# MaxChen228/pingpong-selfplay-ai

Measured on AMD Instinct MI355X. Metric: env-steps/sec (whole node) at 65536 arenas, 1/2/4/8 GPUs; CPU-ref baseline, higher is better.
Workload: dtype f64 env state / f32 QNet; 1 GPU; configs[2]: 65536 arenas/GPU, full DQN train_iterative loop (act both players + env tick + PER push/sample + double-DQN update + Adam + target sync); arenas_per_gpu=65536, global_arenas=65536, pool=8, batch=256, updates_per_vector_step=1, memory_size=1000000, parallelism=dp1 (arena shards, 1 all-reduce/update)

## Files before the change

### include/pongmi.h

```cpp
#ifndef PONGMI_H
#define PONGMI_H

#include <stddef.h>
#include <stdint.h>

#ifdef __cplusplus
extern "C" {
#endif

#define PM_ABI_VERSION 25

#define PM_OK 0
#define PM_E_ARG (-1)
#define PM_E_SIZE (-2)
#define PM_E_LAUNCH (-3)
#define PM_E_COMM (-4)


typedef struct pm_env_params {
    double paddle_width, paddle_speed, magnus_factor, restitution, friction, ball_mass, radius;
    double speed_lo, speed_hi, spin_lo, spin_hi;
    double ang0_lo, ang0_hi, ang1_lo, ang1_hi;
    double half_width, speed_scale, inertia, jt_coef, inv_mass, inv_inertia;
    int32_t max_score, speed_scale_every, enable_spin, _pad;
} pm_env_params;

typedef struct pm_env_state {
    double *x, *y, *vx, *vy, *spin, *top, *bot;
    int32_t *scoreA, *scoreB, *bounces, *serves;
} pm_env_state;

int pm_env_reset(const pm_env_params* p, const pm_env_state* s, const uint8_t* mask, const double* inject,
                 int32_t inject_cap, uint64_t seed, float* obsA, float* obsB, int32_t* status, int32_t n,
                 void* stream);

int pm_env_step(const pm_env_params* p, const pm_env_state* s, const int8_t* aA, const int8_t* aB, float* obsA,
                float* obsB, float* rA, float* rB, uint8_t* done, float* term_obsA, float* term_obsB,
                int32_t autoreset, const double* inject, int32_t inject_cap, uint64_t seed, uint64_t counter,
                int32_t* status, int32_t n, void* stream);

int pm_collide(const double* in, const double* inertia, double* out, int32_t n, void* stream);

int pm_env_step1(const pm_env_params* p, const pm_env_state* s, int32_t aA, int32_t aB, float* out, uint32_t seq,
                 void* stream);
int pm_env_reset1(const pm_env_state* s, double vx, double vy, double spin, float* out, uint32_t seq, void* stream);
int pm_collide1(const double* row, double inertia, double* out, uint32_t seq, void* stream);
void* pm_host_mapped_alloc(int64_t bytes, void** dev);
int pm_host_mapped_free(void* host);


#define PM_QNET_NP 5452
#define PM_QNET_NHEAD 520
#define PM_QNET_HEAD_OFF 4672
#define PM_QNET_EPS_OFF 5192
#define PM_QNET_NW 9944
#define PM_GRAD_EPISODES 520
#define PM_GRAD_UPDATED 521
#define PM_GRAD_LEN 528

#define PM_FOLD_EVAL 0
#define PM_FOLD_TRAIN 1
#define PM_FOLD_TRAIN_FRESH 2

int pm_qnet_fold(const float* params, float* params_out, int32_t mode, uint64_t seed, uint64_t counter,
                 const uint64_t* counter_dev, float* w_eff, int32_t count, void* stream);

int pm_qnet_q(const float* w_eff, const float* x, float* q, int32_t n, void* stream);

int pm_qnet_act(const float* w_opp, const int32_t* opp_id, int32_t n_opp, const float* w_B, const float* obsA,
                const float* obsB, float epsilon, const double* eps_dev, uint64_t seed, uint64_t counter,
                const uint64_t* counter_dev, int8_t* aA, int8_t* aB, float* qA, float* qB, int32_t n,
                int32_t chunk0, int32_t chunk1, void* stream);

int pm_play(const pm_env_params* p, const float* w_nets, int32_t n_nets, const int32_t* blk_nets,
            const int32_t* blk_range, int32_t n_blocks, const int32_t* order, const double* serves, int32_t n,
            int32_t max_steps, int32_t* scoreA, int32_t* scoreB, int32_t* length, int8_t* last, int32_t* status,
            void* stream);

int pm_play_rnn(const pm_env_params* p, const float* w_qnet, int32_t n_qnet, const float* w_rnn, int32_t n_rnn,
                const int32_t* blk_nets, const int32_t* blk_range, int32_t n_blocks, const int32_t* order,
                const double* serves, int32_t n, int32_t max_steps, float* hc_scratch,
                int32_t* scoreA, int32_t* scoreB, int32_t* length, int8_t* last, int32_t* status, void* stream);
size_t pm_play_rnn_scratch_bytes(int32_t n_blocks);

int pm_play_rec(const pm_env_params* p, const float* w_nets, int32_t n_nets, const int32_t* blk_nets,
                const int32_t* blk_range, int32_t n_blocks, const int32_t* order, const double* serves, int32_t n,
                int32_t max_steps, int32_t* scoreA, int32_t* scoreB, int32_t* length, int8_t* last, int32_t* status,
                const int32_t* rec_row, int32_t n_rec, int32_t rec_cap, double* rec_f64, float* rec_q,
                int32_t* rec_i32, void* stream);
int pm_play_rnn_rec(const pm_env_params* p, const float* w_qnet, int32_t n_qnet, const float* w_rnn, int32_t n_rnn,
                    const int32_t* blk_nets, const int32_t* blk_range, int32_t n_blocks, const int32_t* order,
                    const double* serves, int32_t n, int32_t max_steps, float* hc_scratch,
                    int32_t* scoreA, int32_t* scoreB, int32_t* length, int8_t* last, int32_t* status,
                    const int32_t* rec_row, int32_t n_rec, int32_t rec_cap, double* rec_f64, float* rec_q,
                    int32_t* rec_i32, void* stream);

#define PM_ROLL_HEADS 264
int pm_rollout(const pm_env_params* p, const pm_env_state* s, const float* wA, const float* wB, const float* paramsB,
               float epsilon, uint64_t seed_env, uint64_t seed_net, uint64_t counter0, int32_t steps, float* heads_ws,
               float* obsA, float* obsB, int64_t* stats, int32_t n, void* stream);

typedef struct pm_roll_replay {
    float *trans;
    float *prios;
    void *per_work;
    float *ep_reward;
    int64_t pos, cap;
    float prio, alpha;
} pm_roll_replay;
int pm_rollout_push(const pm_env_params* p, const pm_env_state* s, const float* wA, const float* wB,
                    const float* paramsB, float epsilon, uint64_t seed_env, uint64_t seed_net, uint64_t counter0,
                    int32_t steps, float* heads_ws, float* obsA, float* obsB, const pm_roll_replay* rp, int64_t* stats,
                    int32_t n, void* stream);


#define PM_RNN_NP 192012
#define PM_RNN_NPARAM 174984
#define PM_RNN_NW 157456

int pm_rnn_fold(const float* params, float* params_out, int32_t mode, uint64_t seed, uint64_t counter,
                const uint64_t* counter_dev, float* w_eff, int32_t count, void* stream);

int pm_rnn_q(const float* w_eff, const float* x, float* h, float* c, const uint8_t* reset, float* q, int32_t n,
             void* stream);

int pm_rnn_act(const float* w_opp, const int32_t* opp_id, int32_t n_opp, const float* w_B, const float* obsA,
               const float* obsB, float* hA, float* cA, float* hB, float* cB, const uint8_t* reset, float epsilon,
               const double* eps_dev, uint64_t seed, uint64_t counter, const uint64_t* counter_dev, int8_t* aA,
               int8_t* aB, float* qA, float* qB, int32_t n, int32_t chunk0, int32_t chunk1, const int32_t* opp_list,
               const int32_t* opp_cnt, void* stream);


typedef struct pm_drqn_stats {
    int64_t steps;
    int64_t adam_t;
    float loss;
    float norm;
    float q_mean;
    int32_t status;
} pm_drqn_stats;

typedef struct pm_drqn {
    float *params;
    float *target;
    float *adam_m, *adam_v;
    float *grad;
    void *work;
    pm_drqn_stats *stats;
    const float *obs, *next;
    const int32_t *act;
    const float *rew;
    const uint8_t *done;
    const int32_t *enable;
    int32_t batch;
    int32_t T;
    int64_t target_update_interval;
    double gamma, lr, beta1, beta2, adam_eps, max_norm;
    int32_t poll_limit;
    int32_t reserved;
} pm_drqn;

int64_t pm_drqn_work_bytes(int32_t batch, int32_t T);
int pm_drqn_init(const pm_drqn *d, void *stream);
int pm_drqn_grads(const pm_drqn *d, void *stream);
int pm_drqn_apply(const pm_drqn *d, void *stream);
int pm_drqn_update(const pm_drqn *d, void *stream);


typedef struct pm_rnn_ctrl {
    uint64_t step;
    int64_t episodes;
    int64_t seq_count;
    int64_t seq_size;
    double epsilon;
    int64_t win_A, ep_A, win_P, ep_P;
    double reward_B;
    int32_t status;
    int32_t train;
} pm_rnn_ctrl;

typedef struct pm_rnn_selfplay {
    pm_env_params env;
    pm_env_state st;
    int32_t *opp;
    float *ep_reward;
    int32_t *ep_len;
    int32_t *ep_steps;
    uint8_t *reset;
    const float *w_opp;
    float *paramsB;
    float *w_B;
    float *hA, *cA, *hB, *cB;
    float *obsA, *obsB;
    int8_t *aA, *aB;
    float *trans;
    int64_t *seq_eps;
    int64_t *seq_mark;
    int64_t *fin;
    int64_t *partials;
    int32_t *opp_list;
    int32_t *opp_cnt;
    int32_t *enable;
    pm_rnn_ctrl *ctrl;
    int32_t n, n_pool, depth, T, chunk_A, chunk_P;
    int32_t max_steps;
    int32_t _pad;
    int64_t seq_cap, min_episodes;
    double min_epsilon, epsilon_decay, pool_ratio;
    uint64_t seed_env, seed_net;
    const float *hA_in, *cA_in;
    float *qA, *qB;
} pm_rnn_selfplay;

int pm_rnn_selfplay_init(const pm_rnn_selfplay *sp, void *stream);
int pm_rnn_selfplay_act(const pm_rnn_selfplay *sp, void *stream);
int pm_rnn_selfplay_env(const pm_rnn_selfplay *sp, const pm_drqn *d, void *stream);
int pm_rnn_selfplay_rollout(const pm_rnn_selfplay *sp, const pm_drqn *d, void *stream);
int pm_rnn_selfplay_step(const pm_rnn_selfplay *sp, const pm_drqn *d, void *stream);
int pm_rnn_selfplay_sample(const pm_rnn_selfplay *sp, const pm_drqn *d, int32_t u, void *stream);
int pm_rnn_selfplay_step_multi(const pm_rnn_selfplay *sp, const pm_drqn *d, int32_t updates, void *stream);
int pm_rnn_selfplay_act_part(const pm_rnn_selfplay *sp, int32_t part, void *stream);
int pm_rnn_selfplay_step_overlap(const pm_rnn_selfplay *sp, const pm_drqn *d, int32_t updates, void *side_stream,
                                 void *stream);
int pm_rnn_selfplay_finish_overlap(const pm_rnn_selfplay *sp, const pm_drqn *d, int32_t updates, void *side_stream,
                                   void *stream);


#define PM_TRANS_F 16

int64_t pm_per_work_bytes(int64_t cap);
int pm_per_sample(const float* prios, int64_t size, float alpha, float beta, const double* u, uint64_t seed,
                  uint64_t counter, int64_t* idx, float* w, int32_t bs, void* work, void* stream);

int pm_per_update(float* prios, const int64_t* idx, const float* err, int32_t bs, void* stream);
int pm_per_build(const float* prios, int64_t cap, float alpha, void* work, void* stream);


typedef struct pm_ctrl {
    uint64_t step;
    int64_t pos, size;
    int64_t train_steps;
    int64_t frame_idx;
    int64_t episodes;
    double epsilon;
    float max_prio;
    float last_loss;
    int64_t ep_step;
    int64_t win_A, ep_A, win_P, ep_P;
    double reward_B;
    int32_t status;
    int32_t max_bits;
} pm_ctrl;

typedef struct pm_selfplay {
    pm_env_params env;
    pm_env_state st;
    int32_t *opp;
    float *ep_reward;
    float *w_opp;
    float *paramsB;
    float *paramsT;
    float *w_B;
    float *adam_m, *adam_v;
    float *trans;
    float *prios;
    void *per_work;
    int64_t *idx;
    float *isw;
    float *grad;
    int64_t *partials;
    float *obsA, *obsB;
    int8_t *aA, *aB;
    float *hfeat;
    float *learn_heads;
    pm_ctrl *ctrl;
    int32_t *opp_list;
    int32_t *opp_cnt;
    int32_t n, n_pool, batch, world;
    int32_t chunk_A, chunk_P;
    int32_t fuse_apply;
    int32_t _pad0;
    int64_t cap;
    double gamma, alpha, lr, beta1, beta2, adam_eps;
    double min_epsilon, epsilon_decay, pool_ratio, beta_start;
    int64_t beta_frames, target_update_interval;
    uint64_t seed_env;
    uint64_t seed_net;
    float *featB;
    float *frow;
    int32_t frow_ready;
    int32_t _pad1;
} pm_selfplay;

#define PM_MAX_BATCH 256

int pm_selfplay_init(const pm_selfplay* sp, void* stream);
int pm_selfplay_prepare(const pm_selfplay* sp, void* stream);
int pm_selfplay_repair_tree(const pm_selfplay* sp, void* stream);
int pm_selfplay_rollout(const pm_selfplay* sp, void* stream);
int pm_selfplay_act(const pm_selfplay* sp, void* stream);
int pm_selfplay_env(const pm_selfplay* sp, void* stream);
int pm_selfplay_learn(const pm_selfplay* sp, void* stream);
int pm_selfplay_apply(const pm_selfplay* sp, void* stream);
int pm_selfplay_step(const pm_selfplay* sp, void* stream);

#define PM_ACT_ALL 0
#define PM_ACT_B 1
#define PM_ACT_A 2
int pm_selfplay_act_part(const pm_selfplay* sp, int32_t part, void* stream);
int pm_selfplay_learn_act(const pm_selfplay* sp, void* stream);
int pm_selfplay_actenv(const pm_selfplay* sp, void* stream);
int pm_selfplay_step_overlap(const pm_selfplay* sp, void* stream);

#define PM_UPD_FIRST 1
#define PM_UPD_LAST 2
int pm_selfplay_learn_ex(const pm_selfplay* sp, int32_t mode, int32_t with_act, void* stream);
int pm_selfplay_apply_ex(const pm_selfplay* sp, int32_t mode, void* stream);
int pm_selfplay_resample(const pm_selfplay* sp, void* stream);
int pm_selfplay_commit(const pm_selfplay* sp, void* stream);
int pm_selfplay_step_multi(const pm_selfplay* sp, int32_t updates, void* stream);


#define PM_COMM_ID_BYTES 128
typedef struct pm_comm pm_comm;
int pm_comm_unique_id(const char* rccl_path, uint8_t* id);
int pm_comm_init(const char* rccl_path, const uint8_t* id, int32_t nranks, int32_t rank, pm_comm** out);
int pm_comm_allreduce_f32(pm_comm* comm, float* buf, int64_t n, void* stream);
int pm_comm_destroy(pm_comm* comm);
int pm_comm_info(const pm_comm* comm, int32_t* nranks, int32_t* rank, int32_t* device);
int pm_selfplay_step_sharded(const pm_selfplay* sp, pm_comm* comm, int32_t updates, void* stream);
int pm_rnn_selfplay_step_sharded(const pm_rnn_selfplay* sp, const pm_drqn* d, pm_comm* comm, int32_t updates,
                                 void* stream);
int pm_rnn_selfplay_step_sharded_overlap(const pm_rnn_selfplay* sp, const pm_drqn* d, pm_comm* comm, int32_t updates,
                                         void* side_stream, void* stream);

#define PM_TIMER_ACTENV 0
#define PM_TIMER_LEARN 1
#define PM_TIMER_RNN_ACT 2
#define PM_TIMER_ENV_STEP 3
#define PM_TIMER_ROLLOUT 4
#define PM_TIMER_DRQN 5
#define PM_TIMER_LEARN_MULTI 6
#define PM_TIMER_N 7
int pm_timer_arm(int32_t kernel);
int pm_timer_read(int32_t kernel, float* ms);

const char* pm_last_error(void);
int pm_abi_version(void);
int32_t pm_sizeof(int32_t which);

#ifdef __cplusplus
}
#endif
#endif
```

### pingpong-selfplay-ai_amd/csrc/pm_mfma.h

```cpp
#pragma once
#include "pm_dev.h"

namespace pm {

typedef float f32x16 __attribute__((ext_vector_type(16)));
typedef __attribute__((address_space(3))) void lds_void;

constexpr int PLAIN = 4936;
enum : int {
    F_W1 = 0,
    F_W2 = 512,
    F_B1 = 4608,
    F_B2 = 4672,
    F_H = 4736,
    F_BH = 4992,
    F_SIZE = 5008,
};
static_assert(PLAIN + F_SIZE == PM_QNET_NW, "effective weight block size");

__device__ __forceinline__ int rho(int r) { return (r & 3) + 8 * (r >> 2); }

__device__ __forceinline__ float relu(float x) { return __int_as_float(max(__float_as_int(x), 0)); }

__device__ __forceinline__ void write_feature_frags(const float* __restrict__ p, float* __restrict__ w) {
    const int t = threadIdx.x, nt = blockDim.x;
    for (int k = t; k < PM_QNET_HEAD_OFF; k += nt) w[k] = p[k];
    float* f = w + PLAIN;
    for (int k = t; k < 512; k += nt) {
        const int jt = k >> 8, lane = (k >> 2) & 63, s = k & 3;
        const int row = 32 * jt + (lane & 31), kk = 2 * s + (lane >> 5);
        f[F_W1 + k] = kk == 0 ? p[B1 + row] : p[W1 + row * 7 + kk - 1];
    }
    for (int k = t; k < 4096; k += nt) {
        const int e = k & 3, lane = (k >> 2) & 63, rq = (k >> 8) & 3, tt = (k >> 10) & 1, jt = k >> 11;
        const int row = 32 * jt + (lane & 31), col = 32 * tt + rho(4 * rq + e) + 4 * (lane >> 5);
        f[F_W2 + k] = p[W2 + row * 64 + col];
    }
    for (int k = t; k < 64; k += nt) {
        const int r = k & 15, h = (k >> 4) & 1, jt = k >> 5;
        f[F_B1 + k] = p[B1 + 32 * jt + rho(r) + 4 * h];
        f[F_B2 + k] = p[B2 + 32 * jt + rho(r) + 4 * h];
    }
}

__device__ __forceinline__ void write_head_frags(const float* heads, float* __restrict__ w) {
    const int t = threadIdx.x, nt = blockDim.x;
    for (int k = t; k < 260; k += nt) w[WH + k] = heads[k];
    float* f = w + PLAIN;
    for (int k = t; k < 256; k += nt) {
        const int c = k & 3, r = (k >> 2) & 15, tt = (k >> 6) & 1, h = k >> 7;
        f[F_H + k] = heads[c * 64 + 32 * tt + rho(r) + 4 * h];
    }
    if (t < 16) f[F_BH + t] = t < 4 ? heads[256 + t] : 0.f;
}

constexpr int kLwChunks = (F_SIZE / 4 + 63) / 64;
constexpr int kLwFloats = kLwChunks * 256;

template <int N>
__device__ __forceinline__ void copy_lds_f32(const float* __restrict__ src, float* dst) {
    const int wv = threadIdx.x >> 6, lane = threadIdx.x & 63, nw = blockDim.x >> 6;
    for (int c = wv; c * 64 < N; c += nw) {
        const int k = min(c * 64 + lane, N - 1);
        __builtin_amdgcn_global_load_lds((const void*)(src + k), (lds_void*)(dst + c * 64), 4, 0, 0);
    }
}
constexpr int pad64(int n) { return (n + 63) / 64 * 64; }
template <int N>
__device__ __forceinline__ void copy_lds_f32x4(const float* __restrict__ src, float* dst) {
    static_assert(N % 4 == 0, "whole float4s");
    const int wv = threadIdx.x >> 6, lane = threadIdx.x & 63, nw = blockDim.x >> 6;
    const float4* s4 = reinterpret_cast<const float4*>(src);
    for (int c = wv; c * 256 < N; c += nw) {
        const int k = min(c * 64 + lane, N / 4 - 1);
        __builtin_amdgcn_global_load_lds((const void*)(s4 + k), (lds_void*)(dst + c * 256), 16, 0, 0);
    }
}
constexpr int pad256(int n) { return (n + 255) / 256 * 256; }

__device__ __forceinline__ void stage_frags_lds(const float* __restrict__ w, float* lw, int rot) {
    const int wv = threadIdx.x >> 6, lane = threadIdx.x & 63, nw = blockDim.x >> 6;
    const float4* src = reinterpret_cast<const float4*>(w + PLAIN);
    float4* lw4 = reinterpret_cast<float4*>(lw);
    rot %= kLwChunks;
    for (int c0 = wv; c0 < kLwChunks; c0 += nw) {
        const int c = c0 + rot < kLwChunks ? c0 + rot : c0 + rot - kLwChunks;
        const int k = min(c * 64 + lane, F_SIZE / 4 - 1);
        __builtin_amdgcn_global_load_lds((const void*)(src + k), (lds_void*)(lw4 + c * 64), 16, 0, 0);
    }
}

constexpr int kListNets = 64;
constexpr int kListBlock = 256;
struct OppListSmem {
    int woff[kListBlock / 64][kListNets];
    int noff[kListNets], ncnt[kListNets];
};
__device__ __forceinline__ void write_opp_lists(int nn, int32_t* opp_list, int32_t* opp_cnt, OppListSmem& sm, int blk,
                                                int i, bool valid, int net) {
    if (nn > kListNets) return;
    const int lane = threadIdx.x & 63, wv = threadIdx.x >> 6;
    int rank = 0;
    for (int k = 0; k < nn; ++k) {
        const bool m = valid && net == k;
        const unsigned long long b = __ballot(m);
        if (m) rank = __popcll(b & ((1ull << lane) - 1ull));
        if (lane == 0) sm.woff[wv][k] = __popcll(b);
    }
    __syncthreads();
    if (wv == 0) {
        int acc = 0;
        if (lane < nn) {
            for (int w = 0; w < kListBlock / 64; ++w) {
                const int c = sm.woff[w][lane];
                sm.woff[w][lane] = acc;
                acc += c;
            }
        }
        const int inc = wave_incl_scan_i32(acc);
        if (lane < nn) { sm.ncnt[lane] = acc; sm.noff[lane] = inc - acc; }
    }
    __syncthreads();
    if (valid) opp_list[(size_t)blk * kListBlock + sm.noff[net] + sm.woff[wv][net] + rank] = i;
    if ((int)threadIdx.x < nn) opp_cnt[(size_t)blk * nn + threadIdx.x] = (sm.noff[threadIdx.x] << 16) | sm.ncnt[threadIdx.x];
}

__device__ __forceinline__ void compact_load(const int32_t* __restrict__ id, int lo, int hi, int (&v)[16]) {
    const int base = lo + 16 * (int)threadIdx.x;
    if (base + 16 <= hi && (reinterpret_cast<uintptr_t>(id + base) & 15) == 0) {
        const int4* p4 = reinterpret_cast<const int4*>(id + base);
#pragma unroll
        for (int q = 0; q < 4; ++q) {
            const int4 x = p4[q];
            v[4 * q] = x.x; v[4 * q + 1] = x.y; v[4 * q + 2] = x.z; v[4 * q + 3] = x.w;
        }
    } else {
#pragma unroll
        for (int r = 0; r < 16; ++r) v[r] = base + r < hi ? id[base + r] : -1;
    }
}
__device__ __forceinline__ void compact_scan(const int (&v)[16], int net, int lo, int* list, int* count, int* wtot) {
    const int t = threadIdx.x, lane = t & 63, wv = t >> 6, nw = blockDim.x >> 6;
    const int base = lo + 16 * t;
    unsigned mask = 0;
#pragma unroll
    for (int r = 0; r < 16; ++r) mask |= (v[r] == net ? 1u : 0u) << r;
    const int c = __popc(mask);
    const int incl = wave_incl_scan_i32(c);
    if (lane == 63) wtot[wv] = incl;
    __syncthreads();
    int off = 0, total = 0;
    for (int w = 0; w < nw; ++w) {
        off += w < wv ? wtot[w] : 0;
        total += wtot[w];
    }
    int p = off + incl - c;
    while (mask) {
        const int r = __ffs(mask) - 1;
        mask &= mask - 1;
        list[p++] = base + r;
    }
    if (t == 0) *count = total;
}

struct TileOut {
    int8_t* act;
    float* q;
    double eps;
    uint64_t seed, ctr;
};

__device__ __forceinline__ void heads_to_frags(const float* heads, float* hf) {
    for (int k = threadIdx.x; k < 260; k += blockDim.x) {
        if (k < 256) {
            const int c = k & 3, r = (k >> 2) & 15, tt = (k >> 6) & 1, h = k >> 7;
            hf[k] = heads[c * 64 + 32 * tt + rho(r) + 4 * h];
        } else {
            hf[k] = heads[k];
        }
    }
}

__device__ __forceinline__ void tile_hidden(const float* lw, const float (&xs)[4], int lane, f32x16 (&c2)[2]) {
    const int h = lane >> 5;
    f32x16 c1[2];
    const f32x16 zero = {};
#pragma unroll
    for (int jt = 0; jt < 2; ++jt) {
        const float4 w = reinterpret_cast<const float4*>(lw + F_W1)[jt * 64 + lane];
        c1[jt] = __builtin_amdgcn_mfma_f32_32x32x2f32(w.x, xs[0], zero, 0, 0, 0);
        c1[jt] = __builtin_amdgcn_mfma_f32_32x32x2f32(w.y, xs[1], c1[jt], 0, 0, 0);
        c1[jt] = __builtin_amdgcn_mfma_f32_32x32x2f32(w.z, xs[2], c1[jt], 0, 0, 0);
        c1[jt] = __builtin_amdgcn_mfma_f32_32x32x2f32(w.w, xs[3], c1[jt], 0, 0, 0);
    }
#pragma unroll
    for (int jt = 0; jt < 2; ++jt)
#pragma unroll
        for (int r = 0; r < 16; ++r) c1[jt][r] = relu(c1[jt][r]);
    const float4* w2 = reinterpret_cast<const float4*>(lw + F_W2) + lane;
#pragma unroll
    for (int jt = 0; jt < 2; ++jt) {
        const float4* b = reinterpret_cast<const float4*>(lw + F_B2 + (jt * 2 + h) * 16);
#pragma unroll
        for (int q4 = 0; q4 < 4; ++q4) {
            const float4 v = b[q4];
            c2[jt][4 * q4 + 0] = v.x; c2[jt][4 * q4 + 1] = v.y; c2[jt][4 * q4 + 2] = v.z; c2[jt][4 * q4 + 3] = v.w;
        }
    }
    float4 wcur = w2[0];
#pragma unroll
    for (int g8 = 0; g8 < 16; ++g8) {
        const int jt = g8 >> 3, t = (g8 >> 2) & 1, rq = g8 & 3;
        const float4 wnext = w2[((g8 + 1) & 15) * 64];
        c2[jt] = __builtin_amdgcn_mfma_f32_32x32x2f32(wcur.x, c1[t][4 * rq + 0], c2[jt], 0, 0, 0);
        c2[jt] = __builtin_amdgcn_mfma_f32_32x32x2f32(wcur.y, c1[t][4 * rq + 1], c2[jt], 0, 0, 0);
        c2[jt] = __builtin_amdgcn_mfma_f32_32x32x2f32(wcur.z, c1[t][4 * rq + 2], c2[jt], 0, 0, 0);
        c2[jt] = __builtin_amdgcn_mfma_f32_32x32x2f32(wcur.w, c1[t][4 * rq + 3], c2[jt], 0, 0, 0);
        wcur = wnext;
        __builtin_amdgcn_sched_barrier(0);
    }
}

__device__ __forceinline__ void tile_heads(const float* hf, const f32x16 (&c2)[2], int lane, float (&q)[3]) {
    const int h = lane >> 5;
    float v = 0.f, a0 = 0.f, a1 = 0.f, a2 = 0.f;
    const float4* hw = reinterpret_cast<const float4*>(hf + h * 128);
#pragma unroll
    for (int t = 0; t < 2; ++t) {
#pragma unroll
        for (int r = 0; r < 16; ++r) {
            const float x = relu(c2[t][r]);
            const float4 w = hw[t * 16 + r];
            v = fmaf(w.x, x, v);
            a0 = fmaf(w.y, x, a0);
            a1 = fmaf(w.z, x, a1);
            a2 = fmaf(w.w, x, a2);
        }
        __builtin_amdgcn_sched_barrier(0);
    }
    v += __shfl_xor(v, 32);
    a0 += __shfl_xor(a0, 32);
    a1 += __shfl_xor(a1, 32);
    a2 += __shfl_xor(a2, 32);
    v += hf[256];
    a0 += hf[257];
    a1 += hf[258];
    a2 += hf[259];
    const float mean = ((a0 + a1) + a2) / 3.0f;
    q[0] = v + (a0 - mean);
    q[1] = v + (a1 - mean);
    q[2] = v + (a2 - mean);
}

__device__ __forceinline__ void hidden_half(const float* lw, const float (&xs)[4], int lane, int jt, f32x16& c2) {
    const int h = lane >> 5;
    f32x16 c1[2];
    const f32x16 zero = {};
#pragma unroll
    for (int t = 0; t < 2; ++t) {
        const float4 w = reinterpret_cast<const float4*>(lw + F_W1)[t * 64 + lane];
        c1[t] = __builtin_amdgcn_mfma_f32_32x32x2f32(w.x, xs[0], zero, 0, 0, 0);
        c1[t] = __builtin_amdgcn_mfma_f32_32x32x2f32(w.y, xs[1], c1[t], 0, 0, 0);
        c1[t] = __builtin_amdgcn_mfma_f32_32x32x2f32(w.z, xs[2], c1[t], 0, 0, 0);
        c1[t] = __builtin_amdgcn_mfma_f32_32x32x2f32(w.w, xs[3], c1[t], 0, 0, 0);
    }
#pragma unroll
    for (int t = 0; t < 2; ++t)
#pragma unroll
        for (int r = 0; r < 16; ++r) c1[t][r] = relu(c1[t][r]);
    {
        const float4* b = reinterpret_cast<const float4*>(lw + F_B2 + (jt * 2 + h) * 16);
#pragma unroll
        for (int q4 = 0; q4 < 4; ++q4) {
            const float4 v = b[q4];
            c2[4 * q4 + 0] = v.x; c2[4 * q4 + 1] = v.y; c2[4 * q4 + 2] = v.z; c2[4 * q4 + 3] = v.w;
        }
    }
    const float4* w2 = reinterpret_cast<const float4*>(lw + F_W2) + lane + jt * 8 * 64;
    float4 wcur = w2[0];
#pragma unroll
    for (int g = 0; g < 8; ++g) {
        const int t = g >> 2, rq = g & 3;
        const float4 wnext = w2[((g + 1) & 7) * 64];
        c2 = __builtin_amdgcn_mfma_f32_32x32x2f32(wcur.x, c1[t][4 * rq + 0], c2, 0, 0, 0);
        c2 = __builtin_amdgcn_mfma_f32_32x32x2f32(wcur.y, c1[t][4 * rq + 1], c2, 0, 0, 0);
        c2 = __builtin_amdgcn_mfma_f32_32x32x2f32(wcur.z, c1[t][4 * rq + 2], c2, 0, 0, 0);
        c2 = __builtin_amdgcn_mfma_f32_32x32x2f32(wcur.w, c1[t][4 * rq + 3], c2, 0, 0, 0);
        wcur = wnext;
        __builtin_amdgcn_sched_barrier(0);
    }
}

__device__ __forceinline__ void heads_half(const float* hf, const f32x16& c2, int lane, int t, float (&acc)[4]) {
    const float4* hw = reinterpret_cast<const float4*>(hf + (lane >> 5) * 128) + t * 16;
#pragma unroll
    for (int r = 0; r < 16; ++r) {
        const float x = relu(c2[r]);
        const float4 w = hw[r];
        acc[0] = fmaf(w.x, x, acc[0]);
        acc[1] = fmaf(w.y, x, acc[1]);
        acc[2] = fmaf(w.z, x, acc[2]);
        acc[3] = fmaf(w.w, x, acc[3]);
    }
}

__device__ __forceinline__ void heads_finish(const float (&acc)[4], const float* hf, float (&q)[3]) {
    float v = acc[0], a0 = acc[1], a1 = acc[2], a2 = acc[3];
    v += __shfl_xor(v, 32);
    a0 += __shfl_xor(a0, 32);
    a1 += __shfl_xor(a1, 32);
    a2 += __shfl_xor(a2, 32);
    v += hf[256];
    a0 += hf[257];
    a1 += hf[258];
    a2 += hf[259];
    const float mean = ((a0 + a1) + a2) / 3.0f;
    q[0] = v + (a0 - mean);
    q[1] = v + (a1 - mean);
    q[2] = v + (a2 - mean);
}

__device__ __forceinline__ void tile_inputs(const float* __restrict__ o, int h, float (&xs)[4]) {
    xs[0] = h ? o[0] : 1.0f;
    xs[1] = o[1 + h];
    xs[2] = o[3 + h];
    xs[3] = o[5 + h];
}

struct TilePre {
    bool have;
    float xs[4];
};

__device__ __forceinline__ void run_tiles(const float* lw, const float* __restrict__ obs, const int* list, int count,
                                          const TileOut& out, const TilePre pre) {
    const int lane = threadIdx.x & 63, wave = threadIdx.x >> 6, nw = blockDim.x >> 6;
    const int h = lane >> 5, col = lane & 31;
    const int ntiles = (count + 31) >> 5;
    int tl = wave;
    if (tl >= ntiles) return;
    int arena = list[min(tl * 32 + col, count - 1)];
    float xs[4];
    if (pre.have) {
#pragma unroll
        for (int k = 0; k < 4; ++k) xs[k] = pre.xs[k];
    } else {
        tile_inputs(obs + (size_t)arena * 7, h, xs);
    }
    for (; tl < ntiles; tl += nw) {
        const int row = tl * 32 + col;
        const bool valid = row < count;
        const int tn = tl + nw;
        int arena_n = arena;
        float xn[4] = {xs[0], xs[1], xs[2], xs[3]};
        if (tn < ntiles) {
            arena_n = list[min(tn * 32 + col, count - 1)];
            tile_inputs(obs + (size_t)arena_n * 7, h, xn);
        }
        f32x16 c2[2];
#ifdef PM_DIAG
        if (tl == wave) {
            __builtin_amdgcn_s_waitcnt(0);
            PM_BLK(5);
        }
#endif
        tile_hidden(lw, xs, lane, c2);
#ifdef PM_DIAG
        if (tl == wave) PM_BLK(6);
#endif
        float q[3];
        tile_heads(lw + F_H, c2, lane, q);
#ifdef PM_DIAG
        if (tl == wave) PM_BLK(7);
#endif
        int a = argmax3(q);
        if (out.eps >= 0.0) {
            const U4 rr = philox64((uint32_t)arena, TAG_ACT, out.ctr, out.seed);
            if (u53(rr.x, rr.y) < out.eps) a = below(rr.z, 3u);
        }
        if (h == 0 && valid) {
            if (out.act) out.act[arena] = (int8_t)a;
            if (out.q) {
                out.q[(size_t)arena * 3 + 0] = q[0];
                out.q[(size_t)arena * 3 + 1] = q[1];
                out.q[(size_t)arena * 3 + 2] = q[2];
            }
        }
        arena = arena_n;
#pragma unroll
        for (int k = 0; k < 4; ++k) xs[k] = xn[k];
    }
}

constexpr int kChunkB = 256;

struct ActGrid {
    int n, n_opp, chunk0, chunk1, side_b;
    __host__ __device__ int nb() const { return side_b ? (n + kChunkB - 1) / kChunkB : 0; }
    __host__ __device__ int na0() const { return (n + chunk0 - 1) / chunk0; }
    __host__ __device__ int na1() const { return (n + chunk1 - 1) / chunk1; }
    __host__ __device__ int blocks() const { return nb() + na0() + (n_opp - 1) * na1(); }
};

constexpr int kActBlock = 256;
constexpr int kListMax = 4096;
constexpr int kListMaxLearn = 16384;

template <int LIST>
struct ActSharedT {
    static constexpr int kList = LIST;
    float lw[kLwFloats];
    int list[LIST];
    int count;
    int wtot[16];
    int lpre[LIST / 256], loff[LIST / 256], lcnt[LIST / 256];
};
using ActShared = ActSharedT<kListMax>;
using ActSharedLearn = ActSharedT<kListMaxLearn>;
static_assert(kListMaxLearn / 256 <= 64, "one lane per list segment in act_block's scan");

template <class Sh>
__device__ __forceinline__ void act_block(Sh& sh, const ActGrid& g, const float* __restrict__ w_opp,
                                          const int32_t* __restrict__ opp, const float* __restrict__ w_B,
                                          const float* __restrict__ obsA, const float* __restrict__ obsB,
                                          TileOut outA, TileOut outB, int b,
                                          const int32_t* __restrict__ opp_list = nullptr,
                                          const int32_t* __restrict__ opp_cnt = nullptr) {
    const float* w;
    const float* obs;
    TileOut out;
    int net, lo, hi;
    bool compact;
    if (b < g.nb()) {
        w = w_B; obs = obsB; out = outB; net = -1; lo = b * kChunkB; hi = min(lo + kChunkB, g.n); compact = false;
    } else {
        b -= g.nb();
        if (b < g.na0()) { net = 0; lo = b * g.chunk0; hi = min(lo + g.chunk0, g.n); }
        else { b -= g.na0(); net = 1 + b / g.na1(); lo = (b % g.na1()) * g.chunk1; hi = min(lo + g.chunk1, g.n); }
        w = w_opp + (size_t)net * PM_QNET_NW; obs = obsA; out = outA;
        compact = opp != nullptr;
        if (!compact && net != 0) return;
    }
    __builtin_amdgcn_s_setprio(2);
    stage_frags_lds(w, sh.lw, b);
    const bool lists = compact && opp_list != nullptr && (lo & 255) == 0 && (((hi - lo) & 255) == 0 || hi == g.n);
    int ids[16];
    if (compact && !lists) compact_load(opp, lo, hi, ids);
    PM_BLK(4);
    if (lists) {
        const int g0 = lo >> 8, G = (hi - lo + 255) >> 8;
        if (threadIdx.x < 64) {
            const int lane = threadIdx.x;
            const int v = lane < G ? opp_cnt[(size_t)(g0 + lane) * g.n_opp + net] : 0;
            const int c = v & 0xFFFF;
            const int incl = wave_incl_scan_i32(c);
            if (lane < G) { sh.lpre[lane] = incl - c; sh.loff[lane] = v >> 16; sh.lcnt[lane] = c; }
            if (lane == 63) sh.count = incl;
        }
        __syncthreads();
        const int j0 = threadIdx.x & 15;
        for (int seg = threadIdx.x >> 4; seg < G; seg += blockDim.x >> 4) {
            const int c = sh.lcnt[seg], dst = sh.lpre[seg];
            const int32_t* src = opp_list + (size_t)(g0 + seg) * 256 + sh.loff[seg];
            int v[16];
#pragma unroll
            for (int r = 0; r < 16; ++r) v[r] = j0 + 16 * r < c ? src[j0 + 16 * r] : 0;
#pragma unroll
            for (int r = 0; r < 16; ++r)
                if (j0 + 16 * r < c) sh.list[dst + j0 + 16 * r] = v[r];
        }
    } else if (compact) {
        compact_scan(ids, net, lo, sh.list, &sh.count, sh.wtot);
    } else {
        if (threadIdx.x == 0) sh.count = hi - lo;
        for (int k = threadIdx.x; k < hi - lo; k += blockDim.x) sh.list[k] = lo + k;
    }
    TilePre pre{false, {0.f, 0.f, 0.f, 0.f}};
    if (!compact && !lists) {
        const int wave = threadIdx.x >> 6, lane = threadIdx.x & 63, cnt = hi - lo;
        if (wave * 32 < cnt) {
            pre.have = true;
            tile_inputs(obs + (size_t)(lo + min(wave * 32 + (lane & 31), cnt - 1)) * 7, lane >> 5, pre.xs);
        }
    }
    __syncthreads();
    PM_BLK(1);
    __builtin_amdgcn_s_setprio(0);
    run_tiles(sh.lw, obs, sh.list, sh.count, out, pre);
}

constexpr int kFeatTileFloats = 8 * 64 * 4;
__device__ __forceinline__ void store_f4_sc1(__amdgpu_buffer_rsrc_t r, int byte_off, float4 v) {
    typedef __attribute__((ext_vector_type(4))) unsigned u32x4;
    __builtin_amdgcn_raw_buffer_store_b128(*reinterpret_cast<const u32x4*>(&v), r, byte_off, 0, 16 );
}
__device__ __forceinline__ void feat_tiles(float* lw, const float* __restrict__ w, const float* __restrict__ obs, int n,
                                           int t0, int t1, float* __restrict__ feat) {
    const int wave = threadIdx.x >> 6, lane = threadIdx.x & 63, nw = blockDim.x >> 6;
    stage_frags_lds(w, lw, t0);
    int tl = t0 + wave;
    float xs[4] = {0.f, 0.f, 0.f, 0.f};
    if (tl < t1) tile_inputs(obs + (size_t)min(tl * 32 + (lane & 31), n - 1) * 7, lane >> 5, xs);
    __syncthreads();
    for (; tl < t1; tl += nw) {
        const int tn = tl + nw;
        float xn[4] = {xs[0], xs[1], xs[2], xs[3]};
        if (tn < t1) tile_inputs(obs + (size_t)min(tn * 32 + (lane & 31), n - 1) * 7, lane >> 5, xn);
        f32x16 c2[2];
        tile_hidden(lw, xs, lane, c2);
        const __amdgpu_buffer_rsrc_t rs = __builtin_amdgcn_make_buffer_rsrc(feat, (short)0, 0x7fffffff, 0x00020000);
        const int off = (tl * 8 * 64 + lane) * 16;
#pragma unroll
        for (int k = 0; k < 4; ++k) {
            store_f4_sc1(rs, off + k * 64 * 16, make_float4(c2[0][4 * k], c2[0][4 * k + 1], c2[0][4 * k + 2], c2[0][4 * k + 3]));
            store_f4_sc1(rs, off + (4 + k) * 64 * 16,
                         make_float4(c2[1][4 * k], c2[1][4 * k + 1], c2[1][4 * k + 2], c2[1][4 * k + 3]));
        }
#pragma unroll
        for (int k = 0; k < 4; ++k) xs[k] = xn[k];
    }
}
__device__ __forceinline__ void feat_load(const float* __restrict__ feat, int tile, int lane, f32x16 (&c2)[2]) {
    const float4* src = reinterpret_cast<const float4*>(feat) + (size_t)tile * 8 * 64 + lane;
#pragma unroll
    for (int k = 0; k < 4; ++k) {
        const float4 a = src[k * 64], b = src[(4 + k) * 64];
        c2[0][4 * k] = a.x; c2[0][4 * k + 1] = a.y; c2[0][4 * k + 2] = a.z; c2[0][4 * k + 3] = a.w;
        c2[1][4 * k] = b.x; c2[1][4 * k + 1] = b.y; c2[1][4 * k + 2] = b.z; c2[1][4 * k + 3] = b.w;
    }
}

}
```

### pingpong-selfplay-ai_amd/csrc/pm_selfplay.hip

```cpp
#include <algorithm>
#include <cmath>

#include "pm_host.h"
#include "pm_mfma.h"
#include "pm_per.h"

using namespace pm;

#ifdef PM_DIAG
static __device__ unsigned long long pm_diag_env[8][1024];
static __device__ unsigned long long pm_diag_side[4][1024];
#define PM_SIDE(k, sb, v)                                                        \
    do {                                                                         \
        if (threadIdx.x == 0 && (sb) < 1024) pm_diag_side[(k)][(sb)] = (v);      \
    } while (0)
#define PM_ENV_STAMP(k, blk)                                                                   \
    do {                                                                                       \
        asm volatile("" ::: "memory");                                                         \
        if (threadIdx.x == 0 && (blk) < 1024) pm_diag_env[(k)][(blk)] = __builtin_amdgcn_s_memrealtime(); \
    } while (0)
#define PM_ENV_STAMP_DRAIN(k, blk)                                                             \
    do {                                                                                       \
        asm volatile("s_waitcnt vmcnt(0) lgkmcnt(0)" ::: "memory");                            \
        if (threadIdx.x == 0 && (blk) < 1024) pm_diag_env[(k)][(blk)] = __builtin_amdgcn_s_memrealtime(); \
    } while (0)
#else
#define PM_SIDE(k, sb, v) \
    do {                  \
    } while (0)
#define PM_ENV_STAMP(k, blk) \
    do {                     \
    } while (0)
#define PM_ENV_STAMP_DRAIN(k, blk) \
    do {                           \
    } while (0)
#endif

namespace {

constexpr int kBlock = 256;
static_assert(kBlock == kRowBlock, "row staging assumes kRowBlock-thread blocks");
constexpr int kLearn = 1024;
constexpr int kGradN = PM_GRAD_EPISODES;
static_assert(PM_GRAD_EPISODES == PM_QNET_NHEAD && PM_GRAD_UPDATED == kGradN + 1 && PM_GRAD_LEN >= kGradN + 2, "grad layout");
constexpr uint32_t kHashEmpty = 0xFFFFFFFFu;

__device__ __forceinline__ bool learner_active(const pm_selfplay& sp) {
    const int64_t s = sp.ctrl->size + sp.n;
    return (s < sp.cap ? s : sp.cap) >= sp.batch;
}

__device__ __forceinline__ double beta_of(const pm_selfplay& sp, int64_t frame) {
    const double b = sp.beta_start + (double)frame * (1.0 - sp.beta_start) / (double)sp.beta_frames;
    return b < 1.0 ? b : 1.0;
}

__device__ __forceinline__ float push_prio(int64_t size, float max_prio) { return size == 0 ? 1.0f : max_prio; }
__device__ __forceinline__ PushRange push_of(const pm_selfplay& sp, int64_t pos, int64_t size, float max_prio) {
    return PushRange{pos, sp.n, sp.cap, prio_pow(push_prio(size, max_prio), (float)sp.alpha)};
}
}

template <int NS = PER_BS, class Hook = NoHook>
__device__ __forceinline__ void sample_block(const pm_selfplay& sp, int b, bool pending, PerSampleSmem& sm,
                                             int64_t* sidx = nullptr, Hook l2done = Hook()) {
    static_assert(NS == PER_BS || NS == PER_BS / 2, "64 or 32 samples per block");
    const pm_ctrl* c = sp.ctrl;
    const int64_t s = c->size + sp.n;
    const int64_t size = s < sp.cap ? s : sp.cap;
    const int64_t frame = c->frame_idx + 1;
    const PushRange pr = pending ? push_of(sp, c->pos, c->size, c->max_prio) : PushRange{0, 0, sp.cap, 0.f};
    const uint64_t key = sp.seed_env;
    per_sample_block(
        size >= sp.batch, size, per_tree(sp.per_work, sp.cap), pr, beta_of(sp, frame), b * NS,
        min(sp.batch, b * NS + NS), sm,
        [&](int j) {
            const U4 r = philox64((uint32_t)j, TAG_PER, (uint64_t)frame, key);
            return u53(r.x, r.y);
        },
        [&](int j, int64_t idx, float w) {
            sp.idx[j] = idx;
            sp.isw[j] = w;
            if (sidx) sidx[j - b * NS] = idx;
        },
        l2done);
}

union ActSpShared {
    ActShared act;
    PerSampleSmem per;
};
constexpr int kFeatTilesAct = 8, kFeatTilesLearn = 16;
#ifndef PM_ENV_WT
#define PM_ENV_WT 6
#endif
constexpr bool kEnvWTRows = (PM_ENV_WT & 1) != 0, kEnvWTState = (PM_ENV_WT & 2) != 0, kEnvWTObs = (PM_ENV_WT & 4) != 0;
__host__ __device__ inline int feat_ntiles(int n) { return (n + 31) / 32; }

__global__ __launch_bounds__(kActBlock, 4) void k_act_sp(const pm_selfplay sp, int part) {
    __shared__ __attribute__((aligned(16))) ActSpShared sh;
    PM_BLK(0);
    const int nsb = part == PM_ACT_A ? 0 : (sp.batch + PER_BS - 1) / PER_BS;
    {
        const ActGrid g{sp.n, sp.n_pool + 1, sp.chunk_A, sp.chunk_P, part == PM_ACT_A ? 0 : 1};
        const int fb = (int)blockIdx.x - nsb - g.blocks();
        if (fb >= 0) {
            const int t0 = fb * kFeatTilesAct;
            feat_tiles(sh.act.lw, sp.w_B, sp.obsB, sp.n, t0, min(t0 + kFeatTilesAct, feat_ntiles(sp.n)), sp.featB);
            return;
        }
    }
    if ((int)blockIdx.x < nsb) {
        PM_STAMP(64);
        sample_block(sp, (int)blockIdx.x, true, sh.per);
        PM_STAMP(65);
        PM_BLK_END();
        return;
    }
    if ((int)blockIdx.x == nsb) PM_STAMP_ANY(70);
    const ActGrid g{sp.n, sp.n_pool + 1, sp.chunk_A, sp.chunk_P, part == PM_ACT_A ? 0 : 1};
    const TileOut outA{sp.aA, nullptr, -1.0, 0, 0};
    const TileOut outB{sp.aB, nullptr, -1.0, 0, 0};
    act_block(sh.act, g, sp.w_opp, sp.n_pool > 0 ? sp.opp : nullptr, sp.w_B, sp.obsA, sp.obsB, outA, outB,
              (int)blockIdx.x - nsb, sp.n_pool + 1 <= kListNets ? sp.opp_list : nullptr, sp.opp_cnt);
    PM_BLK_END();
}

__device__ __forceinline__ void batch_row_fwd(const pm_selfplay& sp, const float* lw, const float* hf0, const float* hf1,
                                              int64_t id, bool nxt, int lane, f32x16 (&c2)[2], float (&qb)[3],
                                              float (&qt)[3], float (&rb)[2]) {
    float xs[4];
    const float* tr = sp.trans + id * PM_TRANS_F;
    tile_inputs(tr + (nxt ? 8 : 0), lane >> 5, xs);
    rb[0] = tr[7];
    rb[1] = tr[15];
    tile_hidden(lw, xs, lane, c2);
    tile_heads(hf0, c2, lane, qb);
    tile_heads(hf1, c2, lane, qt);
}

template <bool WT = false>
__device__ __forceinline__ void store_hfeat(float* hfeat, int j, bool nxt, int lane, const f32x16 (&c2)[2],
                                            const float (&qb)[3], const float (&qt)[3], const float (&rb)[2]) {
    float* row = hfeat + (size_t)j * 80;
    const int h = lane >> 5;
    if (!nxt) {
#pragma unroll
        for (int t = 0; t < 2; ++t)
#pragma unroll
            for (int q = 0; q < 16; ++q) st_out<WT>(&row[32 * t + rho(q) + 4 * h], relu(c2[t][q]));
    }
    if (h == 0) {
        if (!nxt) {
            st_out<WT>(&row[64], qb[0]); st_out<WT>(&row[65], qb[1]); st_out<WT>(&row[66], qb[2]);
            st_out<WT>(&row[67], rb[0]);
            st_out<WT>(&row[71], rb[1]);
        } else {
            st_out<WT>(&row[68], qb[0]); st_out<WT>(&row[69], qb[1]); st_out<WT>(&row[70], qb[2]);
            st_out<WT>(&row[72], qt[0]); st_out<WT>(&row[73], qt[1]); st_out<WT>(&row[74], qt[2]);
        }
    }
}

__device__ __forceinline__ void env_fwd_block(const pm_selfplay& sp, int f, bool pending = true) {
    __shared__ __attribute__((aligned(16))) float lw[kLwFloats];
    __shared__ __attribute__((aligned(16))) float hf[2][264];
    if (!learner_active(sp)) return;
    stage_frags_lds(sp.w_B, lw, f * 5);
    for (int k = threadIdx.x; k < 2 * 264; k += blockDim.x) hf[k / 264][k % 264] = sp.learn_heads[k];
    __syncthreads();
    const int lane = threadIdx.x & 63, B = sp.batch;
    const int r0 = f * 128 + (int)(threadIdx.x >> 6) * 32;
    if (r0 >= 2 * B) return;
    const int r = min(r0 + (lane & 31), 2 * B - 1);
    const bool nxt = r >= B;
    const int j = nxt ? r - B : r;
    const int64_t id = sp.idx[j];
    const pm_ctrl* c = sp.ctrl;
    const bool mine = r0 + (lane & 31) < 2 * B && !(pending && push_of(sp, c->pos, c->size, c->max_prio).covers(id));
    f32x16 c2[2];
    float qb[3], qt[3];
    float rb[2];
    batch_row_fwd(sp, lw, hf[0], hf[1], id, nxt, lane, c2, qb, qt, rb);
    if (mine) store_hfeat(sp.hfeat, j, nxt, lane, c2, qb, qt, rb);
}

struct SampleFwd32Smem {
    PerSampleSmem per;
    float lw[kLwFloats];
    float hf[pad256(2 * 264)];
    int64_t sidx[PER_BS / 2];
    float part[2][64][8];
};
__device__ __forceinline__ void sample_fwd_block32(const pm_selfplay& sp, int b, SampleFwd32Smem& sm) {
    constexpr int NS = PER_BS / 2;
    sample_block<NS>(sp, b, true, sm.per, sm.sidx, [&] {
        stage_frags_lds(sp.w_B, sm.lw, b * 5);
        copy_lds_f32x4<2 * 264>(sp.learn_heads, sm.hf);
    });
    if (!learner_active(sp)) return;
    __syncthreads();
    PM_BLK(1);
    const int lane = threadIdx.x & 63, B = sp.batch;
    const int wv = __builtin_amdgcn_readfirstlane(threadIdx.x >> 6);
    const bool nxt = (wv >> 1) != 0;
    const int jt = wv & 1;
    const int j = b * NS + (lane & 31);
    const int64_t id = sm.sidx[min(j, B - 1) - b * NS];
    const pm_ctrl* c = sp.ctrl;
    const bool mine = j < B && !push_of(sp, c->pos, c->size, c->max_prio).covers(id);
    float xs[4];
    const float* tr = sp.trans + id * PM_TRANS_F;
    tile_inputs(tr + (nxt ? 8 : 0), lane >> 5, xs);
    const float rb0 = tr[7], rb1 = tr[15];
    f32x16 c2;
    hidden_half(sm.lw, xs, lane, jt, c2);
    const float* hf0 = sm.hf;
    const float* hf1 = sm.hf + 264;
    float ab[4] = {0.f, 0.f, 0.f, 0.f}, at[4] = {0.f, 0.f, 0.f, 0.f};
    float* row = sp.hfeat + (size_t)j * 80;
    const int h = lane >> 5;
    if (jt == 0) {
        heads_half(hf0, c2, lane, 0, ab);
        if (nxt) heads_half(hf1, c2, lane, 0, at);
        *reinterpret_cast<float4*>(&sm.part[nxt][lane][0]) = make_float4(ab[0], ab[1], ab[2], ab[3]);
        if (nxt) *reinterpret_cast<float4*>(&sm.part[nxt][lane][4]) = make_float4(at[0], at[1], at[2], at[3]);
    }
    if (mine && !nxt) {
#pragma unroll
        for (int q = 0; q < 16; ++q) row[32 * jt + rho(q) + 4 * h] = relu(c2[q]);
    }
    __syncthreads();
    if (jt == 0) return;
    {
        const float4 pa = *reinterpret_cast<const float4*>(&sm.part[nxt][lane][0]);
        ab[0] = pa.x; ab[1] = pa.y; ab[2] = pa.z; ab[3] = pa.w;
    }
    heads_half(hf0, c2, lane, 1, ab);
    float qb[3], qt[3];
    heads_finish(ab, hf0, qb);
    if (nxt) {
        const float4 pt = *reinterpret_cast<const float4*>(&sm.part[nxt][lane][4]);
        at[0] = pt.x; at[1] = pt.y; at[2] = pt.z; at[3] = pt.w;
        heads_half(hf1, c2, lane, 1, at);
        heads_finish(at, hf1, qt);
    }
    if (mine && h == 0) {
        if (!nxt) {
            row[64] = qb[0]; row[65] = qb[1]; row[66] = qb[2];
            row[67] = rb0;
            row[71] = rb1;
        } else {
            row[68] = qb[0]; row[69] = qb[1]; row[70] = qb[2];
            row[72] = qt[0]; row[73] = qt[1]; row[74] = qt[2];
        }
    }
}

__device__ __forceinline__ void write_opp_lists(const pm_selfplay& sp, OppListSmem& sm, int blk, int i, bool valid,
                                                int net) {
    write_opp_lists(sp.n_pool + 1, sp.opp_list, sp.opp_cnt, sm, blk, i, valid, net);
}

struct EnvSmem {
    float lds[2][kBlock][7];
    long long red[kBlock / 64][6];
    OppListSmem ol;
};
struct ActEnvSmem {
    EnvSmem e;
    float lw[kLwFloats];
};

template <bool ACT>
__device__ __forceinline__ void env_block(const pm_selfplay& sp, int blk, EnvSmem& sm, float* lw) {
    const int i0 = blk * kBlock;
    const int i = i0 + threadIdx.x;
    const int lane = threadIdx.x & 63, wv = threadIdx.x >> 6;
    const bool valid = i < sp.n;
    const int ii = valid ? i : sp.n - 1;
    const pm_ctrl* c = sp.ctrl;
    if (blk == 0) PM_STAMP_ANY(72);
    PM_ENV_STAMP(0, blk);
    float xs[2][4];
    f32x16 fc2[2][2];
    if (ACT && sp.featB) {
        if (threadIdx.x < 65)
            reinterpret_cast<float4*>(lw + F_H)[threadIdx.x] =
                reinterpret_cast<const float4*>(sp.w_B + PLAIN + F_H)[threadIdx.x];
#pragma unroll
        for (int k = 0; k < 2; ++k) feat_load(sp.featB, blk * 8 + 2 * wv + k, lane, fc2[k]);
    } else if (ACT) {
        stage_frags_lds(sp.w_B, lw, blk);
#pragma unroll
        for (int k = 0; k < 2; ++k) {
            const int row = min(i0 + 64 * wv + 32 * k + (lane & 31), sp.n - 1);
            tile_inputs(sp.obsB + (size_t)row * 7, lane >> 5, xs[k]);
        }
    }
    const uint32_t ns = (uint32_t)__builtin_nontemporal_load(&sp.st.serves[ii]);
    const int64_t pos = c->pos, size = c->size;
    const float cmaxp = c->max_prio;
    const uint64_t cstep = c->step;
    const double ceps = c->epsilon;
    const int o = sp.opp[ii];
    const float er0 = sp.ep_reward[ii];
    Arena a = load_arena(sp.st, ii);
    const int aA = sp.aA[ii];
    int aB = ACT ? 0 : sp.aB[ii];
    __builtin_amdgcn_sched_barrier(0);
    const float maxp = push_prio(size, cmaxp);
    float* leaf = per_tree(sp.per_work, sp.cap).leaf;
    const float pval = prio_pow(maxp, (float)sp.alpha);

    int onext, eps_a;
    bool eps_hit;
    double svx, svy, sspn;
    {
        const U4 rr = philox64((uint32_t)ii, TAG_ACT, cstep, sp.seed_env);
        eps_hit = u53(rr.x, rr.y) < ceps;
        eps_a = (int)below(rr.z, 3u);
        const U4 q = philox((uint32_t)ii, TAG_OPP, ns, 0u, sp.seed_env);
        onext = (sp.n_pool > 0 && u53(q.x, q.y) < sp.pool_ratio) ? 1 + below(q.z, (uint32_t)sp.n_pool) : 0;
        philox_serve(sp.env, (uint32_t)ii, ns, sp.seed_env, svx, svy, sspn);
        asm volatile("" ::"v"(onext), "v"(svx), "v"(svy), "v"(sspn), "v"(eps_hit), "v"(eps_a));
        __builtin_amdgcn_sched_barrier(0);
    }
    if (ACT) {
        __syncthreads();
        PM_ENV_STAMP(7, blk);
        int act[2];
#pragma unroll
        for (int k = 0; k < 2; ++k) {
            float q[3];
            if (sp.featB) {
                tile_heads(lw + F_H, fc2[k], lane, q);
            } else {
                f32x16 c2[2];
                tile_hidden(lw, xs[k], lane, c2);
                tile_heads(lw + F_H, c2, lane, q);
            }
            act[k] = argmax3(q);
            if (sp.featB && sp.frow) {
                const int ar = i0 + 64 * wv + 32 * k + (lane & 31);
                if (ar < sp.n) {
                    int64_t slot = pos + ar;
                    if (slot >= sp.cap) slot -= sp.cap;
                    float4* fr = reinterpret_cast<float4*>(sp.frow + slot * 64) + (lane >> 5);
#pragma unroll
                    for (int jt = 0; jt < 2; ++jt)
#pragma unroll
                        for (int q4 = 0; q4 < 4; ++q4)
                            st_f4<kEnvWTRows>(fr + 8 * jt + 2 * q4,
                                              make_float4(relu(fc2[k][jt][4 * q4]), relu(fc2[k][jt][4 * q4 + 1]),
                                                          relu(fc2[k][jt][4 * q4 + 2]), relu(fc2[k][jt][4 * q4 + 3])));
                }
            }
        }
        aB = lane < 32 ? act[0] : act[1];
    }
    PM_ENV_STAMP(1, blk);
    if (eps_hit) aB = eps_a;
    float oA[7], oB[7];
    observe(a, oA, oB);
    float rA, rB;
    const int d = tick(sp.env, a, aA, aB, rA, rB);
    float nA[7], nB[7];
    observe(a, nA, nB);
#ifdef PM_DIAG
    asm volatile("" ::"v"(nA[0]), "v"(nB[1]), "v"(d));
#endif
    PM_ENV_STAMP(2, blk);
    const float er = er0 + rB;
    const bool fin = valid && d;
    {
        const bool win = er > 0.f;
        const unsigned long long mf = __ballot(fin), mA = __ballot(fin && o == 0), mwA = __ballot(fin && o == 0 && win);
        const unsigned long long mP = __ballot(fin && o != 0), mwP = __ballot(fin && o != 0 && win);
        const int rs = wave_sum(fin ? (int)er : 0);
        if (lane == 0) {
            sm.red[wv][0] = __popcll(mf); sm.red[wv][1] = __popcll(mA); sm.red[wv][2] = __popcll(mwA);
            sm.red[wv][3] = __popcll(mP); sm.red[wv][4] = __popcll(mwP); sm.red[wv][5] = rs;
        }
    }
    int onew = o;
    if (valid) {
        int64_t slot = pos + i;
        if (slot >= sp.cap) slot -= sp.cap;
        float4* row = reinterpret_cast<float4*>(sp.trans + slot * PM_TRANS_F);
        st_f4<kEnvWTRows>(row + 0, make_float4(oB[0], oB[1], oB[2], oB[3]));
        st_f4<kEnvWTRows>(row + 1, make_float4(oB[4], oB[5], oB[6], rB));
        st_f4<kEnvWTRows>(row + 2, make_float4(nB[0], nB[1], nB[2], nB[3]));
        st_f4<kEnvWTRows>(row + 3, make_float4(nB[4], nB[5], nB[6], __int_as_float(aB | (d << 8))));
        sp.prios[slot] = maxp;
        leaf[slot] = pval;
        float ernew = er;
        if (d) {
            onew = onext;
            serve(a, svx, svy, sspn);
            sp.st.serves[i] = (int32_t)ns + 1;
            ernew = 0.f;
            observe(a, nA, nB);
        }
        store_arena<kEnvWTState>(sp.st, i, a);
        sp.opp[i] = onew;
        sp.aB[i] = (int8_t)aB;
        sp.ep_reward[i] = ernew;
    }
    PM_ENV_STAMP(3, blk);
#pragma unroll
    for (int k = 0; k < 7; ++k) { sm.lds[0][threadIdx.x][k] = nA[k]; sm.lds[1][threadIdx.x][k] = nB[k]; }
    __syncthreads();
    PM_ENV_STAMP(4, blk);
    if (threadIdx.x < 6) {
        long long t = 0;
        for (int w = 0; w < kBlock / 64; ++w) t += sm.red[w][threadIdx.x];
        sp.partials[(size_t)blk * 8 + threadIdx.x] = t;
    }
    write_opp_lists(sp, sm.ol, blk, i, valid, onew);
    PM_ENV_STAMP(5, blk);
    copy_rows7<kEnvWTObs>(sp.obsA, sm.lds[0], i0, sp.n);
    copy_rows7<kEnvWTObs>(sp.obsB, sm.lds[1], i0, sp.n);
    PM_ENV_STAMP_DRAIN(6, blk);
}

__global__ __launch_bounds__(kBlock) void k_env(const pm_selfplay sp) {
    const int blk = (int)blockIdx.x;
    const int nenv = (sp.n + kBlock - 1) / kBlock;
    if (blk >= nenv) {
        env_fwd_block(sp, blk - nenv);
        return;
    }
    __shared__ __attribute__((aligned(16))) EnvSmem sm;
    env_block<false>(sp, blk, sm, nullptr);
}

union ActEnvShared {
    ActEnvSmem ae;
    SampleFwd32Smem sf32;
};
__global__ __launch_bounds__(kBlock) void k_actenv(const pm_selfplay sp) {
    __shared__ __attribute__((aligned(16))) ActEnvShared sh;
    const int nsb = (sp.batch + 31) / 32;
    if ((int)blockIdx.x < nsb) {
        PM_BLK(0);
        sample_fwd_block32(sp, (int)blockIdx.x, sh.sf32);
        PM_BLK_END();
        return;
    }
    env_block<true>(sp, (int)blockIdx.x - nsb, sh.ae.e, sh.ae.lw);
}

__global__ __launch_bounds__(kBlock) void k_sp_init(const pm_selfplay sp) {
    __shared__ __attribute__((aligned(16))) float lds[kBlock][7];
    const int i0 = blockIdx.x * kBlock;
    const int i = i0 + threadIdx.x;
    float oA[7] = {0}, oB[7] = {0};
    int net = 0;
    if (i < sp.n) {
        const uint32_t ns = (uint32_t)sp.st.serves[i];
        const U4 q = philox((uint32_t)i, TAG_OPP, ns, 0u, sp.seed_env);
        net = (sp.n_pool > 0 && u53(q.x, q.y) < sp.pool_ratio) ? 1 + below(q.z, (uint32_t)sp.n_pool) : 0;
        sp.opp[i] = net;
        Arena a;
        double vx, vy, spn;
        philox_serve(sp.env, (uint32_t)i, ns, sp.seed_env, vx, vy, spn);
        serve(a, vx, vy, spn);
        store_arena(sp.st, i, a);
        sp.st.serves[i] = (int32_t)ns + 1;
        sp.ep_reward[i] = 0.f;
        observe(a, oA, oB);
    }
    {
        __shared__ OppListSmem ol;
        write_opp_lists(sp, ol, blockIdx.x, i, i < sp.n, net);
    }
    store_rows7(sp.obsA, lds, oA, i0, sp.n);
    store_rows7(sp.obsB, lds, oB, i0, sp.n);
}

struct __attribute__((aligned(16))) ApplySmem {
    float hp[pad256(PM_QNET_NHEAD)];
    float tmu[pad256(PM_QNET_NHEAD)];
    float m[pad256(PM_QNET_NHEAD)], v[pad256(PM_QNET_NHEAD)];
    float g[PM_QNET_NHEAD + 2];
    float ak[2];
    float nact[132], ntrain[132];
    float heads[3][260];
    double eps_next;
};

__device__ __forceinline__ void adam_consts(const pm_selfplay& sp, int64_t ts, ApplySmem& sm) {
    const double bc1 = 1.0 - pow(sp.beta1, (double)ts);
    const double bc2 = 1.0 - pow(sp.beta2, (double)ts);
    sm.ak[0] = (float)(sp.lr / bc1);
    sm.ak[1] = (float)sqrt(bc2);
}
__device__ __forceinline__ void adam_const_lane(const pm_selfplay& sp, int64_t ts, ApplySmem& sm, int which) {
    const double bc = 1.0 - pow(which ? sp.beta2 : sp.beta1, (double)ts);
    sm.ak[which] = which ? (float)sqrt(bc) : (float)(sp.lr / bc);
}

__device__ __forceinline__ void load_apply_inputs(const pm_selfplay& sp, ApplySmem& sm, bool with_grad) {
    copy_lds_f32x4<PM_QNET_NHEAD>(sp.paramsB + PM_QNET_HEAD_OFF, sm.hp);
    copy_lds_f32x4<PM_QNET_NHEAD>(sp.paramsT + PM_QNET_HEAD_OFF, sm.tmu);
    copy_lds_f32x4<PM_QNET_NHEAD>(sp.adam_m, sm.m);
    copy_lds_f32x4<PM_QNET_NHEAD>(sp.adam_v, sm.v);
    if (with_grad)
        for (int k = threadIdx.x; k < PM_QNET_NHEAD + 2; k += blockDim.x) sm.g[k] = sp.grad[k];
}

__device__ __forceinline__ void derive_weights(const pm_selfplay& sp, ApplySmem& sm) {
    const int t = threadIdx.x;
    float* lh = sp.learn_heads;
    const int g = (t - 256) >> 8, u = (t - 256) & 255;
    if (t >= 256 && g == 0) {
        fold_heads_from(sm.hp, nullptr, sm.nact, PM_FOLD_TRAIN_FRESH, sm.heads[0], sp.paramsB + PM_QNET_EPS_OFF, u, 256);
    } else if (t >= 256 && g == 1) {
        fold_heads_from(sm.hp, nullptr, sm.ntrain, PM_FOLD_TRAIN_FRESH, sm.heads[1], lh + 528, u, 256);
    } else if (t >= 256 && g == 2) {
        fold_heads_from(sm.tmu, nullptr, nullptr, PM_FOLD_EVAL, sm.heads[2], nullptr, u, 256);
    }
    __syncthreads();
    write_head_frags(sm.heads[0], sp.w_B);
    heads_to_frags(sm.heads[1], lh);
    heads_to_frags(sm.heads[2], lh + 264);
}

__device__ __forceinline__ void derive_weights_lds(ApplySmem& sm) {
    const int t = threadIdx.x;
    const int g = (t - 256) >> 8, u = (t - 256) & 255;
    if (t >= 256 && g == 1) {
        fold_heads_from(sm.hp, nullptr, sm.ntrain, PM_FOLD_TRAIN_FRESH, sm.heads[1], nullptr, u, 256);
    } else if (t >= 256 && g == 2) {
        fold_heads_from(sm.tmu, nullptr, nullptr, PM_FOLD_EVAL, sm.heads[2], nullptr, u, 256);
    }
    __syncthreads();
}

__device__ __forceinline__ void gen_both_noises(const pm_selfplay& sp, ApplySmem& sm, uint64_t act_ctr,
                                                uint64_t train_ctr) {
    const int t = threadIdx.x, half = blockDim.x / 2;
    if (t < half) gen_noise(sp.seed_net, TAG_NOISE_ACT, act_ctr, sm.nact, t, half);
    else gen_noise(sp.seed_net, TAG_NOISE_TRAIN, train_ctr, sm.ntrain, t - half, half);
}
__device__ __forceinline__ void gen_both_noises_on(const pm_selfplay& sp, ApplySmem& sm, uint64_t act_ctr,
                                                   uint64_t train_ctr, int t0) {
    const int u = (int)threadIdx.x - t0;
    if (u < 0 || u >= 512) return;
    if (u < 256) gen_noise(sp.seed_net, TAG_NOISE_ACT, act_ctr, sm.nact, u, 256);
    else gen_noise(sp.seed_net, TAG_NOISE_TRAIN, train_ctr, sm.ntrain, u - 256, 256);
}

__device__ __forceinline__ void adam_one(const pm_selfplay& sp, ApplySmem& sm, int k, float gsum, bool store = true) {
    const float step_size = sm.ak[0], bc2s = sm.ak[1];
    const float g = gsum / (float)sp.world;
    float m = sm.m[k], v = sm.v[k], p = sm.hp[k];
    m = m + (float)(1.0 - sp.beta1) * (g - m);
    v = v * (float)sp.beta2 + (float)(1.0 - sp.beta2) * g * g;
    const float denom = sqrtf(v) / bc2s + (float)sp.adam_eps;
    p = p - step_size * (m / denom);
    if (store) {
        sp.paramsB[PM_QNET_HEAD_OFF + k] = p;
        sp.adam_m[k] = m;
        sp.adam_v[k] = v;
    }
    sm.hp[k] = p;
    sm.m[k] = m;
    sm.v[k] = v;
}
__device__ __forceinline__ void apply_adam(const pm_selfplay& sp, ApplySmem& sm) {
    const int t = threadIdx.x, nt = blockDim.x;
    if (sm.g[kGradN + 1] > 0.5f)
        for (int k = t; k < PM_QNET_NHEAD; k += nt) adam_one(sp, sm, k, sm.g[k]);
}
__device__ __forceinline__ void apply_finish(const pm_selfplay& sp, ApplySmem& sm, const pm_ctrl& cs, int mode) {
    const int t = threadIdx.x, nt = blockDim.x;
    const bool train = sm.g[kGradN + 1] > 0.5f;
    const int64_t ts = cs.train_steps + (train ? 1 : 0);
    const uint64_t step = cs.step;
    PM_STAMP(20);
    if (train && ts % sp.target_update_interval == 0) {
        for (int k = t; k < PM_QNET_NHEAD; k += nt) sm.tmu[k] = sm.hp[k];
        for (int k = t; k < PM_QNET_NP; k += nt) {
            const int h = k - PM_QNET_HEAD_OFF;
            sp.paramsT[k] = (h >= 0 && h < PM_QNET_NHEAD) ? sm.hp[h] : sp.paramsB[k];
        }
        __syncthreads();
    }
    derive_weights(sp, sm);
    PM_STAMP(21);
    if (t == 0) {
        pm_ctrl* c = sp.ctrl;
        if (mode & PM_UPD_FIRST) {
            const double e = sm.eps_next;
            c->epsilon = e > sp.min_epsilon ? e : sp.min_epsilon;
        }
        if (train) { c->train_steps = ts; c->frame_idx = cs.frame_idx + 1; }
        if (mode & PM_UPD_LAST) {
            c->pos = (cs.pos + sp.n) % sp.cap;
            const int64_t s = cs.size + sp.n;
            c->size = s < sp.cap ? s : sp.cap;
            c->step = step + 1;
        }
    }
}

template <typename Emit>
__device__ __forceinline__ void push_rows_fwd(const pm_selfplay& sp, const float* lw, const float* hf,
                                              const int64_t* sidx, const int* plist, const int* pcnt, int wv, int lane,
                                              Emit emit) {
    int pre[5] = {0, 0, 0, 0, 0};
#pragma unroll
    for (int w = 0; w < 4; ++w) pre[w + 1] = pre[w] + pcnt[w];
    const int np = pre[4];
    if (wv * 32 >= 2 * np) return;
    const int rr = min(wv * 32 + (lane & 31), 2 * np - 1);
    const bool nxt = rr >= np;
    const int k = nxt ? rr - np : rr;
    const int w = k >= pre[3] ? 3 : k >= pre[2] ? 2 : k >= pre[1] ? 1 : 0;
    const int pw = k >= pre[3] ? pre[3] : k >= pre[2] ? pre[2] : k >= pre[1] ? pre[1] : 0;
    const int j = plist[w * 64 + k - pw];
    f32x16 c2[2];
    float qb[3], qt[3], rb[2];
    batch_row_fwd(sp, lw, hf, hf + 264, sidx[j], nxt, lane, c2, qb, qt, rb);
    if (wv * 32 + (lane & 31) < 2 * np) emit(j, nxt, lane, c2, qb, qt, rb);
}

constexpr int kPushPollMax = 20000;
constexpr int PM_CTRL_PUSH_TIMEOUT = 1;
constexpr int PM_CTRL_NAN_PRIO = 2;
__device__ __forceinline__ bool push_handoff(int mode, bool train) { return (mode & PM_UPD_FIRST) && train; }
__device__ __forceinline__ int* push_flag(const pm_selfplay& sp) {
    return reinterpret_cast<int*>(sp.hfeat + (size_t)2 * sp.batch * 80);
}
__device__ __forceinline__ int push_token(const pm_ctrl& cs) { return (int)((uint32_t)cs.step + 1u); }
__device__ __forceinline__ uint32_t* tr_epoch(const pm_selfplay& sp) {
    return reinterpret_cast<uint32_t*>(sp.hfeat + (size_t)2 * sp.batch * 80) + 1;
}
constexpr int kPushGF = 76;
constexpr int kPushGN = 75;
__device__ __forceinline__ uint64_t* push_granules(const pm_selfplay& sp) {
    return reinterpret_cast<uint64_t*>(sp.hfeat + (size_t)(2 * sp.batch + 8) * 80);
}
__device__ __forceinline__ void push_publish(uint64_t* g, uint32_t tag, float v) {
    __hip_atomic_store(g, ((uint64_t)tag << 32) | __float_as_uint(v), __ATOMIC_RELAXED, __HIP_MEMORY_SCOPE_AGENT);
}

__device__ __forceinline__ bool push_wait(const pm_selfplay& sp, const pm_ctrl& cs) {
    const int* flag = push_flag(sp);
    const int tok = push_token(cs);
    for (int it = 0; __hip_atomic_load(flag, __ATOMIC_RELAXED, __HIP_MEMORY_SCOPE_AGENT) != tok; ++it) {
        if (it == kPushPollMax) {
            sp.ctrl->status = cs.status | PM_CTRL_PUSH_TIMEOUT;
            return false;
        }
        __builtin_amdgcn_s_sleep(2);
    }
    return true;
}

struct PushFwdSmem {
    float lw[kLwFloats];
    float hf[pad256(2 * 264)];
    int64_t sidx[PM_MAX_BATCH];
    int plist[PM_MAX_BATCH];
    int pcnt[16];
    float part[8][64][8];
};

__device__ __forceinline__ void push_rows_fwd2(const pm_selfplay& sp, PushFwdSmem& sm, int wv, int lane, float* pay,
                                               uint32_t gtag) {
    uint64_t* pg = push_granules(sp);
    auto put = [&](int j, int f, float v) {
        if (gtag) push_publish(pg + (size_t)j * kPushGF + f, gtag, v);
        else st_out<true>(pay + (size_t)j * 80 + f, v);
    };
    int pre[5] = {0, 0, 0, 0, 0};
#pragma unroll
    for (int w = 0; w < 4; ++w) pre[w + 1] = pre[w] + sm.pcnt[w];
    const int np = pre[4];
    const int ntile = (2 * np + 31) >> 5;
    const int jt = wv & 1, h = lane >> 5;
    const float* hf0 = sm.hf;
    const float* hf1 = sm.hf + 264;
    for (int it = 0; it * 8 < ntile; ++it) {
        const int tile = it * 8 + (wv >> 1);
        const bool act = tile < ntile;
        f32x16 c2 = {};
        float ab[4] = {0.f, 0.f, 0.f, 0.f}, at[4] = {0.f, 0.f, 0.f, 0.f};
        float rb0 = 0.f, rb1 = 0.f;
        bool nxt = false, mine = false;
        int j = 0;
        if (act) {
            const int r0 = tile * 32 + (lane & 31);
            const int rr = min(r0, 2 * np - 1);
            nxt = rr >= np;
            const int k = nxt ? rr - np : rr;
            const int w = k >= pre[3] ? 3 : k >= pre[2] ? 2 : k >= pre[1] ? 1 : 0;
            const int pw = k >= pre[3] ? pre[3] : k >= pre[2] ? pre[2] : k >= pre[1] ? pre[1] : 0;
            j = sm.plist[w * 64 + k - pw];
            mine = r0 < 2 * np;
            const float* tr = sp.trans + sm.sidx[j] * PM_TRANS_F;
            float xs[4];
            tile_inputs(tr + (nxt ? 8 : 0), h, xs);
            rb0 = tr[7];
            rb1 = tr[15];
            hidden_half(sm.lw, xs, lane, jt, c2);
            if (mine && !nxt) {
#pragma unroll
                for (int q = 0; q < 16; ++q) put(j, 32 * jt + rho(q) + 4 * h, relu(c2[q]));
            }
            if (jt == 0) {
                heads_half(hf0, c2, lane, 0, ab);
                heads_half(hf1, c2, lane, 0, at);
                *reinterpret_cast<float4*>(&sm.part[wv >> 1][lane][0]) = make_float4(ab[0], ab[1], ab[2], ab[3]);
                *reinterpret_cast<float4*>(&sm.part[wv >> 1][lane][4]) = make_float4(at[0], at[1], at[2], at[3]);
            }
        }
        __syncthreads();
        if (act && jt == 1) {
            const float4 pb = *reinterpret_cast<const float4*>(&sm.part[wv >> 1][lane][0]);
            const float4 pt = *reinterpret_cast<const float4*>(&sm.part[wv >> 1][lane][4]);
            ab[0] = pb.x; ab[1] = pb.y; ab[2] = pb.z; ab[3] = pb.w;
            at[0] = pt.x; at[1] = pt.y; at[2] = pt.z; at[3] = pt.w;
            heads_half(hf0, c2, lane, 1, ab);
            heads_half(hf1, c2, lane, 1, at);
            float qb[3], qt[3];
            heads_finish(ab, hf0, qb);
            heads_finish(at, hf1, qt);
            if (mine && h == 0) {
                if (!nxt) {
                    put(j, 64, qb[0]); put(j, 65, qb[1]); put(j, 66, qb[2]);
                    put(j, 67, rb0);
                    put(j, 71, rb1);
                } else {
                    put(j, 68, qb[0]); put(j, 69, qb[1]); put(j, 70, qb[2]);
                    put(j, 72, qt[0]); put(j, 73, qt[1]); put(j, 74, qt[2]);
                }
            }
        }
        if ((it + 1) * 8 < ntile) __syncthreads();
    }
}
__device__ __forceinline__ pm_ctrl push_fwd_block(const pm_selfplay& sp, int mode, PushFwdSmem& sm, bool push2, bool pushg) {
    const int t = threadIdx.x, lane = t & 63, wv = t >> 6, B = sp.batch;
    PM_STAMP_ANY(50);
    stage_frags_lds(sp.w_B, sm.lw, 0);
    copy_lds_f32x4<2 * 264>(sp.learn_heads, sm.hf);
    const int64_t id = t < B ? sp.idx[t] : 0;
    const uint32_t gtag = pushg ? __hip_atomic_load(tr_epoch(sp), __ATOMIC_RELAXED, __HIP_MEMORY_SCOPE_AGENT) + 1u : 0u;
    __builtin_amdgcn_sched_barrier(0);
    const pm_ctrl cs = *sp.ctrl;
    const int64_t s_after = cs.size + sp.n < sp.cap ? cs.size + sp.n : sp.cap;
    if (!push_handoff(mode, s_after >= B)) {
        if ((mode & PM_UPD_FIRST) && t == 0) st_out<true>(push_flag(sp), push_token(cs));
        return cs;
    }
    if (pushg && t == 0) st_out<true>(push_flag(sp), push_token(cs));
    const bool ip = t < B && push_of(sp, cs.pos, cs.size, cs.max_prio).covers(id);
    const unsigned long long m = __ballot(ip);
    if (ip) sm.plist[wv * 64 + __popcll(m & ((1ull << lane) - 1ull))] = t;
    if (lane == 0) sm.pcnt[wv] = __popcll(m);
    if (t < B) sm.sidx[t] = id;
    __syncthreads();
    PM_STAMP_ANY(51);
    float* pay = sp.hfeat + (size_t)B * 80;
    if (push2)
        push_rows_fwd2(sp, sm, wv, lane, pay, gtag);
    else
        push_rows_fwd(sp, sm.lw, sm.hf, sm.sidx, sm.plist, sm.pcnt, wv, lane,
                      [&](int j, bool nxt, int ln, const f32x16 (&c2)[2], const float (&qb)[3], const float (&qt)[3],
                          const float (&rb)[2]) { store_hfeat<true>(pay, j, nxt, ln, c2, qb, qt, rb); });
    PM_STAMP_ANY(52);
    if (pushg) return cs;
    asm volatile("s_waitcnt vmcnt(0)" ::: "memory");
    __syncthreads();
    PM_STAMP_ANY(53);
    if (t == 0) st_out<true>(push_flag(sp), push_token(cs));
    return cs;
}

constexpr int kTrSlots = PM_MAX_BATCH + 8;
constexpr int kTrHash = 1024;
constexpr uint32_t kTrEmpty = 0xFFFFFFFFu;
constexpr int kTrPollMax = 20000;
constexpr int PM_CTRL_TREE_TIMEOUT = 4;
constexpr int PM_CTRL_TREE_REPAIRED = 8;
struct TreeRefreshSmem {
    __attribute__((aligned(16))) float lf[kTrSlots][PER_SUB];
    __attribute__((aligned(16))) double ls[kTrSlots][PER_FAN];
    double subv[kTrSlots];
    uint32_t subid[kTrSlots], chid[kTrSlots];
    int16_t cmap[kTrSlots][PER_FAN];
    uint32_t skey[kTrHash];
    int sslot[kTrHash];
    uint32_t ckey[kTrHash];
    int cslot[kTrHash];
    uint32_t ikey[512];
    int iwin[512];
    uint32_t eidx[kTrSlots];
    int esub[kTrSlots];
    float leaf_new[PM_MAX_BATCH];
    float maxp_next;
    int scattered, ok, nsub, nch;
};
__device__ __forceinline__ uint64_t* tr_granules(const pm_selfplay& sp) {
    return reinterpret_cast<uint64_t*>(sp.hfeat + (size_t)(2 * sp.batch + 1) * 80);
}
__device__ __forceinline__ void tr_publish(const pm_selfplay& sp, int k, uint32_t v, uint32_t tag) {
    __hip_atomic_store(tr_granules(sp) + k, ((uint64_t)tag << 32) | v, __ATOMIC_RELAXED, __HIP_MEMORY_SCOPE_AGENT);
}
__device__ __forceinline__ int tr_hash(uint32_t k, int bits) { return (int)((k * 2654435761u) >> (32 - bits)); }
__device__ __forceinline__ int tr_insert(uint32_t* key, uint32_t k, int bits) {
    const int mask = (1 << bits) - 1;
    int h = tr_hash(k, bits);
    for (;;) {
        const uint32_t old = atomicCAS(&key[h], kTrEmpty, k);
        if (old == kTrEmpty || old == k) return h;
        h = (h + 1) & mask;
    }
}
__device__ __forceinline__ int tr_lookup(const uint32_t* key, uint32_t k, int bits) {
    const int mask = (1 << bits) - 1;
    for (int h = tr_hash(k, bits);; h = (h + 1) & mask) {
        const uint32_t v = key[h];
        if (v == k) return h;
        if (v == kTrEmpty) return -1;
    }
}

__device__ __forceinline__ void tree_block(const pm_selfplay& sp, int mode, TreeRefreshSmem& sm, const pm_ctrl& cs,
                                           int poll_max) {
    const int t = threadIdx.x, lane = t & 63, wv = t >> 6, B = sp.batch;
    PM_STAMP_ANY(55);
    const PerTree tree = per_tree(sp.per_work, sp.cap);
    const uint32_t tag = __hip_atomic_load(tr_epoch(sp), __ATOMIC_RELAXED, __HIP_MEMORY_SCOPE_AGENT) + 1u;
    const bool last = mode & PM_UPD_LAST;
    const int64_t s_after = cs.size + sp.n < sp.cap ? cs.size + sp.n : sp.cap;
    const int ns = s_after >= B ? B : 0;
    const int64_t npos = (cs.pos + sp.n) % sp.cap;
    const int64_t end1 = npos + sp.n < sp.cap ? npos + sp.n : sp.cap;
    const int64_t end2 = npos + sp.n - sp.cap;
    const int nedge = last ? (end2 > 0 ? 4 : 2) : 0;
    const int ne = ns + nedge;
    for (int k = t; k < kTrHash; k += kLearn) { sm.skey[k] = kTrEmpty; sm.ckey[k] = kTrEmpty; }
    for (int k = t; k < 512; k += kLearn) { sm.ikey[k] = kTrEmpty; sm.iwin[k] = -1; }
    for (int k = t; k < kTrSlots * PER_FAN; k += kLearn) (&sm.cmap[0][0])[k] = -1;
    if (t == 0) { sm.nsub = 0; sm.nch = 0; sm.ok = 1; }
    if (t < ne) {
        const int64_t e = t < ns ? sp.idx[t] : (t - ns == 0 ? npos : t - ns == 1 ? end1 - 1 : t - ns == 2 ? 0 : end2 - 1);
        sm.eidx[t] = (uint32_t)e;
    }
    __syncthreads();
    if (t < ne) {
        tr_insert(sm.skey, sm.eidx[t] / PER_SUB, 10);
        if (t < ns) atomicMax(&sm.iwin[tr_insert(sm.ikey, sm.eidx[t], 9)], t);
    }
    __syncthreads();
    if (t < kTrHash && sm.skey[t] != kTrEmpty) {
        const int s = atomicAdd(&sm.nsub, 1);
        sm.sslot[t] = s;
        sm.subid[s] = sm.skey[t];
    }
    __syncthreads();
    const int nsub = sm.nsub;
    if (t < ne) sm.esub[t] = sm.sslot[tr_lookup(sm.skey, sm.eidx[t] / PER_SUB, 10)];
    if (t < nsub) tr_insert(sm.ckey, sm.subid[t] / PER_FAN, 10);
    __syncthreads();
    if (t < kTrHash && sm.ckey[t] != kTrEmpty) {
        const int c = atomicAdd(&sm.nch, 1);
        sm.cslot[t] = c;
        sm.chid[c] = sm.ckey[t];
    }
    __syncthreads();
    const int nch = sm.nch;
    if (t < nsub) sm.cmap[sm.cslot[tr_lookup(sm.ckey, sm.subid[t] / PER_FAN, 10)]][sm.subid[t] % PER_FAN] = (int16_t)t;
    for (int i = wv; 4 * i < nsub; i += kLearn / 64) {
        const int s = min(4 * i + (lane >> 4), nsub - 1);
        __builtin_amdgcn_global_load_lds((const void*)(tree.leaf + (size_t)sm.subid[s] * PER_SUB + 4 * (lane & 15)),
                                         (lds_void*)&sm.lf[4 * i][0], 16, 0, 0);
    }
    for (int i = wv; 8 * i < nch; i += kLearn / 64) {
        const int c = min(8 * i + (lane >> 3), nch - 1);
        __builtin_amdgcn_global_load_lds((const void*)(tree.sub + (size_t)sm.chid[c] * PER_FAN + 2 * (lane & 7)),
                                         (lds_void*)&sm.ls[8 * i][0], 16, 0, 0);
    }
    PM_STAMP_ANY(56);
    if (t < B + 2) {
        uint64_t g = 0;
        bool got = false;
        for (int it = 0; it < poll_max; ++it) {
            g = __hip_atomic_load(tr_granules(sp) + t, __ATOMIC_RELAXED, __HIP_MEMORY_SCOPE_AGENT);
            if ((uint32_t)(g >> 32) == tag) { got = true; break; }
            __builtin_amdgcn_s_sleep(2);
        }
        if (!got) sm.ok = 0;
        const uint32_t v = (uint32_t)g;
        if (t < B) sm.leaf_new[t] = __uint_as_float(v);
        else if (t == B) sm.maxp_next = __uint_as_float(v);
        else sm.scattered = (int)(v & 1u);
    }
    asm volatile("s_waitcnt vmcnt(0)" ::: "memory");
    __syncthreads();
    PM_STAMP_ANY(57);
    if (!sm.ok) {
        if (t == 0) {
            atomicOr(&sp.ctrl->status, PM_CTRL_TREE_TIMEOUT);
            __hip_atomic_store(tr_epoch(sp), tag, __ATOMIC_RELAXED, __HIP_MEMORY_SCOPE_AGENT);
        }
        return;
    }
    if (sm.scattered && t < ns && sm.iwin[tr_lookup(sm.ikey, sm.eidx[t], 9)] == t)
        sm.lf[sm.esub[t]][sm.eidx[t] % PER_SUB] = sm.leaf_new[t];
    const float pval = last ? prio_pow(push_prio(s_after, sm.maxp_next), (float)sp.alpha) : 0.f;
    const PushRange next = last ? PushRange{npos, sp.n, sp.cap, pval} : PushRange{0, 0, sp.cap, 0.f};
    const int cap32 = (int)sp.cap;
    const int q1lo = last ? (int)npos : 0, q1hi = last ? (int)end1 : 0, q2hi = last && end2 > 0 ? (int)end2 : 0;
    const int p1lo = (q1lo + PER_SUB - 1) / PER_SUB, p1hi = q1hi / PER_SUB, p2hi = q2hi / PER_SUB;
    PM_STAMP_ANY(60);
    __syncthreads();
    for (int base = 0; base < 4 * nsub; base += kLearn) {
        const int k = base + t, s = min(k >> 2, nsub - 1), q = k & 3;
        const int lo = (int)sm.subid[s] * PER_SUB + 16 * q;
        float v[16];
        const float4* l4 = reinterpret_cast<const float4*>(&sm.lf[s][16 * q]);
#pragma unroll
        for (int j = 0; j < 4; ++j) {
            const float4 x = l4[j];
            v[4 * j] = x.x; v[4 * j + 1] = x.y; v[4 * j + 2] = x.z; v[4 * j + 3] = x.w;
        }
#pragma unroll
        for (int j = 0; j < 16; ++j) asm volatile("" : "+v"(v[j]));
        double acc = 0.0;
#pragma unroll
        for (int i = 0; i < 16; ++i) {
            const int e = lo + i;
            const bool pushed = (e >= q1lo && e < q1hi) || e < q2hi;
            const double x = (double)(pushed ? pval : v[i]);
            acc += e < cap32 ? x : 0.0;
        }
        const double node = per_combine(quad_f64<0>(acc), quad_f64<1>(acc), quad_f64<2>(acc), quad_f64<3>(acc));
        if (q == 0 && k < 4 * nsub) {
            sm.subv[s] = node;
            tree.sub[sm.subid[s]] = node;
        }
    }
    PM_STAMP_ANY(61);
    const double csub = per_sub_pushed_sum(next);
    {
        const int n1 = p1hi > p1lo ? p1hi - p1lo : 0;
        for (int k = t; k < n1 + p2hi; k += kLearn) tree.sub[k < n1 ? p1lo + k : k - n1] = csub;
    }
    PM_STAMP_ANY(62);
    __syncthreads();
    PM_STAMP_ANY(58);
    const int nsub_tree = (int)tree.nsub;
    static_assert(PER_FAN == 16, "one DPP row per level-2 node");
    for (int base = wv * 4; base < nch; base += kLearn / 16) {
        const int slot = min(base + (lane >> 4), nch - 1), k = lane & 15;
        const int m = sm.cmap[slot][k];
        const double old = sm.ls[slot][k];
        const double fresh = sm.subv[m >= 0 ? m : 0];
        const int sb = (int)sm.chid[slot] * PER_FAN + k;
        const bool pushed = (sb >= p1lo && sb < p1hi) || sb < p2hi;
        const double v = m >= 0 ? fresh : (pushed ? csub : old);
        const double x = sb < nsub_tree ? v : 0.0;
        double acc = 0.0;
        acc += x;
        acc += dpp_f64<0x101>(x); acc += dpp_f64<0x102>(x); acc += dpp_f64<0x103>(x);
        acc += dpp_f64<0x104>(x); acc += dpp_f64<0x105>(x); acc += dpp_f64<0x106>(x);
        acc += dpp_f64<0x107>(x); acc += dpp_f64<0x108>(x); acc += dpp_f64<0x109>(x);
        acc += dpp_f64<0x10A>(x); acc += dpp_f64<0x10B>(x); acc += dpp_f64<0x10C>(x);
        acc += dpp_f64<0x10D>(x); acc += dpp_f64<0x10E>(x); acc += dpp_f64<0x10F>(x);
        if (k == 0 && base + (lane >> 4) < nch) tree.chunk[sm.chid[slot]] = acc;
    }
    PM_STAMP_ANY(63);
    if (last) {
        double cc = 0.0;
#pragma unroll
        for (int k = 0; k < PER_FAN; ++k) cc += csub;
        const int c1lo = q1lo / PER_CHUNK, c1hi = (q1hi - 1) / PER_CHUNK + 1;
        const int c2hi = q2hi > 0 ? (q2hi - 1) / PER_CHUNK + 1 : 0;
        const int n1 = c1hi > c1lo ? c1hi - c1lo : 0;
        for (int k = t; k < n1 + c2hi; k += kLearn) {
            const int ch = k < n1 ? c1lo + k : k - n1;
            if (tr_lookup(sm.ckey, (uint32_t)ch, 10) < 0) tree.chunk[ch] = cc;
        }
    }
    PM_STAMP_ANY(59);
    if (t == 0) __hip_atomic_store(tr_epoch(sp), tag, __ATOMIC_RELAXED, __HIP_MEMORY_SCOPE_AGENT);
}

struct LearnSmem {
    union {
        float gpart[16][256];
    } u;
    __attribute__((aligned(16))) float Hs[PM_MAX_BATCH][64];
    __attribute__((aligned(16))) float qv4[3][PM_MAX_BATCH][4];
    float coef[PM_MAX_BATCH][4];
    float eps_tr[pad256(260)];
    int64_t sidx[PM_MAX_BATCH];
    uint32_t hkey[512];
    int hwin[512];
    float red[16][8];
    long long cnt[16][6];
    long long ctot[6];
    int plist[PM_MAX_BATCH];
    int pcnt[16];
    int void_upd;
    float loss_out;
    ApplySmem ap;
};

union LearnShared {
    LearnSmem learn;
    ActSharedLearn act;
    PushFwdSmem pf;
    TreeRefreshSmem tr;
};
static_assert(sizeof(LearnShared) <= 160 * 1024, "k_learn LDS");

__device__ __forceinline__ void side_nap(int n) {
    for (int i = 0; i < n; ++i) __builtin_amdgcn_s_sleep(16);
}

template <bool PG>
__global__ __launch_bounds__(kLearn) void k_learn(const pm_selfplay sp, int chunkA, int chunkP, int mode, int tr, int ftiles, int sleepf) {
    __shared__ __attribute__((aligned(16))) LearnShared shm;
    const bool push2 = (tr & 2) != 0, late_noise = (tr & 4) != 0;
    const int tr_poll = (tr & 16) ? 0 : kTrPollMax;
    constexpr bool pushg = PG;
    tr &= 1;
    if (blockIdx.x > 0) {
        if (blockIdx.x == 1) {
            const pm_ctrl cs = push_fwd_block(sp, mode, shm.pf, push2, pushg);
            if (tr) {
                __syncthreads();
                tree_block(sp, mode, shm.tr, cs, tr_poll);
            }
            return;
        }
        const int sb = (int)blockIdx.x - 2;
        PM_SIDE(0, sb, __builtin_amdgcn_s_memrealtime());
        const ActGrid g{sp.n, sp.n_pool + 1, chunkA, chunkP, 0};
        const int fb = sb - g.blocks();
        if (fb >= 0) {
            if (sleepf & 2) side_nap(sleepf >> 8);
            const int t0 = fb * ftiles;
            feat_tiles(shm.act.lw, sp.w_B, sp.obsB, sp.n, t0, min(t0 + ftiles, feat_ntiles(sp.n)), sp.featB);
            PM_STAMP_MAX(67);
            PM_SIDE(2, sb, __builtin_amdgcn_s_memrealtime());
            PM_SIDE(3, sb, 1ull | ((unsigned long long)(min(t0 + ftiles, feat_ntiles(sp.n)) - t0) << 16));
            return;
        }
        if (sleepf & 1) side_nap(sleepf >> 8);
        PM_SIDE(1, sb, __builtin_amdgcn_s_memrealtime());
        const TileOut outA{sp.aA, nullptr, -1.0, 0, 0};
        act_block(shm.act, g, sp.w_opp, sp.n_pool > 0 ? sp.opp : nullptr, nullptr, sp.obsA, nullptr, outA, outA,
                  sb, sp.n_pool + 1 <= kListNets ? sp.opp_list : nullptr, sp.opp_cnt);
        PM_STAMP_MAX(66);
        PM_SIDE(2, sb, __builtin_amdgcn_s_memrealtime());
        PM_SIDE(3, sb, 0ull | ((unsigned long long)shm.act.count << 16));
        return;
    }
    LearnSmem& sm = shm.learn;
    const int t = threadIdx.x, lane = t & 63, wv = t >> 6;
    const int B = sp.batch;
    pm_ctrl* c = sp.ctrl;
    PM_STAMP(0);
    const pm_ctrl cs = *c;
    const PerTree tree = per_tree(sp.per_work, sp.cap);
    const bool first = mode & PM_UPD_FIRST, last = mode & PM_UPD_LAST;

    const int nbr = (sp.n + kBlock - 1) / kBlock;
    copy_lds_f32x4<260>(sp.learn_heads + 528, sm.eps_tr);
    if (sp.fuse_apply) load_apply_inputs(sp, sm.ap, false);
    long long part[6] = {0, 0, 0, 0, 0, 0};
    if (first && t < nbr) {
#pragma unroll
        for (int k = 0; k < 6; ++k) part[k] = sp.partials[(size_t)t * 8 + k];
    }
    const float wraw_l = t < B ? sp.isw[t] : 0.f;
    const int64_t id_l = t < B ? sp.idx[t] : 0;
    const float eps_v = t < 260 ? sp.learn_heads[528 + t] : 0.f;
    const uint32_t tr_tag = tr ? __hip_atomic_load(tr_epoch(sp), __ATOMIC_RELAXED, __HIP_MEMORY_SCOPE_AGENT) + 1u : 0u;
    if (t < PM_MAX_BATCH) {
        const float4* src = reinterpret_cast<const float4*>(sp.hfeat + (size_t)min(t, B - 1) * 80 + 64);
#pragma unroll
        for (int k = 0; k < 3; ++k)
            __builtin_amdgcn_global_load_lds((const void*)(src + k), (lds_void*)&sm.qv4[k][wv * 64][0], 16, 0, 0);
    }
    for (int b = t + kLearn; first && b < nbr; b += kLearn)
#pragma unroll
        for (int k = 0; k < 6; ++k) part[k] += sp.partials[(size_t)b * 8 + k];
    const int64_t s_after = cs.size + sp.n < sp.cap ? cs.size + sp.n : sp.cap;
    bool train = s_after >= B;
    const bool train0 = train;
    bool act = train && t < B;
    if (t == 0) sm.void_upd = 0;
    PM_STAMP(35);
    if (sp.fuse_apply && !late_noise) {
        if (t >= kLearn - 2) adam_const_lane(sp, cs.train_steps + 1, sm.ap, t - (kLearn - 2));
        gen_both_noises_on(sp, sm.ap, cs.step + 1, (uint64_t)(cs.train_steps + (train ? 1 : 0)) + 1, kLearn / 2);
    }
    PM_STAMP(34);
    if (train && t < 260) sp.paramsB[PM_QNET_EPS_OFF + t] = eps_v;
    const float wraw = act ? wraw_l : 0.f;
    const int64_t id = act ? id_l : 0;
    for (int k = t; k < 512; k += kLearn) { sm.hkey[k] = kHashEmpty; sm.hwin[k] = -1; }
    if (act) sm.sidx[t] = id;
    {
        const bool ip = first && act && push_of(sp, cs.pos, cs.size, cs.max_prio).covers(id);
        const unsigned long long m = __ballot(ip);
        if (ip) sm.plist[wv * 64 + __popcll(m & ((1ull << lane) - 1ull))] = t;
        if (lane == 0) sm.pcnt[wv] = __popcll(m);
    }
    PM_STAMP(16);
#if defined(PM_DIAG) && !defined(PM_DIAG_NOWAIT)
    PM_STAMP(30);
    asm volatile("" ::"v"(wraw_l), "v"((int)id_l));
    PM_STAMP(31);
    PM_STAMP(32);
    PM_STAMP(33);
#endif
#pragma unroll
    for (int k = 0; k < 6; ++k) {
        const long long s = wave_sum(part[k]);
        if (lane == 0) sm.cnt[wv][k] = s;
    }
    PM_STAMP(17);
    {
        const float m = wave_max(wraw);
        if (lane == 0) sm.red[wv][0] = m;
    }
    PM_STAMP(18);
    PM_STAMP_T(19, 960);
    if (train)
        for (int ci = wv; 4 * ci < B; ci += kLearn / 64) {
            const int row = min(4 * ci + (lane >> 4), B - 1);
            __builtin_amdgcn_global_load_lds((const void*)(sp.hfeat + (size_t)row * 80 + 4 * (lane & 15)),
                                             (lds_void*)&sm.Hs[4 * ci][0], 16, 0, 0);
        }
#if defined(PM_DIAG) && !defined(PM_DIAG_NOWAIT)
    asm volatile("s_waitcnt vmcnt(0) lgkmcnt(0)" ::: "memory");
    PM_STAMP_T(40, 0); PM_STAMP_T(41, 256); PM_STAMP_T(42, 512); PM_STAMP_T(43, 960);
#endif
    __syncthreads();
    PM_STAMP(1);

    long long ep_fin = 0;
    bool waited = false;
    if (t < 6) {
        long long s = 0;
        for (int w = 0; w < 16; ++w) s += sm.cnt[w][t];
        sm.ctot[t] = s;
    }
    if (sp.fuse_apply && first && !late_noise && t == kLearn - 1) {
        long long s = 0;
        for (int w = 0; w < 16; ++w) s += sm.cnt[w][0];
        sm.ap.eps_next = cs.epsilon * pow(sp.epsilon_decay, (double)(float)s);
        PM_STAMP_T(37, kLearn - 1);
    }
    if (train) {
        int pre[5] = {0, 0, 0, 0, 0};
#pragma unroll
        for (int w = 0; w < 4; ++w) pre[w + 1] = pre[w] + sm.pcnt[w];
        const int np = pre[4];
        if (np > 0 && push_handoff(mode, train)) {
            waited = true;
            if constexpr (PG) {
                const uint64_t* pg = push_granules(sp);
                const int tot = np * kPushGN;
                uint64_t g[4];
                int jf[4];
                auto issue = [&](int k0) {
#pragma unroll
                    for (int u = 0; u < 4; ++u) {
                        const int k = k0 + u * kLearn;
                        g[u] = (uint64_t)tr_tag << 32;
                        jf[u] = 0;
                        if (k < tot) {
                            const int q = k / kPushGN, f = k - q * kPushGN;
                            const int w = q >= pre[3] ? 3 : q >= pre[2] ? 2 : q >= pre[1] ? 1 : 0;
                            const int pw = q >= pre[3] ? pre[3] : q >= pre[2] ? pre[2] : q >= pre[1] ? pre[1] : 0;
                            jf[u] = sm.plist[w * 64 + q - pw] * kPushGF + f;
                            g[u] = __hip_atomic_load(pg + jf[u], __ATOMIC_RELAXED, __HIP_MEMORY_SCOPE_AGENT);
                        }
                    }
                };
                asm volatile("s_waitcnt vmcnt(0)" ::: "memory");
                issue(t);
                __syncthreads();
                PM_STAMP(54);
                for (int k0 = t; k0 < tot; k0 += 4 * kLearn) {
                    if (k0 != t) issue(k0);
                    for (int it = 0;; ++it) {
                        bool done = true;
#pragma unroll
                        for (int u = 0; u < 4; ++u) done &= (uint32_t)(g[u] >> 32) == tr_tag;
                        if (done) break;
                        if (it == kPushPollMax) {
                            sm.void_upd = 1;
                            sp.ctrl->status = cs.status | PM_CTRL_PUSH_TIMEOUT;
                            break;
                        }
                        __builtin_amdgcn_s_sleep(1);
#pragma unroll
                        for (int u = 0; u < 4; ++u)
                            if ((uint32_t)(g[u] >> 32) != tr_tag)
                                g[u] = __hip_atomic_load(pg + jf[u], __ATOMIC_RELAXED, __HIP_MEMORY_SCOPE_AGENT);
                    }
#pragma unroll
                    for (int u = 0; u < 4; ++u) {
                        if (k0 + u * kLearn >= tot) break;
                        const int j = jf[u] / kPushGF, f = jf[u] - j * kPushGF;
                        const float v = __uint_as_float((uint32_t)g[u]);
                        if (f < 64) sm.Hs[j][f] = v;
                        else sm.qv4[(f - 64) >> 2][j][f & 3] = v;
                    }
                }
                PM_STAMP_T(36, 0);
            } else {
            if (t == 0 && !push_wait(sp, cs)) sm.void_upd = 1;
            PM_STAMP_T(36, 0);
            asm volatile("s_waitcnt vmcnt(0)" ::: "memory");
            __syncthreads();
            PM_STAMP(54);
            const float* pay = sp.hfeat + (size_t)B * 80;
            for (int k = t; k < np * 76; k += kLearn) {
                const int q = k / 76, f = k - q * 76;
                const int w = q >= pre[3] ? 3 : q >= pre[2] ? 2 : q >= pre[1] ? 1 : 0;
                const int j = sm.plist[w * 64 + q - pre[w]];
                const float v = __hip_atomic_load(pay + (size_t)j * 80 + f, __ATOMIC_RELAXED, __HIP_MEMORY_SCOPE_AGENT);
                if (f < 64) sm.Hs[j][f] = v;
                else sm.qv4[(f - 64) >> 2][j][f & 3] = v;
            }
            }
        }
    }
    float wmax = sm.red[0][0];
    for (int w = 1; w < 16; ++w) wmax = fmaxf(wmax, sm.red[w][0]);
    if (t < PM_MAX_BATCH) asm volatile("s_waitcnt vmcnt(0)" ::: "memory");
    __syncthreads();
    PM_STAMP(2);
    if (sm.void_upd) train = act = false;
    ep_fin = sm.ctot[0];

    float lossp = 0.f, prio = 0.f;
    float cf[4] = {0.f, 0.f, 0.f, 0.f};
    int slot = 0;
    if (act) {
        const float4 v0 = *reinterpret_cast<const float4*>(sm.qv4[0][t]);
        const float4 v1 = *reinterpret_cast<const float4*>(sm.qv4[1][t]);
        const float4 v2 = *reinterpret_cast<const float4*>(sm.qv4[2][t]);
        const float rwd = v0.w;
        const int bits = __float_as_int(v1.w);
        const int a = bits & 0xff, dn = (bits >> 8) & 1;
        const float qs[3] = {v0.x, v0.y, v0.z};
        const float qn[3] = {v1.x, v1.y, v1.z};
        const float qt[3] = {v2.x, v2.y, v2.z};
        const float q = qs[a];
        const float nq = qt[argmax3(qn)];
        const float tgt = rwd + (float)sp.gamma * nq * (dn ? 0.f : 1.f);
        const float diff = q - tgt;
        const float w = wraw / wmax;
        lossp = w * (diff * diff);
        const float g = 2.f * w * diff / (float)B;
        cf[0] = g;
#pragma unroll
        for (int k = 0; k < 3; ++k) cf[1 + k] = g * ((k == a ? 1.f : 0.f) - 1.f / 3.f);
        *reinterpret_cast<float4*>(sm.coef[t]) = make_float4(cf[0], cf[1], cf[2], cf[3]);
        prio = fabsf(diff) + 1e-6f;
        const uint32_t key = (uint32_t)id;
        slot = (int)((key * 2654435761u) >> 23);
        for (;;) {
            const uint32_t old = atomicCAS(&sm.hkey[slot], kHashEmpty, key);
            if (old == kHashEmpty || old == key) break;
            slot = (slot + 1) & 511;
        }
        atomicMax(&sm.hwin[slot], t);
    } else if (sp.fuse_apply && late_noise && t >= kLearn / 2) {
        if (t >= kLearn - 3) {
            const int which = t - (kLearn - 2);
            long long s = 0;
            for (int w = 0; w < 16; ++w) s += sm.cnt[w][0];
            const double base = which < 0 ? sp.epsilon_decay : which ? sp.beta2 : sp.beta1;
            const double ex = which < 0 ? (double)(float)s : (double)(cs.train_steps + 1);
            const double p = pow(base, ex);
            if (which < 0) {
                if (first) sm.ap.eps_next = cs.epsilon * p;
            } else {
                const double bc = 1.0 - p;
                sm.ap.ak[which] = which ? (float)sqrt(bc) : (float)(sp.lr / bc);
            }
        }
        gen_both_noises_on(sp, sm.ap, cs.step + 1, (uint64_t)(cs.train_steps + (train0 ? 1 : 0)) + 1, kLearn / 2);
    }
    {
        const float s = wave_sum(lossp), mp = wave_max(prio);
#pragma unroll
        for (int k = 0; k < 4; ++k) cf[k] = wave_sum(cf[k]);
        if (lane == 0) {
            sm.red[wv][1] = s; sm.red[wv][2] = mp;
#pragma unroll
            for (int k = 0; k < 4; ++k) sm.red[wv][3 + k] = cf[k];
        }
    }
    asm volatile("s_waitcnt vmcnt(0)" ::: "memory");
    __syncthreads();
    PM_STAMP(3);

    float mpx = 0.f;
    if (train) {
        mpx = sm.red[0][2];
        for (int w = 1; w < 16; ++w) mpx = fmaxf(mpx, sm.red[w][2]);
    }
    const float leaf_v = act ? prio_pow(prio, (float)sp.alpha) : 0.f;
    if (tr) {
        if (t < B) tr_publish(sp, t, __float_as_uint(leaf_v), tr_tag);
        if (t == B) tr_publish(sp, B, __float_as_uint(train ? fmaxf(cs.max_prio, mpx) : cs.max_prio), tr_tag);
        if (t == B + 1) tr_publish(sp, B + 1, train ? 1u : 0u, tr_tag);
    }
    if (train) {
        if (act && sm.hwin[slot] == t) {
            sp.prios[id] = prio;
            tree.leaf[id] = leaf_v;
            if (prio != prio) atomicOr(&sp.ctrl->status, PM_CTRL_NAN_PRIO);
        }
        if (t == 0) {
            float l = 0.f;
            for (int w = 0; w < 16; ++w) l += sm.red[w][1];
            sm.loss_out = l / (float)B;
        }
        const int col = t & 63;
        float g[4] = {0.f, 0.f, 0.f, 0.f};
        const int j0 = wv * 16, j1 = min(j0 + 16, B);
        for (int j = j0; j < j1; ++j) {
            const float4 k4 = *reinterpret_cast<const float4*>(sm.coef[j]);
            const float h = sm.Hs[j][col];
            g[0] = fmaf(k4.x, h, g[0]);
            g[1] = fmaf(k4.y, h, g[1]);
            g[2] = fmaf(k4.z, h, g[2]);
            g[3] = fmaf(k4.w, h, g[3]);
        }
#pragma unroll
        for (int r = 0; r < 4; ++r) sm.u.gpart[wv][r * 64 + col] = g[r];
    }
    const float max_prio_next = train ? fmaxf(cs.max_prio, mpx) : cs.max_prio;
    if (!tr) __threadfence_block();
    __syncthreads();
    PM_STAMP(4);

    const PushRange next = last ? push_of(sp, (cs.pos + sp.n) % sp.cap, s_after, max_prio_next)
                                : PushRange{0, 0, sp.cap, 0.f};
    if (train) {
        if (t < 256) {
            float g = 0.f;
#pragma unroll
            for (int w = 0; w < 16; ++w) g += sm.u.gpart[w][t];
            const int row = t >> 6, col = t & 63;
            float* gs = sm.ap.g;
            const int a = row - 1;
            const int kmu = row == 0 ? col : 130 + a * 64 + col, ksg = row == 0 ? 65 + col : 325 + a * 64 + col;
            const float gsg = g * sm.eps_tr[row == 0 ? P_VWEP - PM_QNET_EPS_OFF + col
                                                     : P_AWEP - PM_QNET_EPS_OFF + a * 64 + col];
            gs[kmu] = g;
            gs[ksg] = gsg;
            if (sp.fuse_apply) {
                adam_one(sp, sm.ap, kmu, g);
                adam_one(sp, sm.ap, ksg, gsg);
            }
        } else if (t < 260) {
            const int k = t - 256;
            float g = 0.f;
            for (int w = 0; w < 16; ++w) g += sm.red[w][3 + k];
            float* gs = sm.ap.g;
            const int kmu = k == 0 ? 64 : 322 + k - 1, ksg = k == 0 ? 129 : 517 + k - 1;
            const float gsg = g * sm.eps_tr[k == 0 ? P_VBEP - PM_QNET_EPS_OFF : P_ABEP - PM_QNET_EPS_OFF + k - 1];
            gs[kmu] = g;
            gs[ksg] = gsg;
            if (sp.fuse_apply) {
                adam_one(sp, sm.ap, kmu, g);
                adam_one(sp, sm.ap, ksg, gsg);
            }
        }
        PM_STAMP(8); PM_STAMP_T(9, 960);
        if (!tr) {
            const int j = min(t >> 2, B - 1);
            const int64_t sb = sm.sidx[j] / PER_SUB;
            const double v = per_sub_sum4(tree.leaf, sb, next);
            if ((t & 3) == 0) tree.sub[sb] = v;
        }
        PM_STAMP(10); PM_STAMP_T(11, 960);
    } else {
        for (int k = t; k < kGradN; k += kLearn) sm.ap.g[k] = 0.f;
    }
    if (t == 0) { sm.ap.g[kGradN] = (float)ep_fin; sm.ap.g[kGradN + 1] = train ? 1.f : 0.f; }
    if (!tr) {
        const RingNodes rn = ring_nodes(next, PER_SUB);
        const double csub = per_sub_pushed_sum(next);
        for (int64_t k = t; k < rn.count(); k += kLearn) {
            const int64_t sb = rn.at(k);
            if (per_sub_pushed(sb, next)) tree.sub[sb] = csub;
        }
        PM_STAMP(12); PM_STAMP_T(13, 960);
        if (wv == 0) {
            const int g = lane >> 2;
            const bool ok = g < 4 && (g < 2 ? rn.na : rn.nb) > 0;
            const int64_t sb = !ok ? 0 : g == 0 ? rn.a0 : g == 1 ? rn.a0 + rn.na - 1 : g == 2 ? 0 : rn.nb - 1;
            const double v = per_sub_sum4(tree.leaf, sb, next);
            if (ok && (lane & 3) == 0 && !per_sub_pushed(sb, next)) tree.sub[sb] = v;
        }
    }
    PM_STAMP(14); PM_STAMP_T(15, 960);
    if (!tr) __threadfence_block();
    __syncthreads();
    PM_STAMP(5);
    for (int k = t; k < kGradN + 2; k += kLearn) sp.grad[k] = sm.ap.g[k];
    if (!tr && act && sm.hwin[slot] == t) {
        const int64_t ch = id / PER_CHUNK;
        tree.chunk[ch] = per_chunk_sum(tree, ch);
    }
    if (!tr) {
        const RingNodes rn = ring_nodes(next, PER_CHUNK);
        for (int64_t k = t; k < rn.count(); k += kLearn) {
            const int64_t ch = rn.at(k);
            tree.chunk[ch] = per_chunk_sum(tree, ch);
        }
    }
    PM_STAMP(6);
    if (sp.fuse_apply && first && !waited) {
        if (t == 0) push_wait(sp, cs);
        __syncthreads();
    }
    if (sp.fuse_apply) apply_finish(sp, sm.ap, cs, mode);
    if (t == 0) {
        if (first) {
            c->ep_step = ep_fin;
            c->episodes = cs.episodes + ep_fin;
            c->ep_A = cs.ep_A + sm.ctot[1]; c->win_A = cs.win_A + sm.ctot[2];
            c->ep_P = cs.ep_P + sm.ctot[3]; c->win_P = cs.win_P + sm.ctot[4];
            c->reward_B = cs.reward_B + (double)sm.ctot[5];
        }
        if (train) {
            c->last_loss = sm.loss_out;
            c->max_prio = max_prio_next;
        }
    }
    PM_STAMP(7);
}

__global__ __launch_bounds__(kLearn) void k_adam(const pm_selfplay sp, int mode) {
    __shared__ ApplySmem sm;
    const int t = threadIdx.x;
    const pm_ctrl cs = *sp.ctrl;
    load_apply_inputs(sp, sm, true);
    const float D = sp.grad[kGradN], upd = sp.grad[kGradN + 1];
    const int64_t ts = cs.train_steps + (upd > 0.5f ? 1 : 0);
    gen_both_noises_on(sp, sm, cs.step + 1, (uint64_t)ts + 1, kLearn / 2);
    if (t >= kLearn - 2) adam_const_lane(sp, cs.train_steps + 1, sm, t - (kLearn - 2));
    if (t == kLearn / 2 - 1) sm.eps_next = cs.epsilon * pow(sp.epsilon_decay, (double)D);
    __syncthreads();
    apply_adam(sp, sm);
    __syncthreads();
    apply_finish(sp, sm, cs, mode);
}

__global__ __launch_bounds__(kLearn) void k_prepare(const pm_selfplay sp) {
    __shared__ ApplySmem sm;
    write_feature_frags(sp.paramsB, sp.w_B);
    load_apply_inputs(sp, sm, false);
    gen_both_noises(sp, sm, sp.ctrl->step, (uint64_t)sp.ctrl->train_steps + 1);
    __syncthreads();
    derive_weights(sp, sm);
}

__global__ __launch_bounds__(256) void k_resample(const pm_selfplay sp) {
    __shared__ PerSampleSmem sm;
    sample_block(sp, (int)blockIdx.x, false, sm);
}
__global__ __launch_bounds__(kBlock) void k_batch_fwd(const pm_selfplay sp) { env_fwd_block(sp, (int)blockIdx.x, false); }

constexpr int kMaxBlocks = 512;
__global__ __launch_bounds__(256) void k_prio_max(const pm_selfplay sp) {
    __shared__ float red[4];
    const pm_ctrl* c = sp.ctrl;
    const int64_t s = c->size + sp.n;
    const int64_t size = s < sp.cap ? s : sp.cap;
    const int64_t n4 = size / 4;
    const float4* p4 = reinterpret_cast<const float4*>(sp.prios);
    float m = 0.f;
    for (int64_t k = (int64_t)blockIdx.x * 256 + threadIdx.x; k < n4; k += (int64_t)gridDim.x * 256) {
        const float4 v = p4[k];
        m = fmaxf(m, fmaxf(fmaxf(v.x, v.y), fmaxf(v.z, v.w)));
    }
    if (blockIdx.x == 0 && threadIdx.x < size - 4 * n4) m = fmaxf(m, sp.prios[4 * n4 + threadIdx.x]);
    m = wave_max(m);
    if ((threadIdx.x & 63) == 0) red[threadIdx.x >> 6] = m;
    __syncthreads();
    if (threadIdx.x == 0) {
        m = fmaxf(fmaxf(red[0], red[1]), fmaxf(red[2], red[3]));
        atomicMax(&sp.ctrl->max_bits, __float_as_int(m));
    }
}

__global__ __launch_bounds__(kLearn) void k_commit(const pm_selfplay sp) {
    const int t = threadIdx.x, lane = t & 63, wv = t >> 6;
    pm_ctrl* c = sp.ctrl;
    const pm_ctrl cs = *c;
    const PerTree tree = per_tree(sp.per_work, sp.cap);
    const int64_t s = cs.size + sp.n;
    const int64_t s_after = s < sp.cap ? s : sp.cap;
    const float mp = __int_as_float(cs.max_bits);
    const PushRange next = push_of(sp, (cs.pos + sp.n) % sp.cap, s_after, mp);
    {
        const RingNodes rn = ring_nodes(next, PER_SUB);
        const double csub = per_sub_pushed_sum(next);
        for (int64_t k = t; k < rn.count(); k += kLearn) {
            const int64_t sb = rn.at(k);
            if (per_sub_pushed(sb, next)) tree.sub[sb] = csub;
        }
        if (wv == 0) {
            const int g = lane >> 2;
            const bool ok = g < 4 && (g < 2 ? rn.na : rn.nb) > 0;
            const int64_t sb = !ok ? 0 : g == 0 ? rn.a0 : g == 1 ? rn.a0 + rn.na - 1 : g == 2 ? 0 : rn.nb - 1;
            const double v = per_sub_sum4(tree.leaf, sb, next);
            if (ok && (lane & 3) == 0 && !per_sub_pushed(sb, next)) tree.sub[sb] = v;
        }
    }
    __threadfence_block();
    __syncthreads();
    {
        const RingNodes rn = ring_nodes(next, PER_CHUNK);
        for (int64_t k = t; k < rn.count(); k += kLearn) {
            const int64_t ch = rn.at(k);
            tree.chunk[ch] = per_chunk_sum(tree, ch);
        }
    }
    if (t == 0) {
        c->max_prio = mp;
        c->max_bits = 0;
        c->pos = (cs.pos + sp.n) % sp.cap;
        c->size = s_after;
        c->step = cs.step + 1;
    }
}

constexpr int kMultiChunks = PER_ROUND;

struct MultiSmem {
    float Hs[PM_MAX_BATCH][68];
    float qv[PM_MAX_BATCH][12];
    float coef[PM_MAX_BATCH][4];
    float gpart[16][256];
    float hf[2][264];
    float eps_tr[pad256(260)];
    double chunk[kMultiChunks];
    double incl[kMultiChunks];
    double wsum[16];
    int64_t sidx[PM_MAX_BATCH];
    float sw[PM_MAX_BATCH];
    uint32_t hkey[512];
    int hwin[512];
    float red[16][8];
    double total;
    double pa[PM_MAX_BATCH];
    int64_t ts, frame;
    float maxp, loss;
    ApplySmem ap;
    pm_selfplay sp;
};
static_assert(sizeof(MultiSmem) <= 160 * 1024, "k_learn_multi LDS");

template <typename T>
__device__ __forceinline__ T ld_nt(const T* p) { return __builtin_nontemporal_load(p); }
typedef float f32x4v __attribute__((ext_vector_type(4)));
__device__ __forceinline__ void ld_nt16(const float* p, int64_t lo, int64_t cap, float (&v)[16]) {
    if (lo + 16 <= cap) {
        const f32x4v* p4 = reinterpret_cast<const f32x4v*>(p + lo);
#pragma unroll
        for (int q = 0; q < 4; ++q) {
            const f32x4v x = __builtin_nontemporal_load(p4 + q);
            v[4 * q] = x.x; v[4 * q + 1] = x.y; v[4 * q + 2] = x.z; v[4 * q + 3] = x.w;
        }
    } else {
#pragma unroll
        for (int i = 0; i < 16; ++i) v[i] = lo + i < cap ? ld_nt(p + lo + i) : 0.f;
    }
}

__device__ __forceinline__ double multi_quarter(const float* leaf, int64_t sb, int k, int64_t cap) {
    const int64_t lo = sb * PER_SUB + 16 * k;
    float v[16];
    ld_nt16(leaf, lo, cap, v);
    double acc = 0.0;
#pragma unroll
    for (int i = 0; i < 16; ++i) acc += lo + i < cap ? (double)v[i] : 0.0;
    return acc;
}
__device__ __forceinline__ double multi_sub_sum4(const float* leaf, int64_t sb, int64_t cap) {
    const int lane = threadIdx.x & 63;
    const double q = multi_quarter(leaf, sb, lane & 3, cap);
    return per_combine(quad_f64<0>(q), quad_f64<1>(q), quad_f64<2>(q), quad_f64<3>(q));
}
__device__ __forceinline__ double multi_chunk_sum(const PerTree& t, int64_t c) {
    typedef double f64x2v __attribute__((ext_vector_type(2)));
    double v[PER_FAN];
    if (c * PER_FAN + PER_FAN <= t.nsub) {
        const f64x2v* p = reinterpret_cast<const f64x2v*>(t.sub + c * PER_FAN);
#pragma unroll
        for (int k = 0; k < PER_FAN / 2; ++k) {
            const f64x2v x = __builtin_nontemporal_load(p + k);
            v[2 * k] = x.x;
            v[2 * k + 1] = x.y;
        }
    } else {
#pragma unroll
        for (int k = 0; k < PER_FAN; ++k) v[k] = c * PER_FAN + k < t.nsub ? ld_nt(t.sub + c * PER_FAN + k) : 0.0;
    }
    double acc = 0.0;
#pragma unroll
    for (int k = 0; k < PER_FAN; ++k) acc += v[k];
    return acc;
}

__device__ __forceinline__ void half_chains(const float* hf, int h, const float (&x)[32], float (&s)[4]) {
    float v = 0.f, a0 = 0.f, a1 = 0.f, a2 = 0.f;
    const float4* hw = reinterpret_cast<const float4*>(hf + h * 128);
#pragma unroll
    for (int k = 0; k < 32; ++k) {
        const float4 w = hw[k];
        v = fmaf(w.x, x[k], v);
        a0 = fmaf(w.y, x[k], a0);
        a1 = fmaf(w.z, x[k], a1);
        a2 = fmaf(w.w, x[k], a2);
    }
    s[0] = v; s[1] = a0; s[2] = a1; s[3] = a2;
}
__device__ __forceinline__ void half_chains2(const float* hf, int h, const float (&xa)[32], const float (&xb)[32],
                                             float (&sa)[4], float (&sb)[4]) {
    float v = 0.f, a0 = 0.f, a1 = 0.f, a2 = 0.f, u = 0.f, b0 = 0.f, b1 = 0.f, b2 = 0.f;
    const float4* hw = reinterpret_cast<const float4*>(hf + h * 128);
#pragma unroll
    for (int k = 0; k < 32; ++k) {
        const float4 w = hw[k];
        v = fmaf(w.x, xa[k], v);
        a0 = fmaf(w.y, xa[k], a0);
        a1 = fmaf(w.z, xa[k], a1);
        a2 = fmaf(w.w, xa[k], a2);
        u = fmaf(w.x, xb[k], u);
        b0 = fmaf(w.y, xb[k], b0);
        b1 = fmaf(w.z, xb[k], b1);
        b2 = fmaf(w.w, xb[k], b2);
    }
    sa[0] = v; sa[1] = a0; sa[2] = a1; sa[3] = a2;
    sb[0] = u; sb[1] = b0; sb[2] = b1; sb[3] = b2;
}
__device__ __forceinline__ void half_heads_finish(const float* hf, const float (&s)[4], float (&q)[3]) {
    float v = s[0] + __shfl_xor(s[0], 1), a0 = s[1] + __shfl_xor(s[1], 1);
    float a1 = s[2] + __shfl_xor(s[2], 1), a2 = s[3] + __shfl_xor(s[3], 1);
    v += hf[256];
    a0 += hf[257];
    a1 += hf[258];
    a2 += hf[259];
    const float mean = ((a0 + a1) + a2) / 3.0f;
    q[0] = v + (a0 - mean);
    q[1] = v + (a1 - mean);
    q[2] = v + (a2 - mean);
}

__device__ __forceinline__ void load_frow_half(const float* frow, int64_t slot, int h, float (&x)[32]) {
    const float4* p = reinterpret_cast<const float4*>(frow + slot * 64) + h;
#pragma unroll
    for (int k = 0; k < 8; ++k) {
        const float4 v = p[2 * k];
        x[4 * k] = v.x; x[4 * k + 1] = v.y; x[4 * k + 2] = v.z; x[4 * k + 3] = v.w;
    }
}
__device__ __forceinline__ void load_featB_half(const float* featB, int a, int h, float (&x)[32]) {
    const float4* p = reinterpret_cast<const float4*>(featB) + (size_t)(a >> 5) * 8 * 64 + 32 * h + (a & 31);
#pragma unroll
    for (int k = 0; k < 8; ++k) {
        const float4 v = p[k * 64];
        x[4 * k] = relu(v.x); x[4 * k + 1] = relu(v.y); x[4 * k + 2] = relu(v.z); x[4 * k + 3] = relu(v.w);
    }
}

__device__ __forceinline__ int group_find16f(const float (&f)[16], int64_t lo, int64_t size, double x, double& before,
                                             double& val) {
    const int lane = threadIdx.x & 63, q = lane & 3, g0 = lane & ~3;
    auto lv = [&](int e) { return lo + e < size ? (double)f[e] : 0.0; };
    double acc = 0.0;
#pragma unroll
    for (int e = 0; e < 16; ++e) acc += lv(e);
    const double s0 = quad_f64<0>(acc), s1 = quad_f64<1>(acc), s2 = quad_f64<2>(acc);
    const double ex = q == 0 ? 0.0 : (q == 1 ? s0 : (q == 2 ? s0 + s1 : (s0 + s1) + s2));
    int hit = -1, nz = -1;
    double hb = 0.0, hv = 0.0, nb = 0.0, nv = 0.0, run = ex;
#pragma unroll
    for (int e = 0; e < 16; ++e) {
        const double v = lv(e);
        if (hit < 0 && run + v > x) { hit = e; hb = run; hv = v; }
        if (v > 0.0) { nz = e; nb = run; nv = v; }
        run += v;
    }
    const unsigned gh = (unsigned)(__ballot(hit >= 0) >> g0) & 15u;
    const unsigned gn = (unsigned)(__ballot(nz >= 0) >> g0) & 15u;
    int src, k;
    if (gh) {
        src = __ffs(gh) - 1;
        k = hit;
    } else {
        src = gn ? 31 - __clz(gn) : 0;
        k = nz < 0 ? 0 : nz;
        hb = nz < 0 ? ex : nb;
        hv = nz < 0 ? 0.0 : nv;
    }
    const int kk = quad_sel_i32(k, src);
    before = quad_sel_f64(hb, src);
    val = quad_sel_f64(hv, src);
    return src * 16 + kk;
}

__device__ __forceinline__ void noise_to_eps(const float* noise, float* eps) {
    const int k = threadIdx.x;
    if (k >= 260) return;
    const int row = k < 256 ? k >> 6 : k - 256, col = k & 63;
    const bool w = k < 256;
    float ep;
    int eo;
    if (row == 0) {
        ep = w ? noise[64] * noise[col] : noise[64];
        eo = w ? E_VWEP + col : E_VBEP;
    } else {
        const int a = row - 1;
        ep = w ? noise[129 + a] * noise[65 + col] : noise[129 + a];
        eo = w ? E_AWEP + a * 64 + col : E_ABEP + a;
    }
    eps[eo] = ep;
}

#ifndef PM_MULTI_INLINE
#define PM_MULTI_INLINE __noinline__
#endif
__device__ PM_MULTI_INLINE void multi_update(const pm_selfplay& sp, MultiSmem& sm, int64_t size, int64_t nb, int64_t c_pos,
                                          uint64_t c_step, bool final, bool early_pow) {
    const int t = threadIdx.x, lane = t & 63, wv = t >> 6, B = sp.batch;
    const PerTree tree = per_tree(sp.per_work, sp.cap);
    PM_STAMP(100);
    const int64_t ts = sm.ts, frame = sm.frame + 1;
    for (int k = t; k < 512; k += kLearn) { sm.hkey[k] = kHashEmpty; sm.hwin[k] = -1; }
    PM_STAMP(119);
    {
        double run[4] = {0.0, 0.0, 0.0, 0.0}, acc = 0.0, incl = 0.0;
        if (t < 256) {
#pragma unroll
            for (int e = 0; e < 4; ++e) {
                const int64_t ch = 4 * t + e;
                acc += ch < nb ? sm.chunk[ch] : 0.0;
                run[e] = acc;
            }
        }
        PM_STAMP(120);
        incl = wave_incl_scan(acc, lane);
        double excl = __shfl_up(incl, 1);
        if (lane == 0) excl = 0.0;
        if (lane == 63) sm.wsum[wv] = incl;
        PM_STAMP(121);
        __syncthreads();
        PM_STAMP(122);
        if (t < 256) {
            double wb = 0.0;
            for (int w = 0; w < wv; ++w) wb += sm.wsum[w];
            const double ex = wb + excl;
#pragma unroll
            for (int e = 0; e < 4; ++e) sm.incl[4 * t + e] = ex + run[e];
        }
        if (t == 0) sm.total = ((0.0 + sm.wsum[0]) + sm.wsum[1]) + sm.wsum[2] + sm.wsum[3];
        __syncthreads();
    }
    PM_STAMP(101);
    const double total = sm.total;
    {
        const int j = t >> 2, q = t & 3;
        const int n = (int)nb;
        double x = 0.0, before = 0.0;
        int64_t blk = 0;
        {
            const U4 r = philox64((uint32_t)j, TAG_PER, (uint64_t)frame, sp.seed_env);
            const double uu = j < B ? u53(r.x, r.y) : 0.0;
            x = uu * total;
            if (total > 0.0) {
                int lo = 0, hi = n;
                while (lo < hi) {
                    const int mid = (lo + hi) >> 1;
                    if (sm.incl[mid] > x) hi = mid;
                    else lo = mid + 1;
                }
                if (lo < n) {
                    blk = lo;
                    before = lo ? sm.incl[lo - 1] : 0.0;
                } else {
                    int l2 = 0, h2 = n - 1;
                    while (l2 < h2) {
                        const int mid = (l2 + h2) >> 1;
                        if (sm.incl[mid] >= sm.incl[n - 1]) h2 = mid;
                        else l2 = mid + 1;
                    }
                    blk = l2;
                    before = l2 ? sm.incl[l2 - 1] : 0.0;
                }
            }
        }
        PM_STAMP(111);
        double sv[4];
        const int64_t s0 = blk * PER_FAN + 4 * q;
#pragma unroll
        for (int e = 0; e < 4; ++e) sv[e] = s0 + e < tree.nsub ? ld_nt(tree.sub + s0 + e) : 0.0;
        double b1, v1;
        const int64_t sb = blk * PER_FAN + per_group_find<4>(sv, x - before, b1, v1);
        PM_STAMP(112);
        float lf[16];
        const int64_t lo = sb * PER_SUB + 16 * q;
        ld_nt16(tree.leaf, lo, sp.cap, lf);
        double b0, pa;
        const int k = group_find16f(lf, lo, size, x - before - b1, b0, pa);
        PM_STAMP(113);
        const int64_t id = sb * PER_SUB + k;
        const int h = q & 1, set = q >> 1;
        float xs[32], xn[32];
        float rb[2] = {0.f, 0.f};
        {
            int64_t a = id - c_pos;
            if (a < 0) a += sp.cap;
            if (a < sp.n) {
                load_featB_half(sp.featB, (int)a, h, xn);
            } else {
                int64_t nx = id + sp.n;
                if (nx >= sp.cap) nx -= sp.cap;
                load_frow_half(sp.frow, nx, h, xn);
            }
        }
        if (set == 0) {
            load_frow_half(sp.frow, id, h, xs);
            if (h) {
                const float* tr = sp.trans + id * PM_TRANS_F;
                rb[0] = tr[7];
                rb[1] = tr[15];
            }
        } else {
#pragma unroll
            for (int e = 0; e < 32; ++e) xs[e] = xn[e];
        }
        float wr = 0.f;
        if (early_pow && q == 0 && j < B) wr = (float)pow((double)size * (pa / total), -beta_of(sp, frame));
#ifdef PM_DIAG
        asm volatile("s_waitcnt vmcnt(0)" ::: "memory");
        PM_STAMP(117);
#endif
        const float* hfs = sm.hf[set];
        float s1[4], s2[4], q1[3], q2[3];
        half_chains2(hfs, h, xs, xn, s1, s2);
        half_heads_finish(hfs, s1, q1);
        half_heads_finish(hfs, s2, q2);
        PM_STAMP(118);
        if (j < B) {
            if (set == 0) {
#pragma unroll
                for (int e = 0; e < 32; e += 4)
                    *reinterpret_cast<float4*>(&sm.Hs[j][32 * (e >> 4) + 8 * ((e >> 2) & 3) + 4 * h]) =
                        make_float4(xs[e], xs[e + 1], xs[e + 2], xs[e + 3]);
                if (h == 0) {
                    sm.qv[j][0] = q1[0]; sm.qv[j][1] = q1[1]; sm.qv[j][2] = q1[2];
                    sm.qv[j][4] = q2[0]; sm.qv[j][5] = q2[1]; sm.qv[j][6] = q2[2];
                    sm.sidx[j] = id;
                    sm.pa[j] = pa;
                    sm.sw[j] = wr;
                    if (final) sp.idx[j] = id;
                } else {
                    sm.qv[j][3] = rb[0];
                    sm.qv[j][7] = rb[1];
                }
            } else if (h == 0) {
                sm.qv[j][8] = q1[0]; sm.qv[j][9] = q1[1]; sm.qv[j][10] = q1[2];
            }
        }
        if (early_pow) {
            const float m = wave_max(wr);
            if (lane == 0) sm.red[wv][0] = m;
        }
    }
    __syncthreads();
    PM_STAMP(102);
    const bool act = t < B;
    float wraw;
    if (early_pow) {
        wraw = act ? sm.sw[t] : 0.f;
    } else {
        wraw = act ? (float)pow((double)size * (sm.pa[t] / total), -beta_of(sp, frame)) : 0.f;
        const float m = wave_max(wraw);
        if (lane == 0) sm.red[wv][0] = m;
        __syncthreads();
    }
    if (act && final) sp.isw[t] = wraw;
    const int64_t id = act ? sm.sidx[t] : 0;
    PM_STAMP(103);
    float wmax = sm.red[0][0];
    for (int w = 1; w < 16; ++w) wmax = fmaxf(wmax, sm.red[w][0]);
    PM_STAMP(104);
    float lossp = 0.f, prio = 0.f;
    float cf[4] = {0.f, 0.f, 0.f, 0.f};
    int slot = 0;
    if (act) {
        const float rwd = sm.qv[t][3];
        const int bits = __float_as_int(sm.qv[t][7]);
        const int a = bits & 0xff, dn = (bits >> 8) & 1;
        const float qs[3] = {sm.qv[t][0], sm.qv[t][1], sm.qv[t][2]};
        const float qn[3] = {sm.qv[t][4], sm.qv[t][5], sm.qv[t][6]};
        const float qt[3] = {sm.qv[t][8], sm.qv[t][9], sm.qv[t][10]};
        const float q = qs[a];
        const float nq = qt[argmax3(qn)];
        const float tgt = rwd + (float)sp.gamma * nq * (dn ? 0.f : 1.f);
        const float diff = q - tgt;
        const float w = wraw / wmax;
        lossp = w * (diff * diff);
        const float g = 2.f * w * diff / (float)B;
        cf[0] = g;
#pragma unroll
        for (int k = 0; k < 3; ++k) cf[1 + k] = g * ((k == a ? 1.f : 0.f) - 1.f / 3.f);
        *reinterpret_cast<float4*>(sm.coef[t]) = make_float4(cf[0], cf[1], cf[2], cf[3]);
        prio = fabsf(diff) + 1e-6f;
        const uint32_t key = (uint32_t)id;
        slot = (int)((key * 2654435761u) >> 23);
        for (;;) {
            const uint32_t old = atomicCAS(&sm.hkey[slot], kHashEmpty, key);
            if (old == kHashEmpty || old == key) break;
            slot = (slot + 1) & 511;
        }
        atomicMax(&sm.hwin[slot], t);
    } else if (t >= kLearn / 2) {
        if (t >= kLearn - 2) adam_const_lane(sp, ts + 1, sm.ap, t - (kLearn - 2));
        gen_both_noises_on(sp, sm.ap, c_step + 1, (uint64_t)(ts + 1) + 1, kLearn / 2);
    }
    {
        const float s = wave_sum(lossp), mp = wave_max(prio);
#pragma unroll
        for (int k = 0; k < 4; ++k) cf[k] = wave_sum(cf[k]);
        if (lane == 0) {
            sm.red[wv][1] = s; sm.red[wv][2] = mp;
#pragma unroll
            for (int k = 0; k < 4; ++k) sm.red[wv][3 + k] = cf[k];
        }
    }
    __syncthreads();
    PM_STAMP(105);
    if (act && sm.hwin[slot] == t) {
        sp.prios[id] = prio;
        tree.leaf[id] = prio_pow(prio, (float)sp.alpha);
        if (prio != prio) atomicOr(&sp.ctrl->status, PM_CTRL_NAN_PRIO);
    }
    {
        float mpx = sm.red[0][2];
        for (int w = 1; w < 16; ++w) mpx = fmaxf(mpx, sm.red[w][2]);
        float l = 0.f;
        for (int w = 0; w < 16; ++w) l += sm.red[w][1];
        if (t == 0) {
            sm.loss = l / (float)B;
            sm.maxp = fmaxf(sm.maxp, mpx);
        }
        const int col = t & 63;
        float g[4] = {0.f, 0.f, 0.f, 0.f};
        const int j0 = wv * 16, j1 = min(j0 + 16, B);
        for (int j = j0; j < j1; ++j) {
            const float4 k4 = *reinterpret_cast<const float4*>(sm.coef[j]);
            const float h = sm.Hs[j][col];
            g[0] = fmaf(k4.x, h, g[0]);
            g[1] = fmaf(k4.y, h, g[1]);
            g[2] = fmaf(k4.z, h, g[2]);
            g[3] = fmaf(k4.w, h, g[3]);
        }
#pragma unroll
        for (int r = 0; r < 4; ++r) sm.gpart[wv][r * 64 + col] = g[r];
    }
    asm volatile("s_waitcnt vmcnt(0)" ::: "memory");
    __syncthreads();
    PM_STAMP(106);
    if (t < 256) {
        float g = 0.f;
#pragma unroll
        for (int w = 0; w < 16; ++w) g += sm.gpart[w][t];
        const int row = t >> 6, col = t & 63;
        float* gs = sm.ap.g;
        const int a = row - 1;
        const int kmu = row == 0 ? col : 130 + a * 64 + col, ksg = row == 0 ? 65 + col : 325 + a * 64 + col;
        const float gsg = g * sm.eps_tr[row == 0 ? P_VWEP - PM_QNET_EPS_OFF + col
                                                 : P_AWEP - PM_QNET_EPS_OFF + a * 64 + col];
        gs[kmu] = g;
        gs[ksg] = gsg;
        adam_one(sp, sm.ap, kmu, g, final);
        adam_one(sp, sm.ap, ksg, gsg, final);
    } else if (t < 260) {
        const int k = t - 256;
        float g = 0.f;
        for (int w = 0; w < 16; ++w) g += sm.red[w][3 + k];
        float* gs = sm.ap.g;
        const int kmu = k == 0 ? 64 : 322 + k - 1, ksg = k == 0 ? 129 : 517 + k - 1;
        const float gsg = g * sm.eps_tr[k == 0 ? P_VBEP - PM_QNET_EPS_OFF : P_ABEP - PM_QNET_EPS_OFF + k - 1];
        gs[kmu] = g;
        gs[ksg] = gsg;
        adam_one(sp, sm.ap, kmu, g, final);
        adam_one(sp, sm.ap, ksg, gsg, final);
    }
    PM_STAMP(115);
    {
        const int j = min(t >> 2, B - 1);
        const int64_t sb = sm.sidx[j] / PER_SUB;
        const double v = multi_sub_sum4(tree.leaf, sb, sp.cap);
        PM_STAMP(116);
        if ((t & 3) == 0) tree.sub[sb] = v;
    }
    if (t == 0) { sm.ap.g[kGradN] = 0.f; sm.ap.g[kGradN + 1] = 1.f; }
    asm volatile("s_waitcnt vmcnt(0)" ::: "memory");
    __syncthreads();
    PM_STAMP(107);
    if (final)
        for (int k = t; k < kGradN + 2; k += kLearn) sp.grad[k] = sm.ap.g[k];
    if (act && sm.hwin[slot] == t) {
        const int64_t ch = id / PER_CHUNK;
        const double v = multi_chunk_sum(tree, ch);
        tree.chunk[ch] = v;
        sm.chunk[ch] = v;
    }
    if (t == 0) { sm.ts = ts + 1; sm.frame = frame; }
    if ((ts + 1) % sp.target_update_interval == 0) {
        for (int k = t; k < PM_QNET_NHEAD; k += kLearn) sm.ap.tmu[k] = sm.ap.hp[k];
        for (int k = t; k < PM_QNET_NP; k += kLearn) {
            const int h = k - PM_QNET_HEAD_OFF, e = k - PM_QNET_EPS_OFF;
            sp.paramsT[k] = (h >= 0 && h < PM_QNET_NHEAD) ? sm.ap.hp[h]
                            : (e >= 0 ? sm.eps_tr[e] : sp.paramsB[k]);
        }
        __syncthreads();
    }
    PM_STAMP(108);
    if (final) {
        derive_weights(sp, sm.ap);
        __syncthreads();
    } else {
        derive_weights_lds(sm.ap);
    }
    PM_STAMP(109);
    heads_to_frags(sm.ap.heads[1], sm.hf[0]);
    heads_to_frags(sm.ap.heads[2], sm.hf[1]);
    noise_to_eps(sm.ap.ntrain, sm.eps_tr);
    __syncthreads();
    PM_STAMP(124);
}

__global__ __launch_bounds__(kLearn, 1) void k_learn_multi(const pm_selfplay sp, int updates, int mflags) {
    __shared__ __attribute__((aligned(16))) MultiSmem sm;
    const int t = threadIdx.x, B = sp.batch;
    const PerTree tree = per_tree(sp.per_work, sp.cap);
    pm_ctrl* c = sp.ctrl;
    const int64_t c_pos = c->pos, c_size = c->size;
    const uint64_t c_step = c->step;
    const int64_t s_all = c_size + sp.n;
    const int64_t size = s_all < sp.cap ? s_all : sp.cap;
    if (size < B) return;
    const int64_t nb = (size + PER_CHUNK - 1) / PER_CHUNK;
    for (int k = t; k < kMultiChunks; k += kLearn) sm.chunk[k] = k < tree.nchunk ? ld_nt(tree.chunk + k) : 0.0;
    for (int k = t; k < 2 * 264; k += kLearn) sm.hf[k / 264][k % 264] = sp.learn_heads[k];
    for (int k = t; k < 260; k += kLearn) sm.eps_tr[k] = sp.learn_heads[528 + k];
    load_apply_inputs(sp, sm.ap, false);
    if (t == 0) {
        sm.ts = c->train_steps;
        sm.frame = c->frame_idx;
        sm.maxp = c->max_prio;
        sm.loss = c->last_loss;
    }
    for (int k = t; k < (int)(sizeof(pm_selfplay) / 4); k += kLearn)
        reinterpret_cast<uint32_t*>(&sm.sp)[k] = reinterpret_cast<const uint32_t*>(&sp)[k];
    __syncthreads();

    for (int u = 1; u < updates; ++u) multi_update(sm.sp, sm, size, nb, c_pos, c_step, u == updates - 1, mflags & 1);
    if (t == 0) {
        c->train_steps = sm.ts;
        c->frame_idx = sm.frame;
        c->last_loss = sm.loss;
        c->max_prio = sm.maxp;
    }
}

namespace {
int check(const pm_selfplay* sp) {
    PM_REQUIRE(sp && sp->ctrl && sp->trans && sp->prios && sp->per_work && sp->idx && sp->isw && sp->grad &&
                   sp->partials && sp->hfeat && sp->w_opp && sp->paramsB && sp->paramsT && sp->w_B && sp->adam_m &&
                   sp->adam_v && sp->opp && sp->ep_reward,
               PM_E_ARG, "pm_selfplay: null buffer");
    PM_REQUIRE(sp->n > 0 && sp->batch >= 1 && sp->batch <= PM_MAX_BATCH && sp->n > sp->batch && sp->cap >= sp->n &&
                   sp->cap < 0xFFFFFFFFll,
               PM_E_SIZE, "pm_selfplay: n=%d batch=%d cap=%lld", sp->n, sp->batch, (long long)sp->cap);
    PM_REQUIRE(sp->n_pool >= 0 && sp->n_pool <= 4096 && sp->world >= 1, PM_E_SIZE, "pm_selfplay: n_pool/world");
    PM_REQUIRE(sp->obsA && sp->obsB && sp->aA && sp->aB && sp->learn_heads && sp->opp_list && sp->opp_cnt, PM_E_ARG,
               "pm_selfplay: null buffer");
    PM_REQUIRE(!sp->fuse_apply || sp->world == 1, PM_E_ARG, "pm_selfplay: fuse_apply needs world == 1");
    PM_REQUIRE(sp->chunk_A > 0 && sp->chunk_A <= kListMax && sp->chunk_P > 0 && sp->chunk_P <= kListMax, PM_E_SIZE,
               "pm_selfplay: chunk_A/chunk_P must be in [1, %d]", kListMax);
    PM_REQUIRE(((((uintptr_t)sp->w_opp) | ((uintptr_t)sp->w_B) | ((uintptr_t)sp->prios) | ((uintptr_t)sp->per_work) |
                 ((uintptr_t)sp->paramsB) | ((uintptr_t)sp->paramsT) | ((uintptr_t)sp->adam_m) | ((uintptr_t)sp->adam_v) |
                 ((uintptr_t)sp->learn_heads)) &
                15) == 0,
               PM_E_ARG, "pm_selfplay: w_opp / w_B / prios / per_work / paramsB / paramsT / adam_m / adam_v / "
                         "learn_heads must be 16-byte aligned");
    PM_REQUIRE(sp->env.speed_scale_every > 0 && sp->target_update_interval > 0 && sp->beta_frames > 0, PM_E_ARG,
               "pm_selfplay: zero interval");
    return PM_OK;
}
}

extern "C" int pm_selfplay_prepare(const pm_selfplay* sp, void* stream) {
    int rc = check(sp);
    if (rc) return rc;
    hipStream_t st = pm_stream(stream);
    hipLaunchKernelGGL(k_prepare, dim3(1), dim3(kLearn), 0, st, *sp);
    PM_LAUNCHED("k_prepare");
    return per_launch_build(sp->prios, sp->cap, (float)sp->alpha, sp->ctrl, sp->n, sp->per_work, st);
}

namespace {
__global__ void k_tree_repaired(pm_ctrl* c) {
    if (threadIdx.x == 0 && (c->status & PM_CTRL_TREE_TIMEOUT))
        c->status = (c->status & ~PM_CTRL_TREE_TIMEOUT) | PM_CTRL_TREE_REPAIRED;
}
}

extern "C" int pm_selfplay_repair_tree(const pm_selfplay* sp, void* stream) {
    int rc = check(sp);
    if (rc) return rc;
    hipStream_t st = pm_stream(stream);
    if ((rc = per_launch_build(sp->prios, sp->cap, (float)sp->alpha, sp->ctrl, sp->n, sp->per_work, st))) return rc;
    hipLaunchKernelGGL(k_tree_repaired, dim3(1), dim3(64), 0, st, sp->ctrl);
    PM_LAUNCHED("k_tree_repaired");
    return PM_OK;
}

extern "C" int pm_selfplay_init(const pm_selfplay* sp, void* stream) {
    int rc = check(sp);
    if (rc) return rc;
    hipStream_t st = pm_stream(stream);
    hipLaunchKernelGGL(k_sp_init, dim3(pm_blocks(sp->n, kBlock)), dim3(kBlock), 0, st, *sp);
    PM_LAUNCHED("k_sp_init");
    return pm_selfplay_prepare(sp, stream);
}

namespace {
int launch_act(const pm_selfplay* sp, int part, hipStream_t st) {
    const ActGrid g{sp->n, sp->n_pool + 1, sp->chunk_A, sp->chunk_P, part == PM_ACT_A ? 0 : 1};
    const int nsb = part == PM_ACT_A ? 0 : (sp->batch + PER_BS - 1) / PER_BS;
    int blocks = part == PM_ACT_B ? nsb + g.nb() : nsb + g.blocks();
    if (part != PM_ACT_B && sp->featB) blocks += (feat_ntiles(sp->n) + kFeatTilesAct - 1) / kFeatTilesAct;
    hipLaunchKernelGGL(k_act_sp, dim3(blocks), dim3(kActBlock), 0, st, *sp, part);
    PM_LAUNCHED("k_act_sp");
    return PM_OK;
}

bool multi_ok(const pm_selfplay* sp) {
    return sp->frow && sp->frow_ready && sp->featB && sp->fuse_apply && sp->world == 1 &&
           (sp->cap + PER_CHUNK - 1) / PER_CHUNK <= kMultiChunks && ((uintptr_t)sp->frow & 15) == 0;
}

struct LearnGrid {
    ActGrid g;
    int ftiles;
};
constexpr int kSideRows = 480;
int side_sleep() {
    const char* e = getenv("PONGMI_SIDE_SLEEP");
    const char* n = getenv("PONGMI_SIDE_NAP");
    const int roles = e && *e ? atoi(e) : 2, nap = n && *n ? atoi(n) : 8;
    return (roles & 3) | (std::max(0, std::min(nap, 64)) << 8);
}
int device_cus() {
    static const int v = [] {
        int dev = 0, cus = 0;
        if (hipGetDevice(&dev) != hipSuccess ||
            hipDeviceGetAttribute(&cus, hipDeviceAttributeMultiprocessorCount, dev) != hipSuccess || cus <= 0)
            cus = 256;
        return cus;
    }();
    return v;
}
int side_chunk(double p) {
    if (!(p > 0.0)) return kListMaxLearn;
    const double c = std::ceil(kSideRows / p / 256.0) * 256.0;
    return c >= kListMaxLearn ? kListMaxLearn : (c < 256.0 ? 256 : (int)c);
}
LearnGrid learn_grid(const pm_selfplay* sp) {
    const int ntiles = feat_ntiles(sp->n);
    const double pp = sp->n_pool > 0 ? sp->pool_ratio : 0.0;
    const ActGrid g{sp->n, sp->n_pool + 1, side_chunk(1.0 - pp), side_chunk(sp->n_pool > 0 ? pp / sp->n_pool : 0.0), 0};
    const int left = device_cus() - 2 - g.blocks();
    const int slots = left >= 32 ? left : device_cus();
    int ft = (ntiles + slots - 1) / slots;
    ft = std::max(ft, kFeatTilesLearn);
    return LearnGrid{g, std::min(ft, std::max(ntiles, 1))};
}

int tree_refresh_block() {
    const int v = [] {
        const char* e = getenv("PONGMI_TR");
        const char* p = getenv("PONGMI_PUSH2");
        const char* q = getenv("PONGMI_LATE_NOISE");
        const char* g = getenv("PONGMI_PUSHG");
        const int tr = e && *e ? (atoi(e) != 0) : 1, p2 = p && *p ? (atoi(p) != 0) : 1;
        const int pg = (g && *g ? (atoi(g) != 0) : 1) && tr && p2;
        const char* f = getenv("PONGMI_TR_FORCE_TIMEOUT");
        return tr | (p2 << 1) | ((q && *q ? (atoi(q) != 0) : 1) << 2) | (pg << 3) | ((f && *f && atoi(f) != 0) << 4);
    }();
    return v;
}

int launch_learn(const pm_selfplay* sp, bool with_act, hipStream_t st, int mode = PM_UPD_FIRST | PM_UPD_LAST) {
    const LearnGrid lg = learn_grid(sp);
    const ActGrid& g = lg.g;
    unsigned blocks = 2u + (with_act ? (unsigned)g.blocks() : 0u);
    if (with_act && sp->featB) blocks += (unsigned)((feat_ntiles(sp->n) + lg.ftiles - 1) / lg.ftiles);
    const int tr = tree_refresh_block();
    pm_launch(PM_TIMER_LEARN, (tr & 8) ? k_learn<true> : k_learn<false>, dim3(blocks), dim3(kLearn), st, *sp, g.chunk0,
              g.chunk1, mode, tr, lg.ftiles, side_sleep());
    PM_LAUNCHED("k_learn");
    return PM_OK;
}
}

extern "C" int pm_selfplay_act(const pm_selfplay* sp, void* stream) {
    return pm_selfplay_act_part(sp, PM_ACT_ALL, stream);
}

extern "C" int pm_selfplay_act_part(const pm_selfplay* sp, int32_t part, void* stream) {
    int rc = check(sp);
    if (rc) return rc;
    PM_REQUIRE(part == PM_ACT_ALL || part == PM_ACT_B || part == PM_ACT_A, PM_E_ARG,
               "pm_selfplay_act_part: part=%d", part);
    return launch_act(sp, part, pm_stream(stream));
}

extern "C" int pm_selfplay_env(const pm_selfplay* sp, void* stream) {
    int rc = check(sp);
    if (rc) return rc;
    const unsigned nfwd = pm_blocks(2 * sp->batch, 128);
    hipLaunchKernelGGL(k_env, dim3(pm_blocks(sp->n, kBlock) + nfwd), dim3(kBlock), 0, pm_stream(stream), *sp);
    PM_LAUNCHED("k_env");
    return PM_OK;
}

extern "C" int pm_selfplay_actenv(const pm_selfplay* sp, void* stream) {
    int rc = check(sp);
    if (rc) return rc;
    const unsigned nsb = pm_blocks(sp->batch, 32);
    pm_launch(PM_TIMER_ACTENV, k_actenv, dim3(nsb + pm_blocks(sp->n, kBlock)), dim3(kBlock), pm_stream(stream), *sp);
    PM_LAUNCHED("k_actenv");
    return PM_OK;
}

extern "C" int pm_selfplay_rollout(const pm_selfplay* sp, void* stream) {
    int rc = pm_selfplay_act(sp, stream);
    return rc ? rc : pm_selfplay_env(sp, stream);
}

extern "C" int pm_selfplay_learn(const pm_selfplay* sp, void* stream) {
    int rc = check(sp);
    return rc ? rc : launch_learn(sp, false, pm_stream(stream));
}

extern "C" int pm_selfplay_learn_act(const pm_selfplay* sp, void* stream) {
    int rc = check(sp);
    return rc ? rc : launch_learn(sp, true, pm_stream(stream));
}

extern "C" int pm_selfplay_apply(const pm_selfplay* sp, void* stream) {
    return pm_selfplay_apply_ex(sp, PM_UPD_FIRST | PM_UPD_LAST, stream);
}

extern "C" int pm_selfplay_apply_ex(const pm_selfplay* sp, int32_t mode, void* stream) {
    int rc = check(sp);
    if (rc) return rc;
    PM_REQUIRE(mode >= 0 && mode <= (PM_UPD_FIRST | PM_UPD_LAST), PM_E_ARG, "pm_selfplay_apply_ex: mode=%d", mode);
    if (sp->fuse_apply) return PM_OK;
    hipLaunchKernelGGL(k_adam, dim3(1), dim3(kLearn), 0, pm_stream(stream), *sp, (int)mode);
    PM_LAUNCHED("k_adam");
    return PM_OK;
}

extern "C" int pm_selfplay_learn_ex(const pm_selfplay* sp, int32_t mode, int32_t with_act, void* stream) {
    int rc = check(sp);
    if (rc) return rc;
    PM_REQUIRE(mode >= 0 && mode <= (PM_UPD_FIRST | PM_UPD_LAST), PM_E_ARG, "pm_selfplay_learn_ex: mode=%d", mode);
    return launch_learn(sp, with_act != 0, pm_stream(stream), (int)mode);
}

extern "C" int pm_selfplay_resample(const pm_selfplay* sp, void* stream) {
    int rc = check(sp);
    if (rc) return rc;
    hipStream_t st = pm_stream(stream);
    hipLaunchKernelGGL(k_resample, dim3((sp->batch + PER_BS - 1) / PER_BS), dim3(256), 0, st, *sp);
    PM_LAUNCHED("k_resample");
    hipLaunchKernelGGL(k_batch_fwd, dim3(pm_blocks(2 * sp->batch, 128)), dim3(kBlock), 0, st, *sp);
    PM_LAUNCHED("k_batch_fwd");
    return PM_OK;
}

extern "C" int pm_selfplay_commit(const pm_selfplay* sp, void* stream) {
    int rc = check(sp);
    if (rc) return rc;
    hipStream_t st = pm_stream(stream);
    const int64_t blocks = std::min<int64_t>(kMaxBlocks, std::max<int64_t>(1, (sp->cap + 4095) / 4096));
    hipLaunchKernelGGL(k_prio_max, dim3((unsigned)blocks), dim3(256), 0, st, *sp);
    PM_LAUNCHED("k_prio_max");
    hipLaunchKernelGGL(k_commit, dim3(1), dim3(kLearn), 0, st, *sp);
    PM_LAUNCHED("k_commit");
    return PM_OK;
}

extern "C" int pm_selfplay_step_multi(const pm_selfplay* sp, int32_t updates, void* stream) {
    int rc = check(sp);
    if (rc) return rc;
    PM_REQUIRE(updates >= 1, PM_E_ARG, "pm_selfplay_step_multi: updates=%d", updates);
    PM_REQUIRE(sp->world == 1, PM_E_ARG, "pm_selfplay_step_multi: unsharded only (world=%d)", sp->world);
    if (updates == 1) return pm_selfplay_step_overlap(sp, stream);
    hipStream_t st = pm_stream(stream);
    if ((rc = pm_selfplay_actenv(sp, stream))) return rc;
    if ((rc = launch_learn(sp, true, st, PM_UPD_FIRST))) return rc;
    if ((rc = pm_selfplay_apply_ex(sp, PM_UPD_FIRST, stream))) return rc;
    if (multi_ok(sp)) {
        const char* ep = getenv("PONGMI_MULTI_EARLYPOW");
        const int mflags = ep && *ep ? (atoi(ep) != 0) : 0;
        pm_launch(PM_TIMER_LEARN_MULTI, k_learn_multi, dim3(1), dim3(kLearn), st, *sp, (int)updates, mflags);
        PM_LAUNCHED("k_learn_multi");
        return pm_selfplay_commit(sp, stream);
    }
    for (int u = 1; u < updates; ++u) {
        if ((rc = pm_selfplay_resample(sp, stream))) return rc;
        if ((rc = launch_learn(sp, false, st, 0))) return rc;
        if ((rc = pm_selfplay_apply_ex(sp, 0, stream))) return rc;
    }
    return pm_selfplay_commit(sp, stream);
}

extern "C" int pm_selfplay_step(const pm_selfplay* sp, void* stream) {
    int rc = pm_selfplay_rollout(sp, stream);
    if (!rc) rc = pm_selfplay_learn(sp, stream);
    return rc ? rc : pm_selfplay_apply(sp, stream);
}

extern "C" int pm_selfplay_step_overlap(const pm_selfplay* sp, void* stream) {
    int rc = pm_selfplay_actenv(sp, stream);
    if (!rc) rc = pm_selfplay_learn_act(sp, stream);
    return rc ? rc : pm_selfplay_apply(sp, stream);
}

#ifdef PM_DIAG
extern "C" int pm_diag_read_side(uint64_t* out) {
    return (int)hipMemcpyFromSymbol(out, HIP_SYMBOL(pm_diag_side), sizeof(uint64_t) * 4 * 1024);
}
extern "C" int pm_diag_read(uint64_t* out, int32_t n) {
    hipError_t e = hipMemcpyFromSymbol(out, HIP_SYMBOL(pm_diag_buf), sizeof(uint64_t) * (n < 256 ? n : 256));
    return e == hipSuccess ? 0 : (int)e;
}
extern "C" int pm_diag_read_blk(uint64_t* out) {
    return (int)hipMemcpyFromSymbol(out, HIP_SYMBOL(pm_diag_blk), sizeof(uint64_t) * 8 * 4096);
}
extern "C" int pm_diag_read_env(uint64_t* out) {
    return (int)hipMemcpyFromSymbol(out, HIP_SYMBOL(pm_diag_env), sizeof(uint64_t) * 8 * 1024);
}
extern "C" int pm_diag_clear(void) {
    static const unsigned long long z[256] = {0};
    return (int)hipMemcpyToSymbol(HIP_SYMBOL(pm_diag_buf), z, sizeof(z));
}
#endif
```

### pingpong-selfplay-ai_amd/pongmi/_lib.py

```python
import ctypes
import os

import numpy as np

import torch

HERE = os.path.dirname(os.path.abspath(__file__))
LIB_PATH = os.environ.get("PONGMI_LIB", os.path.join(HERE, "libpongmi.so"))

c_double, c_float = ctypes.c_double, ctypes.c_float
c_i32, c_i64, c_u64 = ctypes.c_int32, ctypes.c_int64, ctypes.c_uint64
c_void_p = ctypes.c_void_p

PM_QNET_NP = 5452
PM_QNET_NHEAD = 520
PM_QNET_HEAD_OFF = 4672
PM_QNET_EPS_OFF = 5192
PM_QNET_NW = 9944
PM_GRAD_EPISODES, PM_GRAD_UPDATED, PM_GRAD_LEN = 520, 521, 528
PM_QNET_PLAIN = 4936
PM_RNN_NP = 192012
PM_RNN_NPARAM = 174984
PM_RNN_NW = 157456
PM_TRANS_F = 16
PM_MAX_BATCH = 256
PM_FOLD_EVAL, PM_FOLD_TRAIN, PM_FOLD_TRAIN_FRESH = 0, 1, 2
PM_ACT_ALL, PM_ACT_B, PM_ACT_A = 0, 1, 2
PM_UPD_FIRST, PM_UPD_LAST = 1, 2
PM_COMM_ID_BYTES = 128
ABI_VERSION = 25
PM_TIMER_ACTENV, PM_TIMER_LEARN, PM_TIMER_RNN_ACT, PM_TIMER_ENV_STEP, PM_TIMER_ROLLOUT, PM_TIMER_DRQN = 0, 1, 2, 3, 4, 5
PM_TIMER_LEARN_MULTI, PM_TIMER_N = 6, 7
PM_ROLL_HEADS = 264


class EnvParams(ctypes.Structure):
    _fields_ = [(n, c_double) for n in (
        "paddle_width", "paddle_speed", "magnus_factor", "restitution", "friction", "ball_mass", "radius",
        "speed_lo", "speed_hi", "spin_lo", "spin_hi", "ang0_lo", "ang0_hi", "ang1_lo", "ang1_hi",
        "half_width", "speed_scale", "inertia", "jt_coef", "inv_mass", "inv_inertia")] + \
        [("max_score", c_i32), ("speed_scale_every", c_i32), ("enable_spin", c_i32), ("_pad", c_i32)]


class EnvState(ctypes.Structure):
    _fields_ = [(n, c_void_p) for n in ("x", "y", "vx", "vy", "spin", "top", "bot",
                                        "scoreA", "scoreB", "bounces", "serves")]


class Ctrl(ctypes.Structure):
    _fields_ = [("step", c_u64), ("pos", c_i64), ("size", c_i64), ("train_steps", c_i64), ("frame_idx", c_i64),
                ("episodes", c_i64), ("epsilon", c_double), ("max_prio", c_float), ("last_loss", c_float),
                ("ep_step", c_i64), ("win_A", c_i64), ("ep_A", c_i64), ("win_P", c_i64), ("ep_P", c_i64),
                ("reward_B", c_double), ("status", c_i32), ("max_bits", c_i32)]


class SelfPlay(ctypes.Structure):
    _fields_ = [("env", EnvParams), ("st", EnvState)] + \
        [(n, c_void_p) for n in ("opp", "ep_reward", "w_opp", "paramsB", "paramsT", "w_B", "adam_m", "adam_v",
                                 "trans", "prios", "per_work", "idx", "isw", "grad", "partials", "obsA", "obsB", "aA",
                                 "aB", "hfeat", "learn_heads", "ctrl", "opp_list", "opp_cnt")] + \
        [("n", c_i32), ("n_pool", c_i32), ("batch", c_i32), ("world", c_i32), ("chunk_A", c_i32), ("chunk_P", c_i32),
         ("fuse_apply", c_i32), ("_pad0", c_i32), ("cap", c_i64)] + \
        [(n, c_double) for n in ("gamma", "alpha", "lr", "beta1", "beta2", "adam_eps", "min_epsilon", "epsilon_decay",
                                 "pool_ratio", "beta_start")] + \
        [("beta_frames", c_i64), ("target_update_interval", c_i64), ("seed_env", c_u64), ("seed_net", c_u64),
         ("featB", c_void_p), ("frow", c_void_p), ("frow_ready", c_i32), ("_pad1", c_i32)]


class RollReplay(ctypes.Structure):
    _fields_ = [(n, c_void_p) for n in ("trans", "prios", "per_work", "ep_reward")] + \
        [("pos", c_i64), ("cap", c_i64), ("prio", c_float), ("alpha", c_float)]


class DrqnStats(ctypes.Structure):
    _fields_ = [("steps", c_i64), ("adam_t", c_i64), ("loss", c_float), ("norm", c_float), ("q_mean", c_float),
                ("status", c_i32)]


class Drqn(ctypes.Structure):
    _fields_ = [(n, c_void_p) for n in ("params", "target", "adam_m", "adam_v", "grad", "work", "stats", "obs", "next",
                                        "act", "rew", "done", "enable")] + \
        [("batch", c_i32), ("T", c_i32), ("target_update_interval", c_i64)] + \
        [(n, c_double) for n in ("gamma", "lr", "beta1", "beta2", "adam_eps", "max_norm")] + \
        [("poll_limit", c_i32), ("reserved", c_i32)]


class RnnCtrl(ctypes.Structure):
    _fields_ = [("step", c_u64), ("episodes", c_i64), ("seq_count", c_i64), ("seq_size", c_i64), ("epsilon", c_double),
                ("win_A", c_i64), ("ep_A", c_i64), ("win_P", c_i64), ("ep_P", c_i64), ("reward_B", c_double),
                ("status", c_i32), ("train", c_i32)]


class RnnSelfPlay(ctypes.Structure):
    _fields_ = [("env", EnvParams), ("st", EnvState)] + \
        [(n, c_void_p) for n in ("opp", "ep_reward", "ep_len", "ep_steps", "reset", "w_opp", "paramsB", "w_B", "hA",
                                 "cA", "hB", "cB", "obsA", "obsB", "aA", "aB", "trans", "seq_eps", "seq_mark", "fin",
                                 "partials", "opp_list", "opp_cnt", "enable", "ctrl")] + \
        [(n, c_i32) for n in ("n", "n_pool", "depth", "T", "chunk_A", "chunk_P", "max_steps", "_pad")] + \
        [("seq_cap", c_i64), ("min_episodes", c_i64)] + \
        [(n, c_double) for n in ("min_epsilon", "epsilon_decay", "pool_ratio")] + \
        [("seed_env", c_u64), ("seed_net", c_u64), ("hA_in", c_void_p), ("cA_in", c_void_p), ("qA", c_void_p),
         ("qB", c_void_p)]


CTRL_DTYPE_BYTES = ctypes.sizeof(Ctrl)

_SIGS = {
    "pm_env_reset": (c_i32, [c_void_p, c_void_p, c_void_p, c_void_p, c_i32, c_u64, c_void_p, c_void_p, c_void_p, c_i32,
                             c_void_p]),
    "pm_env_step": (c_i32, [c_void_p, c_void_p, c_void_p, c_void_p, c_void_p, c_void_p, c_void_p, c_void_p, c_void_p,
                            c_void_p, c_void_p, c_i32, c_void_p, c_i32, c_u64, c_u64, c_void_p, c_i32, c_void_p]),
    "pm_collide": (c_i32, [c_void_p, c_void_p, c_void_p, c_i32, c_void_p]),
    "pm_env_step1": (c_i32, [c_void_p, c_void_p, c_i32, c_i32, c_void_p, ctypes.c_uint32, c_void_p]),
    "pm_env_reset1": (c_i32, [c_void_p, c_double, c_double, c_double, c_void_p, ctypes.c_uint32, c_void_p]),
    "pm_collide1": (c_i32, [c_void_p, c_double, c_void_p, ctypes.c_uint32, c_void_p]),
    "pm_host_mapped_alloc": (c_void_p, [ctypes.c_int64, ctypes.POINTER(c_void_p)]),
    "pm_host_mapped_free": (c_i32, [c_void_p]),
    "pm_qnet_fold": (c_i32, [c_void_p, c_void_p, c_i32, c_u64, c_u64, c_void_p, c_void_p, c_i32, c_void_p]),
    "pm_qnet_q": (c_i32, [c_void_p, c_void_p, c_void_p, c_i32, c_void_p]),
    "pm_qnet_act": (c_i32, [c_void_p, c_void_p, c_i32, c_void_p, c_void_p, c_void_p, c_float, c_void_p, c_u64, c_u64,
                            c_void_p, c_void_p, c_void_p, c_void_p, c_void_p, c_i32, c_i32, c_i32, c_void_p]),
    "pm_rnn_fold": (c_i32, [c_void_p, c_void_p, c_i32, c_u64, c_u64, c_void_p, c_void_p, c_i32, c_void_p]),
    "pm_rnn_q": (c_i32, [c_void_p, c_void_p, c_void_p, c_void_p, c_void_p, c_void_p, c_i32, c_void_p]),
    "pm_rnn_act": (c_i32, [c_void_p, c_void_p, c_i32, c_void_p, c_void_p, c_void_p, c_void_p, c_void_p, c_void_p,
                           c_void_p, c_void_p, c_float, c_void_p, c_u64, c_u64, c_void_p, c_void_p, c_void_p, c_void_p,
                           c_void_p, c_i32, c_i32, c_i32, c_void_p, c_void_p, c_void_p]),
    "pm_play": (c_i32, [c_void_p, c_void_p, c_i32, c_void_p, c_void_p, c_i32, c_void_p, c_void_p, c_i32, c_i32,
                        c_void_p, c_void_p, c_void_p, c_void_p, c_void_p, c_void_p]),
    "pm_play_rnn": (c_i32, [c_void_p, c_void_p, c_i32, c_void_p, c_i32, c_void_p, c_void_p, c_i32, c_void_p, c_void_p,
                            c_i32, c_i32, c_void_p, c_void_p, c_void_p, c_void_p, c_void_p, c_void_p, c_void_p]),
    "pm_play_rnn_scratch_bytes": (ctypes.c_size_t, [c_i32]),
    "pm_play_rec": (c_i32, [c_void_p, c_void_p, c_i32, c_void_p, c_void_p, c_i32, c_void_p, c_void_p, c_i32, c_i32,
                            c_void_p, c_void_p, c_void_p, c_void_p, c_void_p, c_void_p, c_i32, c_i32, c_void_p, c_void_p,
                            c_void_p, c_void_p]),
    "pm_play_rnn_rec": (c_i32, [c_void_p, c_void_p, c_i32, c_void_p, c_i32, c_void_p, c_void_p, c_i32, c_void_p,
                                c_void_p, c_i32, c_i32, c_void_p, c_void_p, c_void_p, c_void_p, c_void_p, c_void_p,
                                c_void_p, c_i32, c_i32, c_void_p, c_void_p, c_void_p, c_void_p]),
    "pm_rollout": (c_i32, [c_void_p, c_void_p, c_void_p, c_void_p, c_void_p, c_float, c_u64, c_u64, c_u64, c_i32,
                           c_void_p, c_void_p, c_void_p, c_void_p, c_i32, c_void_p]),
    "pm_per_build": (c_i32, [c_void_p, c_i64, c_float, c_void_p, c_void_p]),
    "pm_rollout_push": (c_i32, [c_void_p, c_void_p, c_void_p, c_void_p, c_void_p, c_float, c_u64, c_u64, c_u64,
                                c_i32, c_void_p, c_void_p, c_void_p, c_void_p, c_void_p, c_i32, c_void_p]),
    "pm_drqn_work_bytes": (c_i64, [c_i32, c_i32]),
    "pm_drqn_init": (c_i32, [c_void_p, c_void_p]),
    "pm_drqn_grads": (c_i32, [c_void_p, c_void_p]),
    "pm_drqn_apply": (c_i32, [c_void_p, c_void_p]),
    "pm_drqn_update": (c_i32, [c_void_p, c_void_p]),
    "pm_rnn_selfplay_init": (c_i32, [c_void_p, c_void_p]),
    "pm_rnn_selfplay_act": (c_i32, [c_void_p, c_void_p]),
    "pm_rnn_selfplay_env": (c_i32, [c_void_p, c_void_p, c_void_p]),
    "pm_rnn_selfplay_rollout": (c_i32, [c_void_p, c_void_p, c_void_p]),
    "pm_rnn_selfplay_step": (c_i32, [c_void_p, c_void_p, c_void_p]),
    "pm_rnn_selfplay_sample": (c_i32, [c_void_p, c_void_p, c_i32, c_void_p]),
    "pm_rnn_selfplay_step_multi": (c_i32, [c_void_p, c_void_p, c_i32, c_void_p]),
    "pm_per_work_bytes": (c_i64, [c_i64]),
    "pm_per_sample": (c_i32, [c_void_p, c_i64, c_float, c_float, c_void_p, c_u64, c_u64, c_void_p, c_void_p, c_i32,
                              c_void_p, c_void_p]),
    "pm_per_update": (c_i32, [c_void_p, c_void_p, c_void_p, c_i32, c_void_p]),
    "pm_selfplay_init": (c_i32, [c_void_p, c_void_p]),
    "pm_selfplay_prepare": (c_i32, [c_void_p, c_void_p]),
    "pm_selfplay_repair_tree": (c_i32, [c_void_p, c_void_p]),
    "pm_selfplay_rollout": (c_i32, [c_void_p, c_void_p]),
    "pm_selfplay_act": (c_i32, [c_void_p, c_void_p]),
    "pm_selfplay_env": (c_i32, [c_void_p, c_void_p]),
    "pm_selfplay_learn": (c_i32, [c_void_p, c_void_p]),
    "pm_selfplay_apply": (c_i32, [c_void_p, c_void_p]),
    "pm_selfplay_step": (c_i32, [c_void_p, c_void_p]),
    "pm_selfplay_act_part": (c_i32, [c_void_p, c_i32, c_void_p]),
    "pm_selfplay_learn_act": (c_i32, [c_void_p, c_void_p]),
    "pm_selfplay_actenv": (c_i32, [c_void_p, c_void_p]),
    "pm_selfplay_step_overlap": (c_i32, [c_void_p, c_void_p]),
    "pm_selfplay_learn_ex": (c_i32, [c_void_p, c_i32, c_i32, c_void_p]),
    "pm_selfplay_apply_ex": (c_i32, [c_void_p, c_i32, c_void_p]),
    "pm_selfplay_resample": (c_i32, [c_void_p, c_void_p]),
    "pm_selfplay_commit": (c_i32, [c_void_p, c_void_p]),
    "pm_selfplay_step_multi": (c_i32, [c_void_p, c_i32, c_void_p]),
    "pm_rnn_selfplay_act_part": (c_i32, [c_void_p, c_i32, c_void_p]),
    "pm_rnn_selfplay_step_overlap": (c_i32, [c_void_p, c_void_p, c_i32, c_void_p, c_void_p]),
    "pm_rnn_selfplay_finish_overlap": (c_i32, [c_void_p, c_void_p, c_i32, c_void_p, c_void_p]),
    "pm_comm_unique_id": (c_i32, [ctypes.c_char_p, c_void_p]),
    "pm_comm_init": (c_i32, [ctypes.c_char_p, c_void_p, c_i32, c_i32, ctypes.POINTER(c_void_p)]),
    "pm_comm_allreduce_f32": (c_i32, [c_void_p, c_void_p, c_i64, c_void_p]),
    "pm_comm_destroy": (c_i32, [c_void_p]),
    "pm_comm_info": (c_i32, [c_void_p, c_void_p, c_void_p, c_void_p]),
    "pm_selfplay_step_sharded": (c_i32, [c_void_p, c_void_p, c_i32, c_void_p]),
    "pm_rnn_selfplay_step_sharded": (c_i32, [c_void_p, c_void_p, c_void_p, c_i32, c_void_p]),
    "pm_rnn_selfplay_step_sharded_overlap": (c_i32, [c_void_p, c_void_p, c_void_p, c_i32, c_void_p, c_void_p]),
    "pm_timer_arm": (c_i32, [c_i32]),
    "pm_timer_read": (c_i32, [c_i32, ctypes.POINTER(c_float)]),
    "pm_last_error": (ctypes.c_char_p, []),
    "pm_abi_version": (c_i32, []),
    "pm_sizeof": (c_i32, [c_i32]),
}
EXPORTED = tuple(_SIGS)

_lib = None


class PongmiError(RuntimeError):
    pass


def load():
    global _lib
    if _lib is not None:
        return _lib
    if not os.path.exists(LIB_PATH):
        raise PongmiError(f"libpongmi.so not found at {LIB_PATH}: run `python -c 'import __graft_entry__ as g; "
                          f"g.build()'` (or `make -C pingpong-selfplay-ai_amd/csrc`) first")
    L = ctypes.CDLL(LIB_PATH)
    for name, (res, args) in _SIGS.items():
        f = getattr(L, name)
        f.restype = res
        f.argtypes = args
    if L.pm_abi_version() != ABI_VERSION:
        raise PongmiError(f"libpongmi ABI {L.pm_abi_version()} != {ABI_VERSION}")
    for which, cls in ((0, EnvParams), (1, EnvState), (2, Ctrl), (3, SelfPlay), (4, Drqn), (5, DrqnStats), (6, RnnCtrl),
                       (7, RnnSelfPlay)):
        if L.pm_sizeof(which) != ctypes.sizeof(cls):
            raise PongmiError(f"struct layout mismatch for {cls.__name__}: C {L.pm_sizeof(which)} "
                              f"vs ctypes {ctypes.sizeof(cls)}")
    _lib = L
    return L


def timer_arm(kernel):
    check(load().pm_timer_arm(int(kernel)), "pm_timer_arm")


def timer_read(kernel):
    ms = c_float()
    check(load().pm_timer_read(int(kernel), ctypes.byref(ms)), "pm_timer_read")
    return ms.value * 1e-3


class MappedSlot:

    def __init__(self, nwords, seq_word):
        self.lib = load()
        dev = c_void_p()
        self.host = self.lib.pm_host_mapped_alloc(4 * int(nwords), ctypes.byref(dev))
        if not self.host:
            raise PongmiError("pm_host_mapped_alloc failed")
        self.dev = dev.value
        self.words = (ctypes.c_uint32 * int(nwords)).from_address(self.host)
        self.f32 = np.ctypeslib.as_array((ctypes.c_float * int(nwords)).from_address(self.host))
        self.f64 = np.ctypeslib.as_array((ctypes.c_double * (int(nwords) // 2)).from_address(self.host))
        self.seq_word = int(seq_word)
        self.seq = 0

    def next_seq(self):
        self.seq = (self.seq + 1) & 0xFFFFFFFF or 1
        return self.seq

    def wait(self, timeout=5.0):
        w, k, want = self.words, self.seq_word, self.seq
        for _ in range(2000):
            if w[k] == want:
                return
        import time
        t0 = time.perf_counter()
        while w[k] != want:
            if time.perf_counter() - t0 > timeout:
                import torch
                torch.cuda.synchronize()
                if w[k] != want:
                    raise PongmiError("scalar drop-in: the device never published its result")
                return

    def floats(self, lo, hi):
        return self.f32[lo:hi].copy()

    def doubles(self, lo, hi):
        return self.f64[lo:hi].copy()

    def __del__(self):
        try:
            if self.host:
                self.lib.pm_host_mapped_free(self.host)
                self.host = None
        except Exception:
            pass


def check(rc, what=""):
    if rc != 0:
        msg = load().pm_last_error().decode(errors="replace")
        raise PongmiError(f"{what or 'libpongmi'} failed (rc={rc}): {msg}")


def ptr(t):
    if t is None:
        return None
    return t.data_ptr()


def stream_ptr(stream=None):
    s = stream if stream is not None else torch.cuda.current_stream()
    return s.cuda_stream


def current_stream():
    return torch.cuda.current_stream()


def require_device(t, name):
    if not t.is_cuda:
        raise PongmiError(f"{name} must be a ROCm device tensor (libpongmi has no CPU path)")
    if not t.is_contiguous():
        raise PongmiError(f"{name} must be contiguous")
```

### pingpong-selfplay-ai_amd/pongmi/selfplay.py

```python
import ctypes

import numpy as np
import torch

from . import _lib, checkpoint
from ._lib import (PM_GRAD_EPISODES, PM_GRAD_LEN, PM_GRAD_UPDATED, PM_QNET_NHEAD, PM_QNET_NP, PM_QNET_NW,
                   PM_TRANS_F, check, ptr, stream_ptr)
from .dist import shard_seeds, splitmix64
from .env import env_config, env_params
from .qnet import HEAD_KEYS, fold, pack_state_dict, unpack_state_dict


def act_chunk(p, rows=96, cap=4096, lo=256):
    if p <= 0:
        return cap
    c = lo
    while c < cap and c * p < rows:
        c *= 2
    return c


def sharded_vector_step(L, allreduce, updates):
    if L.overlap:
        if not L._aA_ready:
            L.act(_lib.PM_ACT_A)
        L.actenv()
    else:
        L.rollout()
    for u in range(updates):
        mode = (_lib.PM_UPD_FIRST | (_lib.PM_UPD_LAST if updates == 1 else 0)) if u == 0 else 0
        if u:
            L.resample()
        L.learn_ex(mode, act_next=L.overlap and u == 0)
        if allreduce is not None:
            allreduce(L.grad)
        L.apply_ex(mode)
    if updates > 1:
        L.commit()


class SelfPlayLearner:
    def __init__(self, env_kw, n_arenas, modelB_state, modelA_state=None, pool_states=(), *, batch=256,
                 memory_size=1_000_000, gamma=0.99, lr=2.5e-4, epsilon=0.02, min_epsilon=0.02, epsilon_decay=0.995,
                 target_update_interval=1000, pool_ratio=0.33, alpha=0.6, beta_start=0.4, beta_frames=100000,
                 episode=0, seed=0, rank=0, world=1, allreduce=None, device=None, modelA_noisy=True,
                 fuse_apply=True, overlap=True, updates_per_step=1, features_ahead=True, learn_multi=True):
        self.lib = _lib.load()
        self.updates_per_step = int(updates_per_step)
        if self.updates_per_step < 1:
            raise ValueError("updates_per_step must be >= 1")
        self.overlap = bool(overlap)
        self._aA_ready = False
        self.device = torch.device(device if device is not None else "cuda")
        if self.device.type != "cuda":
            raise _lib.PongmiError("SelfPlayLearner runs on a ROCm device only")
        self.n, self.batch, self.cap = int(n_arenas), int(batch), int(memory_size)
        self.world, self.rank = int(world), int(rank)
        if self.world > 1 and allreduce is None:
            raise ValueError("world > 1 needs an allreduce(tensor) callable (torch.distributed.all_reduce)")
        self.allreduce = allreduce
        self.env_cfg = env_config(**env_kw)
        dev, n = self.device, self.n
        f32 = dict(dtype=torch.float32, device=dev)

        self.f64 = torch.zeros((7, n), dtype=torch.float64, device=dev)
        self.i32 = torch.zeros((4, n), dtype=torch.int32, device=dev)
        self.opp = torch.zeros(n, dtype=torch.int32, device=dev)
        self.opp_list = torch.zeros(n, dtype=torch.int32, device=dev)
        self.opp_cnt = torch.zeros(((n + 255) // 256) * (len(pool_states) + 1), dtype=torch.int32, device=dev)
        self.ep_reward = torch.zeros(n, **f32)
        self.paramsB = pack_state_dict(modelB_state, dev)
        self.paramsT = self.paramsB.clone()
        self.adam_m = torch.zeros(PM_QNET_NHEAD, **f32)
        self.adam_v = torch.zeros(PM_QNET_NHEAD, **f32)
        self.w_B = torch.zeros(PM_QNET_NW, **f32)
        self.n_pool = len(pool_states)
        self.w_opp = torch.zeros((1 + self.n_pool, PM_QNET_NW), **f32)
        self.modelA_noisy = modelA_noisy
        self.set_modelA(modelA_state if modelA_state is not None else modelB_state)
        if self.n_pool:
            pool = torch.stack([pack_state_dict(s, dev) for s in pool_states])
            self.w_opp[1:] = fold(pool, _lib.PM_FOLD_EVAL)
        self.trans = torch.zeros((self.cap, PM_TRANS_F), **f32)
        self.prios = torch.zeros(self.cap, **f32)
        self.per_work = torch.zeros(max(self.lib.pm_per_work_bytes(self.cap), 256), dtype=torch.uint8, device=dev)
        self.idx = torch.zeros(self.batch, dtype=torch.int64, device=dev)
        self.isw = torch.zeros(self.batch, **f32)
        self.grad = torch.zeros(PM_GRAD_LEN, **f32)
        self.partials = torch.zeros(((n + 255) // 256) * 8, dtype=torch.int64, device=dev)
        self.hfeat = torch.zeros((4 * self.batch + 8, 80), **f32)
        self.learn_heads = torch.zeros(3 * 264, **f32)
        self.obsA = torch.zeros((n, 7), **f32)
        self.obsB = torch.zeros((n, 7), **f32)
        self.aA = torch.zeros(n, dtype=torch.int8, device=dev)
        self.aB = torch.zeros(n, dtype=torch.int8, device=dev)
        self.featB = torch.zeros(((n + 31) // 32) * 2048, **f32) if features_ahead else None
        use_frow = learn_multi and self.updates_per_step > 1 and features_ahead and self.overlap and world == 1
        self.frow = torch.zeros((self.cap, 64), **f32) if use_frow else None
        self._frow_wait = 0
        c = _lib.Ctrl()
        c.epsilon = float(epsilon)
        c.max_prio = 1.0
        c.episodes = int(episode)
        self.ctrl = torch.frombuffer(bytearray(bytes(c)), dtype=torch.uint8).to(dev)

        self.seed = int(seed)
        sp = _lib.SelfPlay()
        sp.env = env_params(**env_kw)
        sp.st = _lib.EnvState(*[ptr(self.f64[k]) for k in range(7)], *[ptr(self.i32[k]) for k in range(4)])
        for name in ("opp", "ep_reward", "w_opp", "paramsB", "paramsT", "w_B", "adam_m", "adam_v", "trans", "prios",
                     "per_work", "idx", "isw", "grad", "partials", "obsA", "obsB", "aA", "aB", "hfeat", "learn_heads",
                     "ctrl", "opp_list", "opp_cnt"):
            setattr(sp, name, ptr(getattr(self, name)))
        sp.featB = ptr(self.featB)
        sp.frow = ptr(self.frow)
        sp.frow_ready = int(self.frow is not None)
        sp.n, sp.n_pool, sp.batch, sp.world, sp.cap = n, self.n_pool, self.batch, self.world, self.cap
        sp.fuse_apply = int(bool(fuse_apply) and self.world == 1)
        p_pool = pool_ratio if self.n_pool else 0.0
        sp.chunk_A = act_chunk(1.0 - p_pool)
        sp.chunk_P = act_chunk(p_pool / self.n_pool) if self.n_pool else 256
        sp.gamma, sp.alpha, sp.lr = gamma, alpha, lr
        sp.beta1, sp.beta2, sp.adam_eps = 0.9, 0.999, 1e-8
        sp.min_epsilon, sp.epsilon_decay, sp.pool_ratio, sp.beta_start = min_epsilon, epsilon_decay, pool_ratio, beta_start
        sp.beta_frames, sp.target_update_interval = int(beta_frames), int(target_update_interval)
        sp.seed_env, sp.seed_net = shard_seeds(self.seed, self.rank)
        self.sp = sp
        self.hparams = dict(gamma=gamma, lr=lr, min_epsilon=min_epsilon, epsilon_decay=epsilon_decay,
                            target_update_interval=target_update_interval, pool_ratio=pool_ratio, alpha=alpha,
                            beta_start=beta_start, beta_frames=beta_frames)
        check(self.lib.pm_selfplay_init(ctypes.byref(sp), stream_ptr()), "pm_selfplay_init")

    def _frow_pushed(self, through_actenv):
        if self.frow is None:
            return
        if through_actenv:
            self._frow_wait = max(0, self._frow_wait - 1)
        else:
            self._frow_wait = -(-self.cap // self.n) + 1
        self.sp.frow_ready = int(self._frow_wait == 0)

    def rollout(self):
        self._aA_ready = False
        self._frow_pushed(False)
        check(self.lib.pm_selfplay_rollout(ctypes.byref(self.sp), stream_ptr()), "pm_selfplay_rollout")

    def act(self, part=_lib.PM_ACT_ALL):
        check(self.lib.pm_selfplay_act_part(ctypes.byref(self.sp), int(part), stream_ptr()), "pm_selfplay_act_part")
        if part != _lib.PM_ACT_B:
            self._aA_ready = True

    def actenv(self):
        self._aA_ready = False
        self._frow_pushed(True)
        check(self.lib.pm_selfplay_actenv(ctypes.byref(self.sp), stream_ptr()), "pm_selfplay_actenv")

    def env_step(self):
        self._aA_ready = False
        self._frow_pushed(False)
        check(self.lib.pm_selfplay_env(ctypes.byref(self.sp), stream_ptr()), "pm_selfplay_env")

    def learn(self, act_next=False):
        if act_next:
            check(self.lib.pm_selfplay_learn_act(ctypes.byref(self.sp), stream_ptr()), "pm_selfplay_learn_act")
            self._aA_ready = True
        else:
            check(self.lib.pm_selfplay_learn(ctypes.byref(self.sp), stream_ptr()), "pm_selfplay_learn")

    def apply(self):
        check(self.lib.pm_selfplay_apply(ctypes.byref(self.sp), stream_ptr()), "pm_selfplay_apply")

    def learn_ex(self, mode, act_next=False):
        check(self.lib.pm_selfplay_learn_ex(ctypes.byref(self.sp), int(mode), int(bool(act_next)), stream_ptr()),
              "pm_selfplay_learn_ex")
        if act_next:
            self._aA_ready = True

    def apply_ex(self, mode):
        check(self.lib.pm_selfplay_apply_ex(ctypes.byref(self.sp), int(mode), stream_ptr()), "pm_selfplay_apply_ex")

    def resample(self):
        check(self.lib.pm_selfplay_resample(ctypes.byref(self.sp), stream_ptr()), "pm_selfplay_resample")

    def commit(self):
        check(self.lib.pm_selfplay_commit(ctypes.byref(self.sp), stream_ptr()), "pm_selfplay_commit")

    def _step_sharded(self, comm):
        self._frow_pushed(True)
        if not self._aA_ready:
            self.act(_lib.PM_ACT_A)
        check(self.lib.pm_selfplay_step_sharded(ctypes.byref(self.sp), comm, self.updates_per_step, stream_ptr()),
              "pm_selfplay_step_sharded")
        self._aA_ready = True

    def _step_multi(self):
        U = self.updates_per_step
        if self.world == 1 and self.overlap:
            if not self._aA_ready:
                self.act(_lib.PM_ACT_A)
            self._frow_pushed(True)
            check(self.lib.pm_selfplay_step_multi(ctypes.byref(self.sp), U, stream_ptr()), "pm_selfplay_step_multi")
            self._aA_ready = True
            return
        sharded_vector_step(self, self.allreduce if self.world > 1 else None, U)

    def step(self):
        comm = getattr(self.allreduce, "pm_comm", None)
        if comm is not None and self.overlap and not self.sp.fuse_apply:
            self._step_sharded(comm)
            return
        if self.updates_per_step > 1:
            self._step_multi()
            return
        if self.world > 1:
            sharded_vector_step(self, self.allreduce, 1)
            return
        if not self.overlap:
            self._frow_pushed(False)
            check(self.lib.pm_selfplay_step(ctypes.byref(self.sp), stream_ptr()), "pm_selfplay_step")
            return
        if not self._aA_ready:
            self.act(_lib.PM_ACT_A)
        self._frow_pushed(True)
        check(self.lib.pm_selfplay_step_overlap(ctypes.byref(self.sp), stream_ptr()), "pm_selfplay_step_overlap")
        self._aA_ready = True

    def counters(self):
        c = _lib.Ctrl.from_buffer_copy(bytes(self.ctrl.cpu().numpy().tobytes()))
        return {k: getattr(c, k) for k, _ in _lib.Ctrl._fields_ if not k.startswith("_")}

    def check_status(self, c=None):
        st = int((c or self.counters())["status"]) & 7
        if st:
            raise _lib.PongmiError(f"self-play learner: device status {st} (bit 0: push-row hand-off timed out; "
                                   f"bit 1: NaN priority scattered; bit 2: tree refresh timed out)")

    def repair_tree(self, c=None):
        if not int((c or self.counters())["status"]) & 4:
            return False
        check(self.lib.pm_selfplay_repair_tree(ctypes.byref(self.sp), stream_ptr()), "pm_selfplay_repair_tree")
        return True

    def set_epsilon(self, eps):
        c = _lib.Ctrl.from_buffer_copy(bytes(self.ctrl.cpu().numpy().tobytes()))
        c.epsilon = float(eps)
        self.ctrl.copy_(torch.frombuffer(bytearray(bytes(c)), dtype=torch.uint8))

    def modelB_state_dict(self):
        return unpack_state_dict(self.paramsB)

    def targetB_state_dict(self):
        return unpack_state_dict(self.paramsT)

    def set_modelA(self, state):
        self._aA_ready = False
        self.paramsA = pack_state_dict(state, self.device)
        self.w_opp[0] = fold(self.paramsA, _lib.PM_FOLD_TRAIN if self.modelA_noisy else _lib.PM_FOLD_EVAL)[0]

    def modelA_state_dict(self):
        return unpack_state_dict(self.paramsA)

    def optimizer_state_dict(self):
        shapes = [(1, 64), (1,), (1, 64), (1,), (3, 64), (3,), (3, 64), (3,)]
        return checkpoint.adam_state_dict(shapes, self.adam_m, self.adam_v, self.counters()["train_steps"],
                                          self.hparams["lr"])

    def reset_B(self, state, epsilon=1.0):
        self.paramsB.copy_(pack_state_dict(state, self.device))
        self.paramsT.copy_(self.paramsB)
        self.adam_m.zero_()
        self.adam_v.zero_()
        self.prios.zero_()
        self.per_work.zero_()
        c = _lib.Ctrl.from_buffer_copy(bytes(self.ctrl.cpu().numpy().tobytes()))
        c.pos = c.size = c.train_steps = c.frame_idx = 0
        c.max_prio = 1.0
        c.epsilon = float(epsilon)
        self.ctrl.copy_(torch.frombuffer(bytearray(bytes(c)), dtype=torch.uint8))
        self.prepare()
        if self.frow is not None:
            self._frow_wait = 0
            self.sp.frow_ready = 1

    def prepare(self):
        self._aA_ready = False
        self._frow_pushed(False)
        check(self.lib.pm_selfplay_prepare(ctypes.byref(self.sp), stream_ptr()), "pm_selfplay_prepare")


HEAD_NAMES = HEAD_KEYS
__all__ = ["SelfPlayLearner", "sharded_vector_step", "splitmix64", "HEAD_NAMES", "PM_QNET_NP", "PM_GRAD_EPISODES",
           "PM_GRAD_UPDATED", "PM_GRAD_LEN"]
```

Baseline: 1.964 billion env-steps/s.

## Compute player-B greedy actions ahead inside learn kernel via published fresh heads

Side blocks of the fused learn kernel now compute B's hidden features, poll for freshly folded Q-heads that the learner publishes through a tagged global buffer, and write argmax actions directly into a per-arena int8 buffer. The following actenv kernel reads these precomputed actions instead of doing the head matmul, and falls back to stored features when a block's poll times out. This moves action selection off the env tick's critical path, at the cost of cross-block spin-waiting, extra LDS, and new host-side ready-state bookkeeping.

```diff
diff --git a/include/pongmi.h b/include/pongmi.h
--- a/include/pongmi.h
+++ b/include/pongmi.h
@@ -8,7 +8,7 @@
 extern "C" {
 #endif
 
-#define PM_ABI_VERSION 25
+#define PM_ABI_VERSION 26
 
 #define PM_OK 0
 #define PM_E_ARG (-1)
@@ -289,8 +289,13 @@
     float *featB;
     float *frow;
     int32_t frow_ready;
-    int32_t _pad1;
+    int32_t gB_ready;
+    int8_t *gB;
+    uint64_t *gheads;
 } pm_selfplay;
+#define PM_GB_NONE 3
+#define PM_GHEADS_EPOCH 260
+#define PM_GHEADS_LEN 264
 
 #define PM_MAX_BATCH 256
 
@@ -311,6 +316,7 @@
 int pm_selfplay_learn_act(const pm_selfplay* sp, void* stream);
 int pm_selfplay_actenv(const pm_selfplay* sp, void* stream);
 int pm_selfplay_step_overlap(const pm_selfplay* sp, void* stream);
+int pm_selfplay_act_ahead(const pm_selfplay* sp, int32_t mode, int32_t with_act);
 
 #define PM_UPD_FIRST 1
 #define PM_UPD_LAST 2
diff --git a/pingpong-selfplay-ai_amd/csrc/pm_mfma.h b/pingpong-selfplay-ai_amd/csrc/pm_mfma.h
--- a/pingpong-selfplay-ai_amd/csrc/pm_mfma.h
+++ b/pingpong-selfplay-ai_amd/csrc/pm_mfma.h
@@ -494,6 +494,16 @@
     typedef __attribute__((ext_vector_type(4))) unsigned u32x4;
     __builtin_amdgcn_raw_buffer_store_b128(*reinterpret_cast<const u32x4*>(&v), r, byte_off, 0, 16 );
 }
+__device__ __forceinline__ void feat_store(float* __restrict__ feat, int tl, int lane, const f32x16 (&c2)[2]) {
+    const __amdgpu_buffer_rsrc_t rs = __builtin_amdgcn_make_buffer_rsrc(feat, (short)0, 0x7fffffff, 0x00020000);
+    const int off = (tl * 8 * 64 + lane) * 16;
+#pragma unroll
+    for (int k = 0; k < 4; ++k) {
+        store_f4_sc1(rs, off + k * 64 * 16, make_float4(c2[0][4 * k], c2[0][4 * k + 1], c2[0][4 * k + 2], c2[0][4 * k + 3]));
+        store_f4_sc1(rs, off + (4 + k) * 64 * 16,
+                     make_float4(c2[1][4 * k], c2[1][4 * k + 1], c2[1][4 * k + 2], c2[1][4 * k + 3]));
+    }
+}
 __device__ __forceinline__ void feat_tiles(float* lw, const float* __restrict__ w, const float* __restrict__ obs, int n,
                                            int t0, int t1, float* __restrict__ feat) {
     const int wave = threadIdx.x >> 6, lane = threadIdx.x & 63, nw = blockDim.x >> 6;
@@ -508,14 +518,7 @@
         if (tn < t1) tile_inputs(obs + (size_t)min(tn * 32 + (lane & 31), n - 1) * 7, lane >> 5, xn);
         f32x16 c2[2];
         tile_hidden(lw, xs, lane, c2);
-        const __amdgpu_buffer_rsrc_t rs = __builtin_amdgcn_make_buffer_rsrc(feat, (short)0, 0x7fffffff, 0x00020000);
-        const int off = (tl * 8 * 64 + lane) * 16;
-#pragma unroll
-        for (int k = 0; k < 4; ++k) {
-            store_f4_sc1(rs, off + k * 64 * 16, make_float4(c2[0][4 * k], c2[0][4 * k + 1], c2[0][4 * k + 2], c2[0][4 * k + 3]));
-            store_f4_sc1(rs, off + (4 + k) * 64 * 16,
-                         make_float4(c2[1][4 * k], c2[1][4 * k + 1], c2[1][4 * k + 2], c2[1][4 * k + 3]));
-        }
+        feat_store(feat, tl, lane, c2);
 #pragma unroll
         for (int k = 0; k < 4; ++k) xs[k] = xn[k];
     }
diff --git a/pingpong-selfplay-ai_amd/csrc/pm_selfplay.hip b/pingpong-selfplay-ai_amd/csrc/pm_selfplay.hip
--- a/pingpong-selfplay-ai_amd/csrc/pm_selfplay.hip
+++ b/pingpong-selfplay-ai_amd/csrc/pm_selfplay.hip
@@ -13,6 +13,10 @@
 #define PM_SIDE(k, sb, v)                                                        \
     do {                                                                         \
         if (threadIdx.x == 0 && (sb) < 1024) pm_diag_side[(k)][(sb)] = (v);      \
+    } while (0)
+#define PM_STAMP_MAX_NB(slot)                                                                              \
+    do {                                                                                                   \
+        if (threadIdx.x == 0) atomicMax(&pm_diag_buf[(slot)], (unsigned long long)__builtin_amdgcn_s_memrealtime()); \
     } while (0)
 #define PM_ENV_STAMP(k, blk)                                                                   \
     do {                                                                                       \
@@ -27,6 +31,9 @@
 #else
 #define PM_SIDE(k, sb, v) \
     do {                  \
+    } while (0)
+#define PM_STAMP_MAX_NB(slot) \
+    do {                      \
     } while (0)
 #define PM_ENV_STAMP(k, blk) \
     do {                     \
@@ -96,6 +103,71 @@
 #endif
 constexpr bool kEnvWTRows = (PM_ENV_WT & 1) != 0, kEnvWTState = (PM_ENV_WT & 2) != 0, kEnvWTObs = (PM_ENV_WT & 4) != 0;
 __host__ __device__ inline int feat_ntiles(int n) { return (n + 31) / 32; }
+
+__device__ __forceinline__ bool gb_current(const pm_selfplay& sp) {
+    return sp.featB && sp.gB && sp.gB_ready && !sp.frow;
+}
+__device__ __forceinline__ uint32_t* gh_epoch(const pm_selfplay& sp) {
+    return reinterpret_cast<uint32_t*>(sp.gheads + PM_GHEADS_EPOCH);
+}
+constexpr int kAheadPollMax = 20000;
+__device__ __forceinline__ void gh_publish(const pm_selfplay& sp, int k, uint32_t tag, float v) {
+    __hip_atomic_store(sp.gheads + k, ((uint64_t)tag << 32) | __float_as_uint(v), __ATOMIC_RELAXED, __HIP_MEMORY_SCOPE_AGENT);
+}
+
+struct FeatAheadSmem {
+    float lw[kLwFloats];
+    float hf[264];
+    int ok;
+};
+__device__ __forceinline__ void feat_tiles_ahead(const pm_selfplay& sp, FeatAheadSmem& sm, int t0, int t1, bool force_timeout) {
+    const int t = threadIdx.x, wave = t >> 6, lane = t & 63, nw = blockDim.x >> 6;
+    stage_frags_lds(sp.w_B, sm.lw, t0);
+    const uint32_t tag = __hip_atomic_load(gh_epoch(sp), __ATOMIC_RELAXED, __HIP_MEMORY_SCOPE_AGENT) + 1u;
+    const int tl[2] = {t0 + wave, t0 + wave + nw};
+    const bool has[2] = {tl[0] < t1, tl[1] < t1};
+    float xs[2][4] = {{0.f, 0.f, 0.f, 0.f}, {0.f, 0.f, 0.f, 0.f}};
+#pragma unroll
+    for (int k = 0; k < 2; ++k)
+        if (has[k]) tile_inputs(sp.obsB + (size_t)min(tl[k] * 32 + (lane & 31), sp.n - 1) * 7, lane >> 5, xs[k]);
+    if (t == 0) sm.ok = 1;
+    __syncthreads();
+    f32x16 c2[2][2] = {};
+#pragma unroll
+    for (int k = 0; k < 2; ++k)
+        if (has[k]) tile_hidden(sm.lw, xs[k], lane, c2[k]);
+    PM_STAMP_MAX_NB(68);
+    if (t < 260) {
+        const int c = t & 3, r = (t >> 2) & 15, tt = (t >> 6) & 1, h = t >> 7;
+        const int src = t < 256 ? c * 64 + 32 * tt + rho(r) + 4 * h : t;
+        uint64_t g = 0;
+        bool got = false;
+        for (int it = 0; !force_timeout && it < kAheadPollMax; ++it) {
+            g = __hip_atomic_load(sp.gheads + src, __ATOMIC_RELAXED, __HIP_MEMORY_SCOPE_AGENT);
+            if ((uint32_t)(g >> 32) == tag) { got = true; break; }
+            __builtin_amdgcn_s_sleep(2);
+        }
+        if (got) sm.hf[t] = __uint_as_float((uint32_t)g);
+        else sm.ok = 0;
+    }
+    __syncthreads();
+    PM_STAMP_MAX_NB(69);
+    const bool ok = sm.ok != 0;
+#pragma unroll
+    for (int k = 0; k < 2; ++k) {
+        if (!has[k]) continue;
+        const int arena = tl[k] * 32 + (lane & 31);
+        int a = PM_GB_NONE;
+        if (ok) {
+            float q[3];
+            tile_heads(sm.hf, c2[k], lane, q);
+            a = argmax3(q);
+        } else {
+            feat_store(sp.featB, tl[k], lane, c2[k]);
+        }
+        if (lane < 32 && arena < sp.n) sp.gB[arena] = (int8_t)a;
+    }
+}
 
 __global__ __launch_bounds__(kActBlock, 4) void k_act_sp(const pm_selfplay sp, int part) {
     __shared__ __attribute__((aligned(16))) ActSpShared sh;
@@ -284,7 +356,9 @@
     PM_ENV_STAMP(0, blk);
     float xs[2][4];
     f32x16 fc2[2][2];
-    if (ACT && sp.featB) {
+    const bool ahead = ACT && gb_current(sp);
+    if (ahead) {
+    } else if (ACT && sp.featB) {
         if (threadIdx.x < 65)
             reinterpret_cast<float4*>(lw + F_H)[threadIdx.x] =
                 reinterpret_cast<const float4*>(sp.w_B + PLAIN + F_H)[threadIdx.x];
@@ -307,7 +381,7 @@
     const float er0 = sp.ep_reward[ii];
     Arena a = load_arena(sp.st, ii);
     const int aA = sp.aA[ii];
-    int aB = ACT ? 0 : sp.aB[ii];
+    int aB = ACT ? (ahead ? (int)sp.gB[ii] : 0) : sp.aB[ii];
     __builtin_amdgcn_sched_barrier(0);
     const float maxp = push_prio(size, cmaxp);
     float* leaf = per_tree(sp.per_work, sp.cap).leaf;
@@ -326,7 +400,21 @@
         asm volatile("" ::"v"(onext), "v"(svx), "v"(svy), "v"(sspn), "v"(eps_hit), "v"(eps_a));
         __builtin_amdgcn_sched_barrier(0);
     }
-    if (ACT) {
+    if (ahead) {
+        const unsigned long long fb = __ballot(valid && aB == PM_GB_NONE);
+        if (fb) {
+#pragma unroll
+            for (int k = 0; k < 2; ++k) {
+                if (!(uint32_t)(fb >> (32 * k))) continue;
+                float q[3];
+                feat_load(sp.featB, blk * 8 + 2 * wv + k, lane, fc2[k]);
+                tile_heads(sp.w_B + PLAIN + F_H, fc2[k], lane, q);
+                if ((lane >> 5) == k) aB = argmax3(q);
+            }
+        }
+        if (!valid) aB = 0;
+        PM_ENV_STAMP(7, blk);
+    } else if (ACT) {
         __syncthreads();
         PM_ENV_STAMP(7, blk);
         int act[2];
@@ -510,12 +598,17 @@
         for (int k = threadIdx.x; k < PM_QNET_NHEAD + 2; k += blockDim.x) sm.g[k] = sp.grad[k];
 }
 
-__device__ __forceinline__ void derive_weights(const pm_selfplay& sp, ApplySmem& sm) {
+__device__ __forceinline__ void derive_weights(const pm_selfplay& sp, ApplySmem& sm, bool gh_on = false, uint32_t gh_tag = 0) {
     const int t = threadIdx.x;
     float* lh = sp.learn_heads;
     const int g = (t - 256) >> 8, u = (t - 256) & 255;
     if (t >= 256 && g == 0) {
         fold_heads_from(sm.hp, nullptr, sm.nact, PM_FOLD_TRAIN_FRESH, sm.heads[0], sp.paramsB + PM_QNET_EPS_OFF, u, 256);
+        if (gh_on) {
+            gh_publish(sp, u, gh_tag, sm.heads[0][u]);
+            if (u < 4) gh_publish(sp, 256 + u, gh_tag, sm.heads[0][256 + u]);
+            PM_STAMP_T(22, 256);
+        }
     } else if (t >= 256 && g == 1) {
         fold_heads_from(sm.hp, nullptr, sm.ntrain, PM_FOLD_TRAIN_FRESH, sm.heads[1], lh + 528, u, 256);
     } else if (t >= 256 && g == 2) {
@@ -574,7 +667,8 @@
     if (sm.g[kGradN + 1] > 0.5f)
         for (int k = t; k < PM_QNET_NHEAD; k += nt) adam_one(sp, sm, k, sm.g[k]);
 }
-__device__ __forceinline__ void apply_finish(const pm_selfplay& sp, ApplySmem& sm, const pm_ctrl& cs, int mode) {
+__device__ __forceinline__ void apply_finish(const pm_selfplay& sp, ApplySmem& sm, const pm_ctrl& cs, int mode,
+                                             bool gh_on = false, uint32_t gh_tag = 0) {
     const int t = threadIdx.x, nt = blockDim.x;
     const bool train = sm.g[kGradN + 1] > 0.5f;
     const int64_t ts = cs.train_steps + (train ? 1 : 0);
@@ -588,7 +682,7 @@
         }
         __syncthreads();
     }
-    derive_weights(sp, sm);
+    derive_weights(sp, sm, gh_on, gh_tag);
     PM_STAMP(21);
     if (t == 0) {
         pm_ctrl* c = sp.ctrl;
@@ -1018,6 +1112,7 @@
     ActSharedLearn act;
     PushFwdSmem pf;
     TreeRefreshSmem tr;
+    FeatAheadSmem fa;
 };
 static_assert(sizeof(LearnShared) <= 160 * 1024, "k_learn LDS");
 
@@ -1026,7 +1121,7 @@
 }
 
 template <bool PG>
-__global__ __launch_bounds__(kLearn) void k_learn(const pm_selfplay sp, int chunkA, int chunkP, int mode, int tr, int ftiles, int sleepf) {
+__global__ __launch_bounds__(kLearn) void k_learn(const pm_selfplay sp, int chunkA, int chunkP, int mode, int tr, int ftiles, int sleepf, int ahead) {
     __shared__ __attribute__((aligned(16))) LearnShared shm;
     const bool push2 = (tr & 2) != 0, late_noise = (tr & 4) != 0;
     const int tr_poll = (tr & 16) ? 0 : kTrPollMax;
@@ -1048,7 +1143,8 @@
         if (fb >= 0) {
             if (sleepf & 2) side_nap(sleepf >> 8);
             const int t0 = fb * ftiles;
-            feat_tiles(shm.act.lw, sp.w_B, sp.obsB, sp.n, t0, min(t0 + ftiles, feat_ntiles(sp.n)), sp.featB);
+            if (ahead & 1) feat_tiles_ahead(sp, shm.fa, t0, min(t0 + ftiles, feat_ntiles(sp.n)), (ahead & 2) != 0);
+            else feat_tiles(shm.act.lw, sp.w_B, sp.obsB, sp.n, t0, min(t0 + ftiles, feat_ntiles(sp.n)), sp.featB);
             PM_STAMP_MAX(67);
             PM_SIDE(2, sb, __builtin_amdgcn_s_memrealtime());
             PM_SIDE(3, sb, 1ull | ((unsigned long long)(min(t0 + ftiles, feat_ntiles(sp.n)) - t0) << 16));
@@ -1085,6 +1181,7 @@
     const int64_t id_l = t < B ? sp.idx[t] : 0;
     const float eps_v = t < 260 ? sp.learn_heads[528 + t] : 0.f;
     const uint32_t tr_tag = tr ? __hip_atomic_load(tr_epoch(sp), __ATOMIC_RELAXED, __HIP_MEMORY_SCOPE_AGENT) + 1u : 0u;
+    const uint32_t gh_tag = (ahead & 1) ? __hip_atomic_load(gh_epoch(sp), __ATOMIC_RELAXED, __HIP_MEMORY_SCOPE_AGENT) + 1u : 0u;
     if (t < PM_MAX_BATCH) {
         const float4* src = reinterpret_cast<const float4*>(sp.hfeat + (size_t)min(t, B - 1) * 80 + 64);
 #pragma unroll
@@ -1385,6 +1482,11 @@
                 adam_one(sp, sm.ap, ksg, gsg);
             }
         }
+        if ((ahead & 1) && t < 260) {
+            fold_heads_from(sm.ap.hp, nullptr, sm.ap.nact, PM_FOLD_TRAIN_FRESH, sm.ap.heads[0], nullptr, t, kLearn);
+            gh_publish(sp, t, gh_tag, sm.ap.heads[0][t]);
+            PM_STAMP(22);
+        }
         PM_STAMP(8); PM_STAMP_T(9, 960);
         if (!tr) {
             const int j = min(t >> 2, B - 1);
@@ -1434,8 +1536,9 @@
         if (t == 0) push_wait(sp, cs);
         __syncthreads();
     }
-    if (sp.fuse_apply) apply_finish(sp, sm.ap, cs, mode);
+    if (sp.fuse_apply) apply_finish(sp, sm.ap, cs, mode, (ahead & 1) && !train, gh_tag);
     if (t == 0) {
+        if (ahead & 1) __hip_atomic_store(gh_epoch(sp), gh_tag, __ATOMIC_RELAXED, __HIP_MEMORY_SCOPE_AGENT);
         if (first) {
             c->ep_step = ep_fin;
             c->episodes = cs.episodes + ep_fin;
@@ -2174,10 +2277,11 @@
     int ftiles;
 };
 constexpr int kSideRows = 480;
-int side_sleep() {
+constexpr int kNapAhead = 2;
+int side_sleep(bool ahead) {
     const char* e = getenv("PONGMI_SIDE_SLEEP");
     const char* n = getenv("PONGMI_SIDE_NAP");
-    const int roles = e && *e ? atoi(e) : 2, nap = n && *n ? atoi(n) : 8;
+    const int roles = e && *e ? atoi(e) : 2, nap = n && *n ? atoi(n) : (ahead ? kNapAhead : 8);
     return (roles & 3) | (std::max(0, std::min(nap, 64)) << 8);
 }
 int device_cus() {
@@ -2220,14 +2324,30 @@
     return v;
 }
 
+unsigned learn_blocks(const pm_selfplay* sp, bool with_act, const LearnGrid& lg) {
+    unsigned blocks = 2u + (with_act ? (unsigned)lg.g.blocks() : 0u);
+    if (with_act && sp->featB) blocks += (unsigned)((feat_ntiles(sp->n) + lg.ftiles - 1) / lg.ftiles);
+    return blocks;
+}
+
+int act_ahead(const pm_selfplay* sp, int mode, bool with_act, const LearnGrid& lg) {
+    if (!with_act || !sp->fuse_apply || mode != (PM_UPD_FIRST | PM_UPD_LAST) || !sp->featB || !sp->gB || !sp->gheads ||
+        sp->frow || lg.ftiles > 2 * (kLearn / 64) || (int)learn_blocks(sp, with_act, lg) > device_cus())
+        return 0;
+    const char* e = getenv("PONGMI_ACT_AHEAD");
+    if (e && *e && atoi(e) == 0) return 0;
+    const char* f = getenv("PONGMI_AHEAD_FORCE_TIMEOUT");
+    return 1 | ((f && *f && atoi(f) != 0) << 1);
+}
+
 int launch_learn(const pm_selfplay* sp, bool with_act, hipStream_t st, int mode = PM_UPD_FIRST | PM_UPD_LAST) {
     const LearnGrid lg = learn_grid(sp);
     const ActGrid& g = lg.g;
-    unsigned blocks = 2u + (with_act ? (unsigned)g.blocks() : 0u);
-    if (with_act && sp->featB) blocks += (unsigned)((feat_ntiles(sp->n) + lg.ftiles - 1) / lg.ftiles);
+    const unsigned blocks = learn_blocks(sp, with_act, lg);
     const int tr = tree_refresh_block();
+    const int ahead = act_ahead(sp, mode, with_act, lg);
     pm_launch(PM_TIMER_LEARN, (tr & 8) ? k_learn<true> : k_learn<false>, dim3(blocks), dim3(kLearn), st, *sp, g.chunk0,
-              g.chunk1, mode, tr, lg.ftiles, side_sleep());
+              g.chunk1, mode, tr, lg.ftiles, side_sleep(ahead & 1), ahead);
     PM_LAUNCHED("k_learn");
     return PM_OK;
 }
@@ -2276,6 +2396,11 @@
 extern "C" int pm_selfplay_learn_act(const pm_selfplay* sp, void* stream) {
     int rc = check(sp);
     return rc ? rc : launch_learn(sp, true, pm_stream(stream));
+}
+
+extern "C" int pm_selfplay_act_ahead(const pm_selfplay* sp, int32_t mode, int32_t with_act) {
+    if (check(sp)) return 0;
+    return act_ahead(sp, (int)mode, with_act != 0, learn_grid(sp)) & 1;
 }
 
 extern "C" int pm_selfplay_apply(const pm_selfplay* sp, void* stream) {
diff --git a/pingpong-selfplay-ai_amd/pongmi/_lib.py b/pingpong-selfplay-ai_amd/pongmi/_lib.py
--- a/pingpong-selfplay-ai_amd/pongmi/_lib.py
+++ b/pingpong-selfplay-ai_amd/pongmi/_lib.py
@@ -28,7 +28,8 @@
 PM_ACT_ALL, PM_ACT_B, PM_ACT_A = 0, 1, 2
 PM_UPD_FIRST, PM_UPD_LAST = 1, 2
 PM_COMM_ID_BYTES = 128
-ABI_VERSION = 25
+ABI_VERSION = 26
+PM_GB_NONE, PM_GHEADS_LEN = 3, 264
 PM_TIMER_ACTENV, PM_TIMER_LEARN, PM_TIMER_RNN_ACT, PM_TIMER_ENV_STEP, PM_TIMER_ROLLOUT, PM_TIMER_DRQN = 0, 1, 2, 3, 4, 5
 PM_TIMER_LEARN_MULTI, PM_TIMER_N = 6, 7
 PM_ROLL_HEADS = 264
@@ -64,7 +65,8 @@
         [(n, c_double) for n in ("gamma", "alpha", "lr", "beta1", "beta2", "adam_eps", "min_epsilon", "epsilon_decay",
                                  "pool_ratio", "beta_start")] + \
         [("beta_frames", c_i64), ("target_update_interval", c_i64), ("seed_env", c_u64), ("seed_net", c_u64),
-         ("featB", c_void_p), ("frow", c_void_p), ("frow_ready", c_i32), ("_pad1", c_i32)]
+         ("featB", c_void_p), ("frow", c_void_p), ("frow_ready", c_i32), ("gB_ready", c_i32), ("gB", c_void_p),
+         ("gheads", c_void_p)]
 
 
 class RollReplay(ctypes.Structure):
@@ -170,6 +172,7 @@
     "pm_selfplay_learn_act": (c_i32, [c_void_p, c_void_p]),
     "pm_selfplay_actenv": (c_i32, [c_void_p, c_void_p]),
     "pm_selfplay_step_overlap": (c_i32, [c_void_p, c_void_p]),
+    "pm_selfplay_act_ahead": (c_i32, [c_void_p, c_i32, c_i32]),
     "pm_selfplay_learn_ex": (c_i32, [c_void_p, c_i32, c_i32, c_void_p]),
     "pm_selfplay_apply_ex": (c_i32, [c_void_p, c_i32, c_void_p]),
     "pm_selfplay_resample": (c_i32, [c_void_p, c_void_p]),
diff --git a/pingpong-selfplay-ai_amd/pongmi/selfplay.py b/pingpong-selfplay-ai_amd/pongmi/selfplay.py
--- a/pingpong-selfplay-ai_amd/pongmi/selfplay.py
+++ b/pingpong-selfplay-ai_amd/pongmi/selfplay.py
@@ -50,7 +50,7 @@
         if self.updates_per_step < 1:
             raise ValueError("updates_per_step must be >= 1")
         self.overlap = bool(overlap)
-        self._aA_ready = False
+        self._aA = self._gB_ready = False
         self.device = torch.device(device if device is not None else "cuda")
         if self.device.type != "cuda":
             raise _lib.PongmiError("SelfPlayLearner runs on a ROCm device only")
@@ -95,6 +95,8 @@
         self.aA = torch.zeros(n, dtype=torch.int8, device=dev)
         self.aB = torch.zeros(n, dtype=torch.int8, device=dev)
         self.featB = torch.zeros(((n + 31) // 32) * 2048, **f32) if features_ahead else None
+        self.gB = torch.full((n,), _lib.PM_GB_NONE, dtype=torch.int8, device=dev) if features_ahead else None
+        self.gheads = torch.zeros(_lib.PM_GHEADS_LEN, dtype=torch.int64, device=dev) if features_ahead else None
         use_frow = learn_multi and self.updates_per_step > 1 and features_ahead and self.overlap and world == 1
         self.frow = torch.zeros((self.cap, 64), **f32) if use_frow else None
         self._frow_wait = 0
@@ -114,6 +116,7 @@
             setattr(sp, name, ptr(getattr(self, name)))
         sp.featB = ptr(self.featB)
         sp.frow = ptr(self.frow)
+        sp.gB, sp.gheads, sp.gB_ready = ptr(self.gB), ptr(self.gheads), 0
         sp.frow_ready = int(self.frow is not None)
         sp.n, sp.n_pool, sp.batch, sp.world, sp.cap = n, self.n_pool, self.batch, self.world, self.cap
         sp.fuse_apply = int(bool(fuse_apply) and self.world == 1)
@@ -131,6 +134,20 @@
                             beta_start=beta_start, beta_frames=beta_frames)
         check(self.lib.pm_selfplay_init(ctypes.byref(sp), stream_ptr()), "pm_selfplay_init")
 
+    @property
+    def _aA_ready(self):
+        return self._aA
+
+    @_aA_ready.setter
+    def _aA_ready(self, v):
+        self._aA = bool(v)
+        if not v:
+            self._gB_ready = False
+
+    def _learned_act(self, mode):
+        self._aA_ready = True
+        self._gB_ready = bool(self.lib.pm_selfplay_act_ahead(ctypes.byref(self.sp), int(mode), 1))
+
     def _frow_pushed(self, through_actenv):
         if self.frow is None:
             return
@@ -149,8 +166,10 @@
         check(self.lib.pm_selfplay_act_part(ctypes.byref(self.sp), int(part), stream_ptr()), "pm_selfplay_act_part")
         if part != _lib.PM_ACT_B:
             self._aA_ready = True
+            self._gB_ready = False
 
     def actenv(self):
+        self.sp.gB_ready = int(self._gB_ready)
         self._aA_ready = False
         self._frow_pushed(True)
         check(self.lib.pm_selfplay_actenv(ctypes.byref(self.sp), stream_ptr()), "pm_selfplay_actenv")
@@ -163,7 +182,7 @@
     def learn(self, act_next=False):
         if act_next:
             check(self.lib.pm_selfplay_learn_act(ctypes.byref(self.sp), stream_ptr()), "pm_selfplay_learn_act")
-            self._aA_ready = True
+            self._learned_act(_lib.PM_UPD_FIRST | _lib.PM_UPD_LAST)
         else:
             check(self.lib.pm_selfplay_learn(ctypes.byref(self.sp), stream_ptr()), "pm_selfplay_learn")
 
@@ -174,7 +193,7 @@
         check(self.lib.pm_selfplay_learn_ex(ctypes.byref(self.sp), int(mode), int(bool(act_next)), stream_ptr()),
               "pm_selfplay_learn_ex")
         if act_next:
-            self._aA_ready = True
+            self._learned_act(mode)
 
     def apply_ex(self, mode):
         check(self.lib.pm_selfplay_apply_ex(ctypes.byref(self.sp), int(mode), stream_ptr()), "pm_selfplay_apply_ex")
@@ -189,9 +208,11 @@
         self._frow_pushed(True)
         if not self._aA_ready:
             self.act(_lib.PM_ACT_A)
+        self.sp.gB_ready = int(self._gB_ready)
         check(self.lib.pm_selfplay_step_sharded(ctypes.byref(self.sp), comm, self.updates_per_step, stream_ptr()),
               "pm_selfplay_step_sharded")
         self._aA_ready = True
+        self._gB_ready = False
 
     def _step_multi(self):
         U = self.updates_per_step
@@ -199,8 +220,10 @@
             if not self._aA_ready:
                 self.act(_lib.PM_ACT_A)
             self._frow_pushed(True)
+            self.sp.gB_ready = int(self._gB_ready)
             check(self.lib.pm_selfplay_step_multi(ctypes.byref(self.sp), U, stream_ptr()), "pm_selfplay_step_multi")
             self._aA_ready = True
+            self._gB_ready = False
             return
         sharded_vector_step(self, self.allreduce if self.world > 1 else None, U)
 
@@ -222,8 +245,9 @@
         if not self._aA_ready:
             self.act(_lib.PM_ACT_A)
         self._frow_pushed(True)
+        self.sp.gB_ready = int(self._gB_ready)
         check(self.lib.pm_selfplay_step_overlap(ctypes.byref(self.sp), stream_ptr()), "pm_selfplay_step_overlap")
-        self._aA_ready = True
+        self._learned_act(_lib.PM_UPD_FIRST | _lib.PM_UPD_LAST)
 
     def counters(self):
         c = _lib.Ctrl.from_buffer_copy(bytes(self.ctrl.cpu().numpy().tobytes()))
```

New measurement: 2.014 billion env-steps/s, median of 6. 2.5% higher.
